# open-mmlab/PowerPaint

Hardware: AMD Instinct MI355X
Metric: inpainted images/sec @512x512, 50-step DDIM CFG, batch4/GPU (higher is better)
Workload: dtype bf16; 1 GPU; ppt-v1 SD1.5-inpaint UNet (9-ch in), 512x512, 50-step DDIM, CFG=7.5, bf16, batch=4/GPU; global_batch=4, denoise_steps=50, network_evaluations=50, parallelism=dp1 (image shards, no step collectives), hipgraph=True, weights=random init (no checkpoints offline)

## Files before the change

### include/pp_hip.h

```cpp
#ifndef PP_HIP_H_
#define PP_HIP_H_

#include <stddef.h>
#include <stdint.h>

#ifdef __cplusplus
extern "C" {
#endif

#define PP_OK 0
#define PP_ERR_BAD_ARG (-1)
#define PP_ERR_UNSUPPORTED (-2)
#define PP_ERR_LAUNCH (-3)
#define PP_ERR_WORKSPACE (-4)

#define PP_ABI_VERSION 29
#define PP_DT_F32 0
#define PP_DT_BF16 1
#define PP_DT_F16 2
int pp_abi_version(void);
const char* pp_build_id(void);
const char* pp_last_error(void);

#define PP_X_PLAIN 0
#define PP_X_CONV3X3 1
#define PP_ACT_NONE 0
#define PP_ACT_GEGLU 1
#define PP_ACT_SILU 2
#define PP_ACT_SOFTMAX80 3

typedef struct PPGemmArgs {
  int32_t M, N, K;
  int32_t x_mode;
  const void* x1;
  const void* x2;
  int32_t c1, c2;
  int32_t ldx1, ldx2;
  int32_t batch, hin, win, hout, wout, stride, up;
  const void* w;
  const float* bias;
  const float* rowvec;
  int32_t ld_rowvec, rows_per_batch;
  const void* res1;
  int32_t ldres1;
  const void* res2;
  int32_t ldres2;
  float scale;
  int32_t act;
  void* out;
  int32_t ldo;
  int32_t out_f32;
  void* out_vt;
  int32_t vt_col0;
  int32_t vt_ld;
  int32_t splitk;
  int32_t tile;
  float* workspace;
  int32_t dbg;
  int32_t dtype;
  int32_t out_dup_rows;
  int32_t res1_wrap_rows;
  float* row_stats_out;
  const float* ln_stats;
  const float* ln_colsum;
  int32_t ln_tiles;
  int32_t ln_dim;
  float ln_eps;
  int32_t w_batch_stride;
  int64_t* gn_acc[2];
  int32_t gn_cg[2];
  int32_t gn_c0[2];
  int32_t gn_groups[2];
  const void* x3;
  const void* x4;
  int32_t c3;
  int32_t c4;
  const int64_t* gn_in_acc;
  const float* gn_in_gb;
  int32_t gn_in_groups;
  int32_t gn_in_silu;
  float gn_in_eps;
  int32_t gn_dup_batch;
  void* gn_next_out;
  const float* gn_next_gamma;
  const float* gn_next_beta;
  float gn_next_eps;
  int32_t gn_next_silu;
  int32_t gn_next_sub;
  int32_t gn_dup_mask;
  int32_t vec_batch_stride;
  uint64_t* tile_ctr;
  uint32_t* combine_fault;
  int32_t subpix;
} PPGemmArgs;
#define PP_GN_SUM_SCALE 16777216.0f
#define PP_GN_SQ_SCALE 1048576.0f

#define PP_TILE_AUTO 0
#define PP_TILE_128x160 1
#define PP_TILE_64x160 2
#define PP_TILE_256x160 3

int pp_gemm_bf16(const PPGemmArgs* args, void* stream);
size_t pp_gemm_workspace_bytes(const PPGemmArgs* args);
int pp_gemm_gn_stats_ok(const PPGemmArgs* args);
int pp_conv_gn_supported(const PPGemmArgs* args);
int pp_conv_gn_preferred(const PPGemmArgs* args);
int pp_upconv_subpix_supported(int batch, int h, int w, int cin, int cout, int dtype);
int pp_upconv_subpix_supported_to(int batch, int h, int w, int hout, int wout, int cin, int cout, int dtype);
int pp_upconv_fold(const void* w, int cout, int cin, int dtype, void* out, void* stream);
int pp_gemm_gn_next_ok(const PPGemmArgs* args, int sub);
size_t pp_gemm_combine_ctr_bytes(const PPGemmArgs* args);
int pp_gemm_combine_fused(const PPGemmArgs* args);
int pp_xcd_placement_ok(void);

int pp_linear_skinny(const float* x, int rows, int K, const void* w, const float* bias, int N, float* out, int ldo,
                     int act_in, int act_out, int dtype, void* stream);

int pp_timestep_embedding(const float* t_dev, int rows, int dim, float* out, void* stream);

size_t pp_groupnorm_workspace_bytes(int batch, int hw, int C);
int pp_groupnorm_stats(const void* x1, int c1, const void* x2, int c2, int batch, int hw, int groups,
                       float* workspace, int dtype, void* stream);
int pp_groupnorm_apply(const void* x1, int c1, const void* x2, int c2, int batch, int hw, int groups, float eps,
                       const float* gamma, const float* beta, const float* workspace, int silu, void* y,
                       int dtype, void* stream);

int pp_groupnorm_apply_acc(const void* x1, int c1, const void* x2, int c2, int batch, int hw, int groups, float eps,
                           const float* gamma, const float* beta, const int64_t* acc, int silu, void* y, int dtype,
                           void* stream);
int pp_zero_u64(void* dst, long long n, void* stream);

int pp_layernorm(const void* x, int rows, int C, const float* gamma, const float* beta, float eps, void* y,
                 int dtype, void* stream);

int pp_attention_fwd(const void* q, int ldq, const void* k, int ldk, const void* vt, int ldvt, void* o, int ldo,
                     int batch, int heads, int nq, int nk, int d, float scale, int dtype, void* stream);
#define PP_ATTN_AUTO 0
#define PP_ATTN_PHASED 1
#define PP_ATTN_PIPE_Q32 2
#define PP_ATTN_PIPE_Q64 3
#define PP_ATTN_PIPE_LOG2 4
int pp_attention_log2_ok(int nq, int nk, int d);
int pp_attention_fwd_variant(const void* q, int ldq, const void* k, int ldk, const void* vt, int ldvt, void* o, int ldo,
                             int batch, int heads, int nq, int nk, int d, float scale, int dtype, int variant,
                             void* stream);
int pp_transpose_v(const void* v, int ld, int batch, int nk, int cols, void* vt, int ldvt, void* stream);

int pp_conv3x3_direct(const void* x, int batch, int hin, int win, int cin, const void* w, const float* bias,
                      int cout, int stride, int silu_out, const void* add, void* out, int dtype, void* stream);
int pp_conv3x3_smallcout(const void* x, int batch, int h, int w_, int cin, const void* w, const float* bias, int cout,
                         float* out_nchw, int dtype, void* stream);
int pp_gn_conv3x3_smallcout_supported(int cin, int cout, int groups);
int pp_gn_conv3x3_smallcout(const void* x, int batch, int h, int w, int cin, int groups, float eps, const float* gamma,
                            const float* beta, const int64_t* acc, const void* wgt, const float* bias, int cout,
                            float* out_nchw, int dtype, void* stream);

int pp_nchw_to_nhwc(const void* src, int src_dtype, int batch, int c, int hw, int src_batch_mod, void* dst, int ldc,
                    int c0, int dtype, void* stream);
int pp_nhwc_to_nchw(const void* src, int batch, int c, int hw, void* dst, int dst_dtype, int dtype, void* stream);
int pp_add_bf16(const void* a, const void* b, void* out, long long n, int dtype, void* stream);

int pp_cfg_sched_step(const float* eps2, int cfg, float guidance, float* latents, float* m_prev, int n, int kind,
                      const float* coef_table, int32_t* step_dev, uint32_t* advance_ticket, void* stream);
int pp_ddim_variance_noise(float* latents, const float* noise, int n, const float* coef_table, const int32_t* step_dev,
                           void* stream);
int pp_cfg_lcm_step(const float* eps2, int cfg, float guidance, float* latents, const float* noise, int n,
                    const float* coef_table, int32_t* step_dev, uint32_t* advance_ticket, void* stream);
int pp_cfg_sigma_step(const float* eps2, int cfg, float guidance, float* latents, const float* noise, int n,
                      const float* coef_table, int32_t* step_dev, uint32_t* advance_ticket, void* stream);
int pp_cfg_ksampler_step(const float* eps2, int cfg, float guidance, float* latents, float* state, const float* noise, int n,
                         const float* coef_table, int32_t* step_dev, uint32_t* advance_ticket, void* stream);

int pp_tfront_supported(int M, int c, int rows_per_batch, int gn_groups);
int pp_tfront(const void* x, int ldx, const void* gn_acc, const float* gn_gamma, const float* gn_beta, float gn_eps, int gn_groups,
              const void* w1, const float* b1, const void* w2p, const float* cs2, const float* b2, float ln_eps, void* hs,
              int ldhs, void* qk, int ldqk, void* vt, int ldvt, int M, int c, int rows_per_batch, float q_scale, int dtype,
              void* stream);
int pp_xattn_block_supported(int M, int c, int rows_per_batch, int nctx, int heads);
int pp_xattn_fold(const void* k, int ldk, const void* vt, int ldvt, int batch, int nctx, int heads, int c, const void* wq,
                  const float* q_colsum, const float* q_bias, const void* wo, float scale, void* gt, float* gcs,
                  float* gbias, void* ht, int kperm, int dtype, void* stream);
int pp_xattn_block(const void* x, int ldx, const void* res, int ldres, const float* ln_stats, int ln_tiles, float ln_eps,
                   const void* gt, const float* gcs, const float* gbias, const void* ht, const float* bias_o, void* out,
                   int ldo, float* row_stats_out, int M, int c, int rows_per_batch, int src_wrap_rows, const void* pre_w,
                   const float* pre_b, int dtype, void* stream);

int pp_ff_fused_supported(int M, int c, int rows_per_batch);
int pp_ff_fused(const PPGemmArgs* g2, const void* w1, const float* b1, const float* cs1, const float* ln_stats, int ln_tiles,
                float ln_eps, int w2_kperm, void* stream);

int pp_latent_blend(float* latents, const float* image_latents, const float* mask, const float* noise,
                    const float* renoise_table, const int32_t* step_dev, int batch, int channels, int hw, void* stream);

int pp_step_head(const float* temb_table, const int32_t* step_dev, float* temb_out, int row_floats, const float* latents,
                 int batch, int c, int hw, int src_batch_mod, void* x_in, int ldc, int c0, int dtype, void* zero_dst,
                 long long n_zero, void* stream);
int pp_step_head_scaled(const float* temb_table, const int32_t* step_dev, float* temb_out, int row_floats, const float* latents,
                        int batch, int c, int hw, int src_batch_mod, void* x_in, int ldc, int c0, int dtype, void* zero_dst,
                        long long n_zero, const float* in_div, void* stream);
int pp_step_select_t(const float* timesteps, const int32_t* step_dev, float* t_out, void* stream);
int pp_step_advance(int32_t* step_dev, void* stream);

int pp_mask_prep(int mode, const float* a, const float* b, float* out, int batch, int c, int h, int w, int ho, int wo,
                 void* stream);

int pp_embed_splice(const void* table, const void* ext, const int32_t* src_row, void* out, int n_rows,
                    long long row_bytes, void* stream);

int pp_softmax_rows(const float* s, long long lds, int rows, int n, float scale, void* p, long long ldp, int dtype,
                    void* stream);

int pp_attention_small(const void* q, int ldq, const void* k, int ldk, const void* v, int ldv, void* o, int ldo,
                       int batch, int heads, int nq, int nk, int d, float scale, int causal, int dtype, void* stream);

#define PP_LORA_MAX_ADAPTERS 8
#define PP_LORA_MAX_RANK 128
#define PP_LORA_ROWS_PLAIN 0
#define PP_LORA_ROWS_GEGLU 1
#define PP_LORA_COLS_PLAIN 0
#define PP_LORA_COLS_IGEMM 1
#define PP_LORA_COLS_KPERM 2
#define PP_LORA_COLS_KPERM_GEGLU 3
typedef struct PPLoraMergeArgs {
  int32_t N, K;
  const float* w;
  int64_t ldw;
  int32_t n_adapters;
  int32_t rank[PP_LORA_MAX_ADAPTERS];
  float coef[PP_LORA_MAX_ADAPTERS];
  const float* up[PP_LORA_MAX_ADAPTERS];
  const float* down[PP_LORA_MAX_ADAPTERS];
  const float* gamma;
  const float* beta;
  const float* badd;
  void* out;
  int64_t ldo;
  int32_t out_rows, out_cols, out_dtype;
  int32_t row_mode, row_off;
  int32_t col_mode, col_off, taps, cin_pad;
  float* colsum;
  float* bias;
} PPLoraMergeArgs;
int pp_lora_merge(const PPLoraMergeArgs* args, void* stream);

int pp_freeu(const void* hidden, void* hidden_out, int ch, const void* skip, void* skip_out, int cs, int batch, int h, int w,
             const float* bs, int64_t* acc, int groups, int dtype, void* stream);

#define PP_IP_MAX_TOKENS 64
int pp_ip_attn_add(const void* q, int ldq, const void* k_ip, const void* v_ip, void* o, int ldo, int batch, int heads, int nq,
                   int nk, int d, float qk_scale, float ip_scale, int dtype, void* stream);

#ifdef __cplusplus
}
#endif
#endif
```

### powerpaint_amd/_lib.py

```python
import ctypes as C
import os

_HERE = os.path.dirname(os.path.abspath(__file__))
LIB_PATH = os.path.join(_HERE, "libpp_hip.so")
if os.environ.get("PP_LAB") == "1" and os.environ.get("PP_LIB"):
    LIB_PATH = os.path.abspath(os.environ["PP_LIB"])

PP_X_PLAIN, PP_X_CONV3X3 = 0, 1
PP_ACT_NONE, PP_ACT_GEGLU, PP_ACT_SILU, PP_ACT_SOFTMAX80 = 0, 1, 2, 3
PP_TILE_AUTO, PP_TILE_128x160, PP_TILE_64x160, PP_TILE_256x160 = 0, 1, 2, 3
PP_DT_F32, PP_DT_BF16, PP_DT_F16 = 0, 1, 2
PP_ATTN_AUTO, PP_ATTN_PHASED, PP_ATTN_PIPE_Q32, PP_ATTN_PIPE_Q64, PP_ATTN_PIPE_LOG2 = 0, 1, 2, 3, 4
ABI_VERSION = 29
PP_ERR = {0: "PP_OK", -1: "PP_ERR_BAD_ARG", -2: "PP_ERR_UNSUPPORTED", -3: "PP_ERR_LAUNCH", -4: "PP_ERR_WORKSPACE"}

vp, i32, f32, sz = C.c_void_p, C.c_int32, C.c_float, C.c_size_t


class PPGemmArgs(C.Structure):
    _fields_ = [
        ("M", i32), ("N", i32), ("K", i32), ("x_mode", i32),
        ("x1", vp), ("x2", vp),
        ("c1", i32), ("c2", i32), ("ldx1", i32), ("ldx2", i32),
        ("batch", i32), ("hin", i32), ("win", i32), ("hout", i32), ("wout", i32), ("stride", i32), ("up", i32),
        ("w", vp), ("bias", vp), ("rowvec", vp),
        ("ld_rowvec", i32), ("rows_per_batch", i32),
        ("res1", vp), ("ldres1", i32),
        ("res2", vp), ("ldres2", i32),
        ("scale", f32), ("act", i32),
        ("out", vp), ("ldo", i32), ("out_f32", i32),
        ("out_vt", vp), ("vt_col0", i32), ("vt_ld", i32),
        ("splitk", i32), ("tile", i32),
        ("workspace", vp),
        ("dbg", i32), ("dtype", i32), ("out_dup_rows", i32), ("res1_wrap_rows", i32),
        ("row_stats_out", vp), ("ln_stats", vp), ("ln_colsum", vp),
        ("ln_tiles", i32), ("ln_dim", i32), ("ln_eps", f32), ("w_batch_stride", i32),
        ("gn_acc", vp * 2), ("gn_cg", i32 * 2), ("gn_c0", i32 * 2), ("gn_groups", i32 * 2),
        ("x3", vp), ("x4", vp), ("c3", i32), ("c4", i32),
        ("gn_in_acc", vp), ("gn_in_gb", vp), ("gn_in_groups", i32), ("gn_in_silu", i32), ("gn_in_eps", f32),
        ("gn_dup_batch", i32),
        ("gn_next_out", vp), ("gn_next_gamma", vp), ("gn_next_beta", vp), ("gn_next_eps", f32), ("gn_next_silu", i32),
        ("gn_next_sub", i32), ("gn_dup_mask", i32), ("vec_batch_stride", i32),
        ("tile_ctr", vp), ("combine_fault", vp),
        ("subpix", i32),
    ]


def gemm_args(dtype: int, M: int, N: int, K: int, x, w, out, x2=None, K2: int = 0, ldx=None, ldx2: int = 0, ldo: int = 0,
              ldres1: int = 0, ldres2: int = 0, rows_per_batch: int = 0, scale: float = 1.0) -> PPGemmArgs:
    a = PPGemmArgs()
    a.dtype = dtype
    a.M, a.N, a.K, a.x_mode = M, N, K + K2, PP_X_PLAIN
    a.x1, a.x2, a.c1, a.c2 = x, x2 or None, K, K2
    a.ldx1, a.ldx2 = (K if ldx is None else ldx), (ldx2 or K2)
    a.w, a.out = w, out
    a.ldo, a.ldres1, a.ldres2 = ldo or N, ldres1 or N, ldres2 or N
    a.rows_per_batch, a.scale = rows_per_batch, scale
    return a


def conv3x3_args(dtype: int, B: int, H: int, W: int, c1: int, cout: int, x, x2=None, c2: int = 0, x3=None, c3: int = 0,
                 x4=None, c4: int = 0, stride: int = 1, up: bool = False, w=None, out=None, scale: float = 1.0,
                 up_size=None) -> PPGemmArgs:
    hv, wv = (2 * H, 2 * W) if up else (H, W)
    if up_size is not None:
        if not up or stride != 1 or up_size[0] not in (2 * H - 1, 2 * H) or up_size[1] not in (2 * W - 1, 2 * W):
            raise ValueError(f"up_size {tuple(up_size)} is no nearest-resize target of a {H}x{W} source")
        hv, wv = up_size
    ho, wo = (hv - 1) // stride + 1, (wv - 1) // stride + 1
    a = PPGemmArgs()
    a.dtype = dtype
    a.M, a.N, a.K, a.x_mode = B * ho * wo, cout, 9 * (c1 + c2) + c3 + c4, PP_X_CONV3X3
    a.x1, a.x2, a.c1, a.c2 = x, x2 or None, c1, c2
    a.x3, a.x4, a.c3, a.c4 = x3 or None, x4 or None, c3, c4
    a.batch, a.hin, a.win, a.hout, a.wout, a.stride, a.up = B, H, W, ho, wo, stride, int(up)
    a.w, a.out = w, out
    a.ldo, a.ldres1, a.ldres2 = cout, cout, cout
    a.rows_per_batch, a.scale = ho * wo, scale
    return a


PP_LORA_MAX_ADAPTERS, PP_LORA_MAX_RANK = 8, 128
PP_LORA_ROWS_PLAIN, PP_LORA_ROWS_GEGLU = 0, 1
PP_IP_MAX_TOKENS = 64
PP_LORA_COLS_PLAIN, PP_LORA_COLS_IGEMM, PP_LORA_COLS_KPERM, PP_LORA_COLS_KPERM_GEGLU = 0, 1, 2, 3


class PPLoraMergeArgs(C.Structure):
    _fields_ = [
        ("N", i32), ("K", i32), ("w", vp), ("ldw", C.c_int64), ("n_adapters", i32),
        ("rank", i32 * PP_LORA_MAX_ADAPTERS), ("coef", f32 * PP_LORA_MAX_ADAPTERS),
        ("up", vp * PP_LORA_MAX_ADAPTERS), ("down", vp * PP_LORA_MAX_ADAPTERS),
        ("gamma", vp), ("beta", vp), ("badd", vp),
        ("out", vp), ("ldo", C.c_int64), ("out_rows", i32), ("out_cols", i32), ("out_dtype", i32),
        ("row_mode", i32), ("row_off", i32), ("col_mode", i32), ("col_off", i32), ("taps", i32), ("cin_pad", i32),
        ("colsum", vp), ("bias", vp),
    ]


SIGNATURES = {
    "pp_abi_version": (C.c_int, []),
    "pp_last_error": (C.c_char_p, []),
    "pp_build_id": (C.c_char_p, []),
    "pp_gemm_bf16": (C.c_int, [C.POINTER(PPGemmArgs), vp]),
    "pp_gemm_workspace_bytes": (sz, [C.POINTER(PPGemmArgs)]),
    "pp_linear_skinny": (C.c_int, [vp, C.c_int, C.c_int, vp, vp, C.c_int, vp, C.c_int, C.c_int, C.c_int, C.c_int, vp]),
    "pp_timestep_embedding": (C.c_int, [vp, C.c_int, C.c_int, vp, vp]),
    "pp_groupnorm_workspace_bytes": (sz, [C.c_int, C.c_int, C.c_int]),
    "pp_gemm_gn_stats_ok": (C.c_int, [C.POINTER(PPGemmArgs)]),
    "pp_conv_gn_supported": (C.c_int, [C.POINTER(PPGemmArgs)]),
    "pp_conv_gn_preferred": (C.c_int, [C.POINTER(PPGemmArgs)]),
    "pp_gemm_gn_next_ok": (C.c_int, [C.POINTER(PPGemmArgs), C.c_int]),
    "pp_upconv_subpix_supported": (C.c_int, [C.c_int] * 6),
    "pp_upconv_subpix_supported_to": (C.c_int, [C.c_int] * 8),
    "pp_upconv_fold": (C.c_int, [vp, C.c_int, C.c_int, C.c_int, vp, vp]),
    "pp_gemm_combine_ctr_bytes": (sz, [C.POINTER(PPGemmArgs)]),
    "pp_gemm_combine_fused": (C.c_int, [C.POINTER(PPGemmArgs)]),
    "pp_xcd_placement_ok": (C.c_int, []),
    "pp_groupnorm_apply_acc": (C.c_int, [vp, C.c_int, vp, C.c_int, C.c_int, C.c_int, C.c_int, f32, vp, vp, vp, C.c_int, vp,
                                         C.c_int, vp]),
    "pp_zero_u64": (C.c_int, [vp, C.c_longlong, vp]),
    "pp_embed_splice": (C.c_int, [vp, vp, vp, vp, C.c_int, C.c_longlong, vp]),
    "pp_attention_small": (C.c_int, [vp, C.c_int, vp, C.c_int, vp, C.c_int, vp, C.c_int, C.c_int, C.c_int, C.c_int,
                                     C.c_int, C.c_int, f32, C.c_int, C.c_int, vp]),
    "pp_softmax_rows": (C.c_int, [vp, C.c_longlong, C.c_int, C.c_int, f32, vp, C.c_longlong, C.c_int, vp]),
    "pp_groupnorm_stats": (C.c_int, [vp, C.c_int, vp, C.c_int, C.c_int, C.c_int, C.c_int, vp, C.c_int, vp]),
    "pp_groupnorm_apply": (C.c_int, [vp, C.c_int, vp, C.c_int, C.c_int, C.c_int, C.c_int, f32, vp, vp, vp, C.c_int, vp,
                                     C.c_int, vp]),
    "pp_layernorm": (C.c_int, [vp, C.c_int, C.c_int, vp, vp, f32, vp, C.c_int, vp]),
    "pp_attention_fwd": (C.c_int, [vp, C.c_int, vp, C.c_int, vp, C.c_int, vp, C.c_int, C.c_int, C.c_int, C.c_int,
                                   C.c_int, C.c_int, f32, C.c_int, vp]),
    "pp_attention_fwd_variant": (C.c_int, [vp, C.c_int, vp, C.c_int, vp, C.c_int, vp, C.c_int, C.c_int, C.c_int, C.c_int,
                                           C.c_int, C.c_int, f32, C.c_int, C.c_int, vp]),
    "pp_transpose_v": (C.c_int, [vp, C.c_int, C.c_int, C.c_int, C.c_int, vp, C.c_int, vp]),
    "pp_conv3x3_direct": (C.c_int, [vp, C.c_int, C.c_int, C.c_int, C.c_int, vp, vp, C.c_int, C.c_int, C.c_int, vp,
                                    vp, C.c_int, vp]),
    "pp_conv3x3_smallcout": (C.c_int, [vp, C.c_int, C.c_int, C.c_int, C.c_int, vp, vp, C.c_int, vp, C.c_int, vp]),
    "pp_nchw_to_nhwc": (C.c_int, [vp, C.c_int, C.c_int, C.c_int, C.c_int, C.c_int, vp, C.c_int, C.c_int, C.c_int, vp]),
    "pp_nhwc_to_nchw": (C.c_int, [vp, C.c_int, C.c_int, C.c_int, vp, C.c_int, C.c_int, vp]),
    "pp_add_bf16": (C.c_int, [vp, vp, vp, C.c_longlong, C.c_int, vp]),
    "pp_cfg_sched_step": (C.c_int, [vp, C.c_int, f32, vp, vp, C.c_int, C.c_int, vp, vp, vp, vp]),
    "pp_step_select_t": (C.c_int, [vp, vp, vp, vp]),
    "pp_ddim_variance_noise": (C.c_int, [vp, vp, C.c_int, vp, vp, vp]),
    "pp_cfg_lcm_step": (C.c_int, [vp, C.c_int, f32, vp, vp, C.c_int, vp, vp, vp, vp]),
    "pp_cfg_sigma_step": (C.c_int, [vp, C.c_int, f32, vp, vp, C.c_int, vp, vp, vp, vp]),
    "pp_cfg_ksampler_step": (C.c_int, [vp, C.c_int, f32, vp, vp, vp, C.c_int, vp, vp, vp, vp]),
    "pp_latent_blend": (C.c_int, [vp, vp, vp, vp, vp, vp, C.c_int, C.c_int, C.c_int, vp]),
    "pp_gn_conv3x3_smallcout_supported": (C.c_int, [C.c_int] * 3),
    "pp_gn_conv3x3_smallcout": (C.c_int, [vp, C.c_int, C.c_int, C.c_int, C.c_int, C.c_int, C.c_float, vp, vp, vp, vp, vp,
                                          C.c_int, vp, C.c_int, vp]),
    "pp_tfront_supported": (C.c_int, [C.c_int] * 4),
    "pp_tfront": (C.c_int, [vp, C.c_int, vp, vp, vp, C.c_float, C.c_int, vp, vp, vp, vp, vp, C.c_float, vp, C.c_int, vp, C.c_int,
                            vp, C.c_int, C.c_int, C.c_int, C.c_int, C.c_float, C.c_int, vp]),
    "pp_attention_log2_ok": (C.c_int, [C.c_int] * 3),
    "pp_xattn_block_supported": (C.c_int, [C.c_int] * 5),
    "pp_xattn_fold": (C.c_int, [vp, C.c_int, vp, C.c_int, C.c_int, C.c_int, C.c_int, C.c_int, vp, vp, vp, vp, C.c_float,
                                vp, vp, vp, vp, C.c_int, C.c_int, vp]),
    "pp_xattn_block": (C.c_int, [vp, C.c_int, vp, C.c_int, vp, C.c_int, C.c_float, vp, vp, vp, vp, vp, vp, C.c_int, vp,
                                 C.c_int, C.c_int, C.c_int, C.c_int, vp, vp, C.c_int, vp]),
    "pp_ff_fused_supported": (C.c_int, [C.c_int] * 3),
    "pp_ff_fused": (C.c_int, [C.POINTER(PPGemmArgs), vp, vp, vp, vp, C.c_int, C.c_float, C.c_int, vp]),
    "pp_step_head": (C.c_int, [vp, vp, vp, C.c_int, vp, C.c_int, C.c_int, C.c_int, C.c_int, vp, C.c_int, C.c_int, C.c_int, vp,
                              C.c_longlong, vp]),
    "pp_step_head_scaled": (C.c_int, [vp, vp, vp, C.c_int, vp, C.c_int, C.c_int, C.c_int, C.c_int, vp, C.c_int, C.c_int, C.c_int,
                                     vp, C.c_longlong, vp, vp]),
    "pp_step_advance": (C.c_int, [vp, vp]),
    "pp_lora_merge": (C.c_int, [C.POINTER(PPLoraMergeArgs), vp]),
    "pp_freeu": (C.c_int, [vp, vp, C.c_int, vp, vp, C.c_int, C.c_int, C.c_int, C.c_int, vp, vp, C.c_int, C.c_int, vp]),
    "pp_mask_prep": (C.c_int, [C.c_int, vp, vp, vp, C.c_int, C.c_int, C.c_int, C.c_int, C.c_int, C.c_int, vp]),
    "pp_ip_attn_add": (C.c_int, [vp, C.c_int, vp, vp, vp, C.c_int, C.c_int, C.c_int, C.c_int, C.c_int, C.c_int, f32, f32,
                                 C.c_int, vp]),
}

_lib = None


class PPError(RuntimeError):
    pass


def lib():
    global _lib
    if _lib is None:
        if not os.path.exists(LIB_PATH):
            raise PPError(
                f"{LIB_PATH} not found: the HIP extension is not built. Run `python -c 'import __graft_entry__ as g; "
                f"g.build()'` (or `make -C powerpaint_amd/csrc`). There is no CPU/PyTorch fallback.")
        l = C.CDLL(LIB_PATH)
        for name, (res, args) in SIGNATURES.items():
            fn = getattr(l, name)
            fn.restype = res
            fn.argtypes = args
        if l.pp_abi_version() != ABI_VERSION:
            raise PPError("libpp_hip.so ABI version mismatch")
        _lib = l
    return _lib


def dtype_code(dtype) -> int:
    import torch
    if dtype == torch.bfloat16:
        return PP_DT_BF16
    if dtype == torch.float16:
        return PP_DT_F16
    raise PPError(f"the HIP path computes in bf16 or fp16 (fp32 accumulate), not {dtype}")


def build_id() -> str:
    return lib().pp_build_id().decode()


def check(rc: int, what: str = ""):
    if rc != 0:
        msg = lib().pp_last_error().decode() if rc == -3 else ""
        raise PPError(f"{what} failed: {PP_ERR.get(rc, rc)} {msg}")
```

### powerpaint_amd/csrc/conv_gn.hip

```cpp
#include <type_traits>
#include <utility>

#include "pp_common.h"
#include "gemm_gn.h"
#include "gemm_combine.h"

namespace {

typedef __attribute__((address_space(3))) void* cg_lds_t;

constexpr int CG_T = 512, CG_BN = 160, CG_NI = 5;
constexpr int CG_WP = 3;
constexpr int CG_HPW_MAX = 6;
constexpr int CG_HALO_PX = 384;
constexpr int CG_HALO = CG_HALO_PX * 128;
constexpr int CG_WST = CG_BN * 128;
constexpr int CG_WOFF = 2 * CG_HALO;
constexpr int CG_TAB = CG_WOFF + 3 * CG_WST;
constexpr int CG_T_STATS = CG_TAB;
constexpr int CG_T_ZERO = CG_TAB + 256;
constexpr int CG_T_GB = CG_TAB + 1024;
constexpr int CG_T_SCSH = CG_TAB + 3072;
constexpr int CG_LDS = CG_TAB + 3584;
static_assert(CG_LDS <= 160 * 1024, "LDS budget");

struct CGDerived {
  int tiles_m, tiles_n, n_major;
  int nch1, nch;
  int ntail3, ntail;
  int hp;
  int cg;
  float inv_cg;
};

template <int... I, class F>
PP_DEVINL void cg_static_for_impl(std::integer_sequence<int, I...>, F&& f) { (f(std::integral_constant<int, I>{}), ...); }
template <int N, class F>
PP_DEVINL void cg_static_for(F&& f) { cg_static_for_impl(std::make_integer_sequence<int, N>{}, f); }

template <int BM, int HPW, bool PP, int NMODE, int EDT>
__global__ void __launch_bounds__(CG_T, 2) pp_conv_gn_kernel(const PPGemmArgs a, const CGDerived d) {
  using E = E16<EDT>;
  typedef typename E::v8 v8_t;
  constexpr int T = CG_T, WN = 2, MI = BM / 64, NI = CG_NI, BN = CG_BN;
  constexpr int CG_HPW = HPW;
  constexpr bool SUBPIX = NMODE == 4;
  static_assert(!SUBPIX || PP, "the sub-pixel form has the ping-pong loop only");
  constexpr bool NORM = NMODE != 2 && !SUBPIX;
  constexpr bool NREAD = NMODE == 0 || NMODE == 3;
  static_assert(HPW >= 2 && HPW <= CG_HPW_MAX, "halo strips per wave");
  constexpr int XP2 = BM / 64;
  constexpr int P2 = XP2 + CG_WP;
  constexpr int ST2 = BM * 128;
  constexpr int EPI_ROWS = 64, EPI_LD = BN * 4 + 16;
  constexpr int RS_OFF = EPI_ROWS * EPI_LD + BM * 8;
  static_assert(3 * ST2 <= 2 * CG_HALO, "tail stages live in the halo buffers");
  static_assert(MI * 16 <= EPI_ROWS && EPI_ROWS % (MI * 16) == 0, "wave rows vs epilogue pass");

  extern __shared__ __attribute__((aligned(16))) char smem[];

  const int tid = threadIdx.x;
  const int lane = tid & 63;
  const int wave = __builtin_amdgcn_readfirstlane(tid >> 6);
  const int wm = wave >> 1, wn = wave & 1;
  const int grp = wave >> 2;

  int lid;
  {
    const int nwg = gridDim.x, bid = blockIdx.x;
    const int q = nwg >> 3, r = nwg & 7, xcd = bid & 7, idx = bid >> 3;
    lid = (xcd < r ? xcd * (q + 1) : r * (q + 1) + (xcd - r) * q) + idx;
  }
  const int par = SUBPIX ? (lid & 3) : 0, pa = par >> 1, pb = par & 1;
  if constexpr (SUBPIX) lid >>= 2;
  int tile_m, tile_n;
  if (d.n_major) {
    tile_n = lid / d.tiles_m;
    tile_m = lid - tile_n * d.tiles_m;
  } else {
    tile_m = lid / d.tiles_n;
    tile_n = lid - tile_m * d.tiles_n;
  }
  const int m_blk = tile_m * BM, n_blk = tile_n * BN;
  const int split = blockIdx.y, splits = gridDim.y;
  const int ch_b = split * d.nch / splits, ch_e = (split + 1) * d.nch / splits;
  const int tk_b = split * d.ntail / splits, tk_e = (split + 1) * d.ntail / splits;

  const int Wd = a.wout, Hd = a.hout, HW = Hd * Wd;
  const int HWs = a.hin * a.win;
  const int bimg = m_blk / HW;
  const int y0 = (m_blk - bimg * HW) / Wd;
  const int ctot = a.c1 + a.c2;
  const uint32_t wbytes = (uint32_t)a.N * (uint32_t)a.K * 2u;
  const void* const wmat = SUBPIX ? (const void*)((const char*)a.w + (size_t)par * wbytes) : a.w;

  const int lrow = lane >> 3;
  const int kslot = (lane & 7) ^ lrow;

  int vw[CG_WP], wlds[CG_WP];
#pragma unroll
  for (int i = 0; i < CG_WP; ++i) {
    const int strip = (wave * 8 + i * 64 < BN) ? i : i - 1;
    const int n = n_blk + wave * 8 + lrow + strip * 64;
    vw[i] = (n < a.N) ? (n * a.K + kslot * 8) * 2 : (int)PP_OOB;
    wlds[i] = (wave * 8 + strip * 64) * 128;
  }
  int hpix[CG_HPW];
#pragma unroll
  for (int j = 0; j < CG_HPW; ++j) {
    const int hp = (wave + 8 * j) * 8 + lrow;
    const int hr = hp / Wd, hx = hp - hr * Wd;
    const int iy = y0 + hr - 1;
    hpix[j] = (hp < d.hp && iy >= 0 && iy < Hd) ? (a.up ? bimg * HWs + (iy >> 1) * a.win + (hx >> 1) : bimg * HW + iy * Wd + hx) : -1;
  }
  const int r16 = lane & 15, g = lane >> 4;
  const int fsw = r16 & 7;
  const int wrow0 = wn * (NI * 16) + r16;
  const int rt0 = wm * (MI * 16) + r16;
  unsigned edge = 0u;
#pragma unroll
  for (int mi = 0; mi < MI; ++mi) {
    const int lx = (rt0 + mi * 16) % Wd;
    if (lx == 0) edge |= 1u << mi;
    if (lx == Wd - 1) edge |= 1u << (8 + mi);
  }

  f32x4_t acc[NI][MI];
#pragma unroll
  for (int ni = 0; ni < NI; ++ni)
#pragma unroll
    for (int mi = 0; mi < MI; ++mi) acc[ni][mi] = f32x4_t{0.f, 0.f, 0.f, 0.f};

  auto mfma_all = [&](const v8_t (&wf)[2][NI], const v8_t (&xf)[2][MI]) __attribute__((always_inline)) {
#pragma unroll
    for (int ks = 0; ks < 2; ++ks)
#pragma unroll
      for (int ni = 0; ni < NI; ++ni)
#pragma unroll
        for (int mi = 0; mi < MI; ++mi) acc[ni][mi] = E::mfma16(wf[ks][ni], xf[ks][mi], acc[ni][mi]);
  };

  if (ch_b < ch_e) {
    auto issue_gb = [&](int c, int gbuf, bool live) __attribute__((always_inline)) {
      const __amdgpu_buffer_rsrc_t rs = make_rsrc(a.gn_in_gb, (NORM && live) ? (uint32_t)ctot * 8u : 0u);
      const int vo = lane < 32 ? lane * 16 : (int)PP_OOB;
      __builtin_amdgcn_raw_ptr_buffer_load_lds(rs, (cg_lds_t)(smem + CG_T_GB + gbuf * 1024), 16, vo, c * 512, 0, 0);
    };
    auto compute_scsh = [&](int c, int gbuf) __attribute__((always_inline)) {
      const char* gp = smem + CG_T_GB + gbuf * 1024 + kslot * 64;
      const f32x2_t* st = reinterpret_cast<const f32x2_t*>(smem + CG_T_STATS);
#pragma unroll
      for (int q = 0; q < 4; ++q) {
        const f32x4_t gbv = *reinterpret_cast<const f32x4_t*>(gp + q * 16);
        f32x4_t o;
#pragma unroll
        for (int h = 0; h < 2; ++h) {
          const int ch = c * 64 + kslot * 8 + 2 * q + h;
          const int gi = min((int)(((float)ch + 0.5f) * d.inv_cg), 31);
          const f32x2_t mr = st[gi];
          const float sv = mr[1] * gbv[2 * h];
          o[2 * h] = sv;
          o[2 * h + 1] = gbv[2 * h + 1] - mr[0] * sv;
        }
        if (lrow == 0) *reinterpret_cast<f32x4_t*>(smem + CG_T_SCSH + kslot * 64 + q * 16) = o;
      }
      asm volatile("s_waitcnt lgkmcnt(0)" ::: "memory");
    };
    auto norm_piece = [&](int hbuf, int j) __attribute__((always_inline)) {
      char* p = smem + hbuf * CG_HALO + (wave + 8 * j) * 1024 + lane * 16;
      if (hpix[j] >= 0) {
        const u32x4_t v = *reinterpret_cast<const u32x4_t*>(p);
        float r[8];
#pragma unroll
        for (int q = 0; q < 4; ++q) {
          const f32x4_t ss = *reinterpret_cast<const f32x4_t*>(smem + CG_T_SCSH + kslot * 64 + q * 16);
          r[2 * q] = E::lo(v[q]) * ss[0] + ss[1];
          r[2 * q + 1] = E::hi(v[q]) * ss[2] + ss[3];
        }
#pragma unroll
        for (int e = 0; e < 8; ++e)
          r[e] = r[e] * __builtin_amdgcn_rcpf(1.0f + __builtin_amdgcn_exp2f(r[e] * -1.44269504088896340736f));
        u32x4_t o;
#pragma unroll
        for (int q = 0; q < 4; ++q) o[q] = E::pack2(r[2 * q], r[2 * q + 1]);
        *reinterpret_cast<u32x4_t*>(p) = o;
      }
    };

    auto norm_math = [&](const u32x4_t v, uint32_t vmask) __attribute__((always_inline)) -> u32x4_t {
      u32x4_t o;
#pragma unroll
      for (int q = 0; q < 4; ++q) {
        const f32x4_t ss = *reinterpret_cast<const f32x4_t*>(smem + CG_T_SCSH + kslot * 64 + q * 16);
        float r0 = E::lo(v[q]) * ss[0] + ss[1];
        float r1 = E::hi(v[q]) * ss[2] + ss[3];
        const float e0 = __builtin_amdgcn_exp2f(r0 * -1.44269504088896340736f);
        const float e1 = __builtin_amdgcn_exp2f(r1 * -1.44269504088896340736f);
        r0 *= __builtin_amdgcn_rcpf(1.0f + e0);
        r1 *= __builtin_amdgcn_rcpf(1.0f + e1);
        o[q] = E::pack2(r0, r1) & vmask;
      }
      return o;
    };

    __amdgpu_buffer_rsrc_t rs_h = make_rsrc(a.x1, 0u);
    int hsoff = 0, hcsrc = 0;
    auto halo_source = [&](int c, bool live) __attribute__((always_inline)) {
      const bool first = c < d.nch1;
      int csrc;
      if (first) {
        csrc = a.c1;
        rs_h = make_rsrc(a.x1, live ? (uint32_t)a.batch * (uint32_t)HWs * (uint32_t)a.c1 * 2u : 0u);
        hsoff = c * 128;
      } else {
        csrc = a.c2;
        rs_h = make_rsrc(a.x2 ? a.x2 : a.x1, (live && a.x2) ? (uint32_t)a.batch * (uint32_t)HWs * (uint32_t)a.c2 * 2u : 0u);
        hsoff = (c - d.nch1) * 128;
      }
      hcsrc = csrc;
    };
    auto issue_halo_piece = [&](int hbuf, int j) __attribute__((always_inline)) {
      const int vo = hpix[j] >= 0 ? (hpix[j] * hcsrc + kslot * 8) * 2 : (int)PP_OOB;
      __builtin_amdgcn_raw_ptr_buffer_load_lds(rs_h, (cg_lds_t)(smem + hbuf * CG_HALO + (wave + 8 * j) * 1024), 16, vo,
                                               hsoff, 0, 0);
    };
    auto issue_w_piece = [&](const __amdgpu_buffer_rsrc_t rs, int stage, int i, int sow) __attribute__((always_inline)) {
      const int vo = vw[i], lo = wlds[i];
      __builtin_amdgcn_raw_ptr_buffer_load_lds(rs, (cg_lds_t)(smem + CG_WOFF + stage * CG_WST + lo), 16, vo, sow, 0, 0);
    };

    {
      const __amdgpu_buffer_rsrc_t rsw = make_rsrc(wmat, wbytes);
#pragma unroll
      for (int i = 0; i < CG_WP; ++i) issue_w_piece(rsw, 0, i, (0 * ctot + ch_b * 64) * 2);
#pragma unroll
// ... 349 lines not shown
        }
#pragma unroll
        for (int j = 0; j < EP; ++j) {
          const int row = r0 + j * ER, m = m0 + row;
          if (row < EPI_ROWS && m < a.M) {
            f32x4_t v0 = *reinterpret_cast<const f32x4_t*>(smem + row * EPI_LD + c8 * 32);
            f32x4_t v1 = *reinterpret_cast<const f32x4_t*>(smem + row * EPI_LD + c8 * 32 + 16);
            v0 += bs0;
            v1 += bs1;
            v0 *= a.scale;
            v1 *= a.scale;
            v0[0] += E::lo(r1[j][0]) + E::lo(r2[j][0]); v0[1] += E::hi(r1[j][0]) + E::hi(r2[j][0]);
            v0[2] += E::lo(r1[j][1]) + E::lo(r2[j][1]); v0[3] += E::hi(r1[j][1]) + E::hi(r2[j][1]);
            v1[0] += E::lo(r1[j][2]) + E::lo(r2[j][2]); v1[1] += E::hi(r1[j][2]) + E::hi(r2[j][2]);
            v1[2] += E::lo(r1[j][3]) + E::lo(r2[j][3]); v1[3] += E::hi(r1[j][3]) + E::hi(r2[j][3]);
            u32x4_t o;
            o[0] = E::pack2(v0[0], v0[1]); o[1] = E::pack2(v0[2], v0[3]);
            o[2] = E::pack2(v1[0], v1[1]); o[3] = E::pack2(v1[2], v1[3]);
            *reinterpret_cast<u32x4_t*>((uint16_t*)a.out + (SUBPIX ? out_row(m) : (size_t)m) * a.ldo + n) = o;
            if (gns) {
#pragma unroll
              for (int jj = 0; jj < 4; ++jj) {
                const float lo = E::lo(o[jj]), hi = E::hi(o[jj]);
                gcs[2 * jj] += lo; gcq[2 * jj] += lo * lo;
                gcs[2 * jj + 1] += hi; gcq[2 * jj + 1] += hi * hi;
              }
            }
          }
        }
      }
    }
  }
  if (gns) {
    unsigned long long* slots = reinterpret_cast<unsigned long long*>(smem + RS_OFF);
    if (tid < 2 * GN_SLOTS * 2) slots[tid] = 0ull;
    asm volatile("s_waitcnt lgkmcnt(0)\n\ts_barrier" ::: "memory");
    if (r0 < ER && n < a.N) {
      float* dstp = reinterpret_cast<float*>(smem) + ((size_t)r0 * BN + c8 * 8) * 2;
#pragma unroll
      for (int jj = 0; jj < 4; ++jj)
        *reinterpret_cast<f32x4_t*>(dstp + 4 * jj) = f32x4_t{gcs[2 * jj], gcq[2 * jj], gcs[2 * jj + 1], gcq[2 * jj + 1]};
    }
    asm volatile("s_waitcnt lgkmcnt(0)\n\ts_barrier" ::: "memory");
    const int ncols = min(BN, a.N - n_blk);
    if (tid < ncols) {
      float sm = 0.f, sq = 0.f;
#pragma unroll 5
      for (int r = 0; r < ER; ++r) {
        const f32x2_t v = *reinterpret_cast<const f32x2_t*>(smem + ((size_t)r * BN + tid) * 8);
        sm += v[0];
        sq += v[1];
      }
      gn_column(a, slots, n_blk, tid, sm, sq);
    }
    asm volatile("s_waitcnt lgkmcnt(0)\n\ts_barrier" ::: "memory");
    gn_flush(a, slots, m_blk, n_blk, ncols, tid);
  }
  if (splitk && a.tile_ctr) {
    static_assert(fc_lds_bytes(BM) <= CG_LDS, "fused combine staging must fit in the kernel's LDS");
    splitk_fused_combine<BM, T, EDT>(a, smem, m_blk, n_blk, blockIdx.x, blockIdx.y, splits, tid);
  }
}

bool cg_shape_ok(const PPGemmArgs& a, int bm) {
  const int hw = a.hout * a.wout;
  return bm % a.wout == 0 && hw % bm == 0 && bm + 2 * a.wout <= CG_HALO_PX;
}

bool cg_geometry_ok(const PPGemmArgs& a) {
  if (a.x_mode != PP_X_CONV3X3 || !pp_dt_ok(a.dtype)) return false;
  if (a.stride != 1 || a.wout < 8 || (a.wout & 7)) return false;
  if (a.up ? (a.hout != 2 * a.hin || a.wout != 2 * a.win) : (a.hin != a.hout || a.win != a.wout)) return false;
  const int ctot = a.c1 + a.c2;
  if (a.c1 <= 0 || a.c1 % 64 || a.c2 % 64 || (a.c2 > 0 && !a.x2)) return false;
  if (a.c3 < 0 || a.c4 < 0 || a.c3 % 64 || a.c4 % 64 || (a.c3 > 0 && !a.x3) || (a.c4 > 0 && (!a.x4 || a.c3 == 0))) return false;
  if (a.K != (a.subpix ? 4 : 9) * ctot + a.c3 + a.c4 || a.M != a.batch * a.hout * a.wout || a.M <= 0 || a.N <= 0) return false;
  if (a.N % 8 || a.ldo % 8 || a.out_f32 || a.out_vt || a.act != PP_ACT_NONE || a.ln_stats || a.row_stats_out) return false;
  if ((a.res1 && a.ldres1 % 8) || (a.res2 && a.ldres2 % 8)) return false;
  if (a.rows_per_batch != a.hout * a.wout || a.out_dup_rows > 0 || a.w_batch_stride > 0 || a.vec_batch_stride > 0) return false;
  if ((uint64_t)a.batch * a.hin * a.win * (uint64_t)(a.c1 > a.c2 ? a.c1 : a.c2) * 2u >= 0x80000000ull) return false;
  if ((uint64_t)a.N * (uint64_t)a.K * 2u >= 0x80000000ull) return false;
  if ((uint64_t)a.M * (uint64_t)(a.c3 > a.c4 ? a.c3 : a.c4) * 2u >= 0x80000000ull) return false;
  for (int k = 0; k < 2; ++k)
    if (a.gn_acc[k] && (a.gn_cg[k] < 8 || a.gn_groups[k] <= 0 || a.gn_c0[k] < 0)) return false;
  return cg_shape_ok(a, 256) || cg_shape_ok(a, 128) || cg_shape_ok(a, 64);
}

bool cg_fused_ok(const PPGemmArgs& a) {
  if (!a.gn_in_acc || !a.gn_in_gb || a.up || a.subpix || !cg_geometry_ok(a)) return false;
  if (a.gn_in_silu != 1 || a.gn_in_groups <= 0 || a.gn_in_groups > 32) return false;
  return (a.c1 + a.c2) % a.gn_in_groups == 0;
}

bool cg_raw_ok(const PPGemmArgs& a) {
  static const int min_w = pp_lab_env("PP_CONV_RAW", 16);
  if (a.gn_in_acc || a.gn_in_gb || a.subpix || a.tile != PP_TILE_AUTO || min_w <= 0 || a.wout < min_w) return false;
  return cg_geometry_ok(a);
}

bool cg_subpix_ok(const PPGemmArgs& a) {
  if (a.subpix != 1 || a.up || a.gn_in_acc || a.gn_in_gb || a.c2 || a.c3 || a.c4 || a.splitk > 1) return false;
  if (a.res1_wrap_rows > 0 || a.gn_next_out || a.gn_dup_mask) return false;
  return cg_geometry_ok(a);
}

CGChoice cg_choose_subpix(const PPGemmArgs& a) {
  const int tn = (a.N + 159) / 160;
  const int want = a.tile == PP_TILE_256x160 ? 256 : a.tile == PP_TILE_128x160 ? 128 : a.tile == PP_TILE_64x160 ? 64 : 0;
  if (want && cg_shape_ok(a, want)) return CGChoice{want, 1};
  for (int bm = 256; bm >= 64; bm >>= 1)
    if (cg_shape_ok(a, bm) && 4 * (a.M / bm) * tn >= 224) return CGChoice{bm, 1};
  return CGChoice{cg_shape_ok(a, 256) ? 256 : cg_shape_ok(a, 128) ? 128 : 64, 1};
}

CGChoice cg_choose(const PPGemmArgs& a) {
  const int tn = (a.N + 159) / 160;
  auto tiles = [&](int bm) { return (a.M / bm) * tn; };
  CGChoice c{0, 1};
  const int want = a.tile == PP_TILE_256x160 ? 256 : a.tile == PP_TILE_128x160 ? 128 : a.tile == PP_TILE_64x160 ? 64 : 0;
  const int nch0 = (a.c1 + a.c2) / 64;
  static const int sk2_from = pp_lab_env("PP_CONV_GN_SK2", 12);
#ifdef PP_LAB
  static const int w16 = pp_lab_env("PP_CONV_GN_W16", 0);
  if (w16 > 0 && a.wout == 16 && !want && a.splitk <= 0 && cg_shape_ok(a, w16 / 10)) {
    c.bm = w16 / 10;
    c.splitk = w16 % 10;
    if (c.splitk > nch0) c.splitk = nch0;
    return c;
  }
#endif
  if (want && cg_shape_ok(a, want)) c.bm = want;
  else if (cg_shape_ok(a, 256) && tiles(256) >= 224) c.bm = 256;
  else if (sk2_from > 0 && nch0 >= sk2_from && a.splitk <= 0 && cg_shape_ok(a, 256) && tiles(256) * 2 >= 224 &&
           tiles(256) < 224 && cg_shape_ok(a, 128) && tiles(128) >= 224) {
    c.bm = 256;
    c.splitk = 2;
    return c;
  }
  else if (cg_shape_ok(a, 128) && tiles(128) >= 224) c.bm = 128;
  else if (cg_shape_ok(a, 256) && cg_shape_ok(a, 128) && tiles(256) * 4 <= 256 && nch0 <= 10 && a.splitk <= 0) c.bm = 128;
  else if (cg_shape_ok(a, 256)) c.bm = 256;
  else if (cg_shape_ok(a, 128)) c.bm = 128;
  else c.bm = 64;
  const int nch = (a.c1 + a.c2) / 64;
  int sk = 1;
  while (tiles(c.bm) * sk * 2 <= 256 && nch / (sk * 2) >= 2 && sk < 8) sk *= 2;
  c.splitk = a.splitk > 0 ? a.splitk : sk;
  if (c.splitk > 8) c.splitk = 8;
  if (c.splitk > nch) c.splitk = nch;
  return c;
}

template <int BM, int HPW, bool PP, int NMODE, int EDT>
int cg_launch(const PPGemmArgs& a, int splitk, hipStream_t st) {
  auto kern = pp_conv_gn_kernel<BM, HPW, PP, NMODE, EDT>;
  if (pp_func_lds(reinterpret_cast<const void*>(kern), CG_LDS, "hipFuncSetAttribute(conv_gn)") != PP_OK) return PP_ERR_LAUNCH;
  CGDerived d;
  d.tiles_m = a.M / BM;
  d.tiles_n = (a.N + CG_BN - 1) / CG_BN;
  d.n_major = (d.tiles_m < d.tiles_n && d.tiles_m <= 8) ? 1 : 0;
  d.nch1 = a.c1 / 64;
  d.nch = (a.c1 + a.c2) / 64;
  d.ntail3 = a.c3 / 64;
  d.ntail = (a.c3 + a.c4) / 64;
  d.hp = BM + 2 * a.wout;
  d.cg = a.gn_in_groups > 0 ? (a.c1 + a.c2) / a.gn_in_groups : 1;
  d.inv_cg = 1.0f / (float)d.cg;
  hipLaunchKernelGGL(kern, dim3(d.tiles_m * d.tiles_n * (NMODE == 4 ? 4 : 1), splitk, 1), dim3(CG_T), CG_LDS, st, a, d);
  PP_CHECK_LAUNCH("pp_conv_gn_kernel");
  return PP_OK;
}

template <int BM, bool PP, int NMODE, int EDT>
int cg_launch_hpw(const PPGemmArgs& a, int splitk, hipStream_t st) {
  const int need = (BM + 2 * a.wout + 63) / 64;
  if constexpr (BM == 256) {
    if (need <= 5) return cg_launch<256, 5, PP, NMODE, EDT>(a, splitk, st);
    return cg_launch<256, 6, PP, NMODE, EDT>(a, splitk, st);
  } else if constexpr (BM == 128) {
    if (need <= 3) return cg_launch<128, 3, PP, NMODE, EDT>(a, splitk, st);
    if (need <= 4) return cg_launch<128, 4, PP, NMODE, EDT>(a, splitk, st);
    return cg_launch<128, 6, PP, NMODE, EDT>(a, splitk, st);
  } else {
    if (need <= 2) return cg_launch<64, 2, PP, NMODE, EDT>(a, splitk, st);
    return cg_launch<64, 3, PP, NMODE, EDT>(a, splitk, st);
  }
}

template <int EDT>
int cg_dispatch(const PPGemmArgs& a, const CGChoice& c, hipStream_t st) {
#ifdef PP_LAB
  static const int pp = pp_lab_env("PP_CONV_GN_PP", 1), nm = pp_lab_env("PP_CONV_GN_NMODE", 1);
  if (!pp || nm != 1) {
#define CG_CASE(BM_)                                                                        \
    case BM_:                                                                               \
      if (!pp) return cg_launch_hpw<BM_, false, 1, EDT>(a, c.splitk, st);                   \
      if (nm == 0) return cg_launch_hpw<BM_, true, 0, EDT>(a, c.splitk, st);                \
      if (nm == 2) return cg_launch_hpw<BM_, true, 2, EDT>(a, c.splitk, st);                \
      return cg_launch_hpw<BM_, true, 3, EDT>(a, c.splitk, st);
    switch (c.bm) {
      CG_CASE(256)
      CG_CASE(128)
      default:
      CG_CASE(64)
    }
#undef CG_CASE
  }
#endif
  if (a.subpix) {
    switch (c.bm) {
      case 256: return cg_launch_hpw<256, true, 4, EDT>(a, 1, st);
      case 128: return cg_launch_hpw<128, true, 4, EDT>(a, 1, st);
      default: return cg_launch_hpw<64, true, 4, EDT>(a, 1, st);
    }
  }
  if (!a.gn_in_acc) {
    switch (c.bm) {
      case 256: return cg_launch_hpw<256, true, 2, EDT>(a, c.splitk, st);
      case 128: return cg_launch_hpw<128, true, 2, EDT>(a, c.splitk, st);
      default: return cg_launch_hpw<64, true, 2, EDT>(a, c.splitk, st);
    }
  }
  switch (c.bm) {
    case 256: return cg_launch_hpw<256, true, 1, EDT>(a, c.splitk, st);
    case 128: return cg_launch_hpw<128, true, 1, EDT>(a, c.splitk, st);
    default: return cg_launch_hpw<64, true, 1, EDT>(a, c.splitk, st);
  }
}

}

int pp_conv_gn_form(const PPGemmArgs& a, CGChoice* c) {
  if (a.x_mode != PP_X_CONV3X3) return 0;
  if (a.subpix) {
    if (!cg_subpix_ok(a)) return PP_ERR_UNSUPPORTED;
    *c = cg_choose_subpix(a);
    return 1;
  }
  if (a.gn_in_acc) {
    if (!cg_fused_ok(a)) return PP_ERR_UNSUPPORTED;
  } else if (!cg_raw_ok(a)) {
    return 0;
  }
  *c = cg_choose(a);
  return 1;
}
int pp_conv_gn_run(const PPGemmArgs& a, const CGChoice& c, hipStream_t st) {
  if (c.splitk > 1 && !a.workspace) return PP_ERR_WORKSPACE;
  return a.dtype == PP_DT_F16 ? cg_dispatch<PP_DT_F16>(a, c, st) : cg_dispatch<PP_DT_BF16>(a, c, st);
}

extern "C" int pp_conv_gn_supported(const PPGemmArgs* args) {
  if (!args) return 0;
  return cg_fused_ok(*args) ? 1 : cg_raw_ok(*args) ? 2 : 0;
}

extern "C" int pp_upconv_subpix_supported(int batch, int h, int w, int cin, int cout, int dtype) {
  if (batch <= 0 || h <= 0 || w <= 0 || cin <= 0 || cout <= 0) return 0;
  PPGemmArgs a = {};
  a.x_mode = PP_X_CONV3X3;
  a.dtype = dtype;
  a.batch = batch;
  a.hin = a.hout = h;
  a.win = a.wout = w;
  a.stride = 1;
  a.c1 = cin;
  a.M = batch * h * w;
  a.N = cout;
  a.K = 4 * cin;
  a.ldo = a.ldres1 = a.ldres2 = cout;
  a.rows_per_batch = h * w;
  a.subpix = 1;
  if ((uint64_t)batch * h * w * 4u * (uint64_t)cout * 2u >= (1ull << 40)) return 0;
  if (!cg_subpix_ok(a)) return 0;
  return w >= 16 ? 2 : 1;
}

extern "C" int pp_upconv_subpix_supported_to(int batch, int h, int w, int hout, int wout, int cin, int cout, int dtype) {
  if (hout != 2 * h || wout != 2 * w) return 0;
  return pp_upconv_subpix_supported(batch, h, w, cin, cout, dtype);
}

extern "C" int pp_conv_gn_preferred(const PPGemmArgs* args) {
  if (!args || !cg_fused_ok(*args)) return 0;
  const PPGemmArgs& a = *args;
  const int nch = (a.c1 + a.c2) / 64;
  int cls;
  if (a.win >= 64) cls = 1;
  else if (a.win == 32) cls = (nch <= 5 && a.c2 == 0) ? 2 : 8;
  else if (a.win == 16) cls = 4;
  else cls = a.win < 16 ? 16 : 8;
  static const int mask = pp_lab_env("PP_CONV_GN_ROUTE", 0);
  return (mask & cls) ? 1 : 0;
}
```

### powerpaint_amd/csrc/gemm.hip

```cpp
#include "pp_common.h"
#include "gemm_gn.h"
#include "gemm_combine.h"

namespace {

struct GemmDerived {
  int tiles_m, tiles_n, kt_total, kt_per_split, ctiles;
  int n_major;
};

PP_DEVINL void ln_row_moments(const PPGemmArgs& a, int m, float& mean, float& rstd) {
  const f32x2_t* p = reinterpret_cast<const f32x2_t*>(a.ln_stats) + (size_t)m * a.ln_tiles;
  float s = 0.f, q = 0.f;
  for (int t = 0; t < a.ln_tiles; ++t) {
    const f32x2_t v = p[t];
    s += v[0];
    q += v[1];
  }
  const float inv = 1.0f / (float)a.ln_dim;
  mean = s * inv;
  rstd = rsqrtf(fmaxf(q * inv - mean * mean, 0.f) + a.ln_eps);
}

PP_DEVINL size_t res1_row(const PPGemmArgs& a, int m) {
  return (size_t)((a.res1_wrap_rows > 0 && m >= a.res1_wrap_rows) ? m - a.res1_wrap_rows : m);
}

template <int BN, int EDT>
PP_DEVINL void epilogue4(const PPGemmArgs& a, int m, int n, f32x4_t v) {
  if (a.ln_stats) {
    float mean, rstd;
    ln_row_moments(a, m, mean, rstd);
    const f32x4_t cs = *reinterpret_cast<const f32x4_t*>(a.ln_colsum + n);
    v = (v - cs * mean) * rstd;
  }
  if (a.bias) {
    const f32x4_t b = *reinterpret_cast<const f32x4_t*>(a.bias + n);
    v += b;
  }
  int bidx = 0, rin = m;
  if (a.rowvec || a.out_vt) {
    bidx = m / a.rows_per_batch;
    rin = m - bidx * a.rows_per_batch;
  }
  if (a.rowvec) {
    const f32x4_t t = *reinterpret_cast<const f32x4_t*>(a.rowvec + (size_t)bidx * a.ld_rowvec + n);
    v += t;
  }
  v *= a.scale;
  if (a.res1) {
    const u32x2_t r = *reinterpret_cast<const u32x2_t*>((const uint16_t*)a.res1 + res1_row(a, m) * a.ldres1 + n);
    v[0] += E16<EDT>::lo(r[0]); v[1] += E16<EDT>::hi(r[0]); v[2] += E16<EDT>::lo(r[1]); v[3] += E16<EDT>::hi(r[1]);
  }
  if (a.res2) {
    const u32x2_t r = *reinterpret_cast<const u32x2_t*>((const uint16_t*)a.res2 + (size_t)m * a.ldres2 + n);
    v[0] += E16<EDT>::lo(r[0]); v[1] += E16<EDT>::hi(r[0]); v[2] += E16<EDT>::lo(r[1]); v[3] += E16<EDT>::hi(r[1]);
  }
  if (a.act == PP_ACT_GEGLU) {
    const float o0 = v[0] * gelu_fast_f(v[2]);
    const float o1 = v[1] * gelu_fast_f(v[3]);
    *reinterpret_cast<uint32_t*>((uint16_t*)a.out + (size_t)m * a.ldo + (n >> 1)) = E16<EDT>::pack2(o0, o1);
    return;
  }
  if (a.act == PP_ACT_SILU) {
    v[0] = silu_f(v[0]); v[1] = silu_f(v[1]); v[2] = silu_f(v[2]); v[3] = silu_f(v[3]);
  }
  if (a.out_vt && n >= a.vt_col0) {
    const int ncols = a.N - a.vt_col0;
    uint16_t* dst = (uint16_t*)a.out_vt + ((size_t)bidx * ncols + (n - a.vt_col0)) * a.vt_ld + rin;
#pragma unroll
    for (int j = 0; j < 4; ++j) dst[(size_t)j * a.vt_ld] = E16<EDT>::from_f(v[j]);
    return;
  }
  if (a.out_f32) {
    *reinterpret_cast<f32x4_t*>((float*)a.out + (size_t)m * a.ldo + n) = v;
  } else {
    u32x2_t o;
    o[0] = E16<EDT>::pack2(v[0], v[1]);
    o[1] = E16<EDT>::pack2(v[2], v[3]);
    *reinterpret_cast<u32x2_t*>((uint16_t*)a.out + (size_t)m * a.ldo + n) = o;
  }
}

template <int BM, int BN, int WM, int WN, int XMODE, int EDT>
__global__ void __launch_bounds__(WM* WN * 64, 2) pp_gemm_kernel(const PPGemmArgs a, const GemmDerived d) {
  typedef typename E16<EDT>::v8 v8_t;
  constexpr int T = WM * WN * 64;
  constexpr int MI = BM / WM / 16;
  constexpr int NI = BN / WN / 16;
  constexpr int RPP = T / 8;
  constexpr int XP = (BM + RPP - 1) / RPP;
  constexpr int WP = (BN + RPP - 1) / RPP;
  constexpr int XBYTES = BM * 128, WBYTES = BN * 128, BUFBYTES = XBYTES + WBYTES;
  static_assert(BM % (WM * 16) == 0 && BN % (WN * 16) == 0, "tile/wave mismatch");

  extern __shared__ __attribute__((aligned(16))) char smem[];

  const int tid = threadIdx.x;
  const int lane = tid & 63;
  const int wave = tid >> 6;
  const int wm = wave / WN, wn = wave % WN;

  int lid;
  {
    const int nwg = gridDim.x, bid = blockIdx.x;
    const int q = nwg >> 3, r = nwg & 7, xcd = bid & 7, idx = bid >> 3;
    lid = (xcd < r ? xcd * (q + 1) : r * (q + 1) + (xcd - r) * q) + idx;
  }
  int tile_m, tile_n;
  if (d.n_major) {
    tile_n = lid / d.tiles_m;
    tile_m = lid - tile_n * d.tiles_m;
  } else {
    tile_m = lid / d.tiles_n;
    tile_n = lid - tile_m * d.tiles_n;
  }
  const int m_blk = tile_m * BM, n_blk = tile_n * BN;
  const int split = blockIdx.y;
  const int kt_begin = split * d.kt_per_split;
  int kt_end = kt_begin + d.kt_per_split;
  if (kt_end > d.kt_total) kt_end = d.kt_total;

  const int slot = tid & 7;
  const int prow = tid >> 3;
  const int lds_piece = prow * 128 + ((slot ^ (prow & 7)) << 4);

  const int ctot = a.c1 + a.c2;
  const __amdgpu_buffer_rsrc_t rs_x1 = make_rsrc(
      a.x1, XMODE == PP_X_PLAIN ? (uint32_t)a.M * (uint32_t)a.ldx1 * 2u
                                : (uint32_t)a.batch * (uint32_t)a.hin * (uint32_t)a.win * (uint32_t)a.c1 * 2u);
  const __amdgpu_buffer_rsrc_t rs_x2 = make_rsrc(
      a.x2 ? a.x2 : a.x1, !a.x2 ? 0u
                          : (XMODE == PP_X_PLAIN ? (uint32_t)a.M * (uint32_t)a.ldx2 * 2u
                                                 : (uint32_t)a.batch * (uint32_t)a.hin * (uint32_t)a.win * (uint32_t)a.c2 * 2u));
  const __amdgpu_buffer_rsrc_t rs_w = make_rsrc(a.w, (uint32_t)a.N * (uint32_t)a.K * 2u);

  bool xvalid[XP];
  int xa[XP], xb[XP], xc[XP];
#pragma unroll
  for (int i = 0; i < XP; ++i) {
    const int row = prow + i * RPP;
    const int m = m_blk + row;
    xvalid[i] = (row < BM) && (m < a.M);
    if (XMODE == PP_X_PLAIN) {
      xa[i] = m * a.ldx1;
      xb[i] = m * a.ldx2;
      xc[i] = 0;
    } else {
      const int hw = a.hout * a.wout;
      const int b = m / hw;
      const int rem = m - b * hw;
      const int oy = rem / a.wout;
      const int ox = rem - oy * a.wout;
      xa[i] = b * a.hin * a.win;
      xb[i] = oy * a.stride - 1;
      xc[i] = ox * a.stride - 1;
    }
  }
  bool wvalid[WP];
  int wo[WP];
#pragma unroll
  for (int i = 0; i < WP; ++i) {
    const int row = prow + i * RPP;
    const int n = n_blk + row;
    wvalid[i] = (row < BN) && (n < a.N);
    wo[i] = n * a.K;
  }

  int tap = 0, cc = 0;
  if (XMODE == PP_X_CONV3X3) {
    tap = kt_begin / d.ctiles;
    cc = (kt_begin - tap * d.ctiles) * 64;
  }
  const int hv = a.up ? (a.stride == 1 ? a.hout : a.hin * 2) : a.hin;
  const int wv = a.up ? (a.stride == 1 ? a.wout : a.win * 2) : a.win;

  u32x4_t xr[XP], wr[WP];

  auto load_tile = [&](int kt) {
    const int k0 = kt * 64;
    if (XMODE == PP_X_PLAIN) {
      const bool first = k0 < a.c1;
      const __amdgpu_buffer_rsrc_t rs = first ? rs_x1 : rs_x2;
      const int kk = (first ? k0 : k0 - a.c1) + slot * 8;
#pragma unroll
      for (int i = 0; i < XP; ++i) {
        const uint32_t off = xvalid[i] ? (uint32_t)((first ? xa[i] : xb[i]) + kk) * 2u : PP_OOB;
        xr[i] = __builtin_amdgcn_raw_buffer_load_b128(rs, off, 0, 0);
      }
    } else {
      const int ky = tap / 3, kx = tap - ky * 3;
      const bool first = cc < a.c1;
      const __amdgpu_buffer_rsrc_t rs = first ? rs_x1 : rs_x2;
      const int csrc = first ? a.c1 : a.c2;
      const int kk = (first ? cc : cc - a.c1) + slot * 8;
#pragma unroll
      for (int i = 0; i < XP; ++i) {
        const int iy = xb[i] + ky, ix = xc[i] + kx;
        const bool ok = xvalid[i] && (unsigned)iy < (unsigned)hv && (unsigned)ix < (unsigned)wv;
        const int sy = a.up ? (iy >> 1) : iy;
        const int sx = a.up ? (ix >> 1) : ix;
        const uint32_t off = ok ? (uint32_t)((xa[i] + sy * a.win + sx) * csrc + kk) * 2u : PP_OOB;
        xr[i] = __builtin_amdgcn_raw_buffer_load_b128(rs, off, 0, 0);
      }
      cc += 64;
      if (cc == ctot) { cc = 0; ++tap; }
    }
#pragma unroll
    for (int i = 0; i < WP; ++i) {
      const uint32_t off = wvalid[i] ? (uint32_t)(wo[i] + k0 + slot * 8) * 2u : PP_OOB;
      wr[i] = __builtin_amdgcn_raw_buffer_load_b128(rs_w, off, 0, 0);
    }
  };
  auto store_tile = [&](int buf) {
    char* xs = smem + buf * BUFBYTES;
    char* ws = xs + XBYTES;
#pragma unroll
    for (int i = 0; i < XP; ++i)
      if ((XP * RPP == BM) || (prow + i * RPP < BM)) *reinterpret_cast<u32x4_t*>(xs + lds_piece + i * RPP * 128) = xr[i];
#pragma unroll
    for (int i = 0; i < WP; ++i)
      if ((WP * RPP == BN) || (prow + i * RPP < BN)) *reinterpret_cast<u32x4_t*>(ws + lds_piece + i * RPP * 128) = wr[i];
  };

  f32x4_t acc[NI][MI];
#pragma unroll
  for (int ni = 0; ni < NI; ++ni)
#pragma unroll
    for (int mi = 0; mi < MI; ++mi) acc[ni][mi] = f32x4_t{0.f, 0.f, 0.f, 0.f};

  const int frow = lane & 15;
  const int fk = lane >> 4;
  const int xrow0 = wm * (MI * 16) + frow;
  const int wrow0 = wn * (NI * 16) + frow;
  const int fsw = frow & 7;

  if (kt_begin < kt_end) {
    load_tile(kt_begin);
    store_tile(0);
  }
  __syncthreads();

  int cur = 0;
  for (int kt = kt_begin; kt < kt_end; ++kt) {
    const bool more = (kt + 1 < kt_end);
    if (more) load_tile(kt + 1);

    const char* xs = smem + cur * BUFBYTES;
    const char* ws = xs + XBYTES;
#pragma unroll
    for (int ks = 0; ks < 2; ++ks) {
      const int so = ((ks * 4 + fk) ^ fsw) << 4;
      v8_t xf[MI], wf[NI];
#pragma unroll
      for (int mi = 0; mi < MI; ++mi)
        xf[mi] = *reinterpret_cast<const v8_t*>(xs + (xrow0 + mi * 16) * 128 + so);
#pragma unroll
      for (int ni = 0; ni < NI; ++ni)
        wf[ni] = *reinterpret_cast<const v8_t*>(ws + (wrow0 + ni * 16) * 128 + so);
#pragma unroll
      for (int ni = 0; ni < NI; ++ni)
#pragma unroll
        for (int mi = 0; mi < MI; ++mi)
          acc[ni][mi] = E16<EDT>::mfma16(wf[ni], xf[mi], acc[ni][mi], 0, 0, 0);
    }

    if (more) store_tile(cur ^ 1);
    __syncthreads();
    cur ^= 1;
  }

  const int m_base = m_blk + wm * (MI * 16) + (lane & 15);
  const int n_base = n_blk + wn * (NI * 16) + 4 * (lane >> 4);
  if (gridDim.y > 1) {
    float* ws = a.workspace + (size_t)split * a.M * a.N;
#pragma unroll
    for (int mi = 0; mi < MI; ++mi) {
      const int m = m_base + mi * 16;
#pragma unroll
      for (int ni = 0; ni < NI; ++ni) {
        const int n = n_base + ni * 16;
        if (m < a.M && n < a.N) *reinterpret_cast<f32x4_t*>(ws + (size_t)m * a.N + n) = acc[ni][mi];
      }
    }
    return;
  }
#pragma unroll
  for (int mi = 0; mi < MI; ++mi) {
    const int m = m_base + mi * 16;
#pragma unroll
    for (int ni = 0; ni < NI; ++ni) {
      const int n = n_base + ni * 16;
      if (m < a.M && n < a.N) epilogue4<BN, EDT>(a, m, n, acc[ni][mi]);
    }
  }
}

template <int BM, int BN, int WM, int WN, int XMODE, int NS, int EPI, bool DMAI, bool PP, int EDT>
__global__ void __launch_bounds__(WM* WN * 64, (PP ? 2 : (WM * WN == 8 && (BM / WM / 16) * (BN / WN / 16) <= 10 ? 4 : 2)))
pp_gemm_kernel_v2(const PPGemmArgs a, const GemmDerived d) {
  typedef typename E16<EDT>::v8 v8_t;
  constexpr bool LNF = EPI == 1 || EPI == 2 || EPI == 5;
  constexpr bool GNS = EPI == 4;
  constexpr int T = WM * WN * 64;
  constexpr int MI = BM / WM / 16;
  constexpr int NI = BN / WN / 16;
  constexpr int RPP = T / 8;
  constexpr int XP = BM / RPP;
  constexpr int WP = (BN + RPP - 1) / RPP;
  constexpr int P = XP + WP;
  constexpr int XBYTES = BM * 128, WBYTES = BN * 128, STAGE = XBYTES + WBYTES;
  constexpr int EPI_ROWS = 64;
  constexpr int EPI_LD = BN * 4 + 16;
  static_assert(BM % RPP == 0, "X tile must be whole passes");
  static_assert(P * (NS - 1) < 64, "vmcnt field");
  constexpr int LN_OFF = EPI_ROWS * EPI_LD;
  constexpr int RS_OFF = LN_OFF + BM * 8;
  static_assert(RS_OFF + EPI_ROWS * (BN / 8) * 8 <= NS * STAGE, "epilogue staging must fit in the pipeline stages");
  static_assert(MI * 16 <= EPI_ROWS && EPI_ROWS % (MI * 16) == 0, "wave rows vs epilogue pass");
  constexpr int LN_TMAX = 4;
  constexpr int PRE_B = NS * STAGE, PRE_C = PRE_B + 1024, PRE_M = PRE_C + 1024;

  extern __shared__ __attribute__((aligned(16))) char smem[];
  typedef __attribute__((address_space(3))) void* lds_ptr_t;

  const int tid = threadIdx.x;
  const int lane = tid & 63;
  const int wave = __builtin_amdgcn_readfirstlane(tid >> 6);
  const int wm = wave / WN, wn = wave % WN;

  int lid;
  {
    const int nwg = gridDim.x, bid = blockIdx.x;
    const int q = nwg >> 3, r = nwg & 7, xcd = bid & 7, idx = bid >> 3;
    lid = (xcd < r ? xcd * (q + 1) : r * (q + 1) + (xcd - r) * q) + idx;
  }
  int tile_m, tile_n;
  if (d.n_major) {
    tile_n = lid / d.tiles_m;
    tile_m = lid - tile_n * d.tiles_m;
  } else {
    tile_m = lid / d.tiles_n;
    tile_n = lid - tile_m * d.tiles_n;
  }
  const int m_blk = tile_m * BM, n_blk = tile_n * BN;
  const int split = blockIdx.y;
  const int kt_begin = split * d.kt_per_split;
  int kt_end = kt_begin + d.kt_per_split;
  if (kt_end > d.kt_total) kt_end = d.kt_total;
  const int nkt = kt_end - kt_begin;
#if defined(PP_LAB) && defined(PP_GEMM_DBG)
  const int dbg = a.dbg;
#elif defined(PP_LAB)
  const int dbg = PP ? 0 : a.dbg;
#else
  constexpr int dbg = 0;
#endif

  const int lrow = lane >> 3;
  const int kslot = (lane & 7) ^ lrow;
  const int prow = wave * 8 + lrow;

  const int ctot = a.c1 + a.c2;
  const uint32_t xbytes1 = XMODE == PP_X_PLAIN ? (uint32_t)a.M * (uint32_t)a.ldx1 * 2u
                                               : (uint32_t)a.batch * (uint32_t)a.hin * (uint32_t)a.win * (uint32_t)a.c1 * 2u;
  const uint32_t xbytes2 = !a.x2 ? 0u
                           : (XMODE == PP_X_PLAIN ? (uint32_t)a.M * (uint32_t)a.ldx2 * 2u
                                                  : (uint32_t)a.batch * (uint32_t)a.hin * (uint32_t)a.win * (uint32_t)a.c2 * 2u);
  const uint32_t wbytes = (uint32_t)a.N * (uint32_t)a.K * 2u;
  const int bitem = a.w_batch_stride > 0 ? m_blk / a.rows_per_batch : 0;
  const void* const w_base = reinterpret_cast<const uint16_t*>(a.w) + (size_t)bitem * (size_t)a.w_batch_stride;

  int vx1[XP], vx2[XP];
  int xa[XP], xb[XP], xc[XP];
#pragma unroll
  for (int i = 0; i < XP; ++i) {
    const int m = m_blk + prow + i * RPP;
    const bool ok = m < a.M;
    if (XMODE == PP_X_PLAIN) {
      vx1[i] = ok ? (m * a.ldx1 + kslot * 8) * 2 : (int)PP_OOB;
      vx2[i] = ok ? (m * a.ldx2 + kslot * 8) * 2 : (int)PP_OOB;
      xa[i] = xb[i] = xc[i] = 0;
    } else {
      const int hw = a.hout * a.wout;
      const int b = m / hw;
      const int rem = m - b * hw;
      const int oy = rem / a.wout;
      const int ox = rem - oy * a.wout;
      xa[i] = ok ? b * a.hin * a.win : -1;
      xb[i] = oy * a.stride - 1;
      xc[i] = ox * a.stride - 1;
      vx1[i] = (int)PP_OOB;
      vx2[i] = (int)PP_OOB;
    }
  }
  int vw[WP];
  int wlds[WP];
#pragma unroll
  for (int i = 0; i < WP; ++i) {
    const int strip = (wave * 8 + i * RPP < BN) ? i : i - 1;
    const int n = n_blk + prow + strip * RPP;
    vw[i] = (n < a.N) ? (n * a.K + kslot * 8) * 2 : (int)PP_OOB;
    wlds[i] = (wave * 8 + strip * RPP) * 128;
  }

  int tap = 0, cc = 0;
  bool retap = true;
  if (XMODE == PP_X_CONV3X3) {
    tap = kt_begin / d.ctiles;
    if (tap > 9) tap = 9;
    cc = (kt_begin - tap * d.ctiles) * 64;
  }
  const uint64_t px1 = reinterpret_cast<uint64_t>(a.x1), px2 = reinterpret_cast<uint64_t>(a.x2);
  const uint64_t px3 = XMODE == PP_X_CONV3X3 ? reinterpret_cast<uint64_t>(a.x3) : 0ull;
  const uint64_t px4 = XMODE == PP_X_CONV3X3 ? reinterpret_cast<uint64_t>(a.x4) : 0ull;
  const int pc1 = a.c1, pc2 = a.c2, pc3 = XMODE == PP_X_CONV3X3 ? a.c3 : 0, pc4 = XMODE == PP_X_CONV3X3 ? a.c4 : 0;
  uint64_t cur_src = px1;
  uint32_t cur_bytes = 0u;
  int cur_cA = pc1, cur_c0 = 0;
  const uint32_t xbytes3 = (XMODE == PP_X_CONV3X3 && a.x3) ? (uint32_t)a.M * (uint32_t)a.c3 * 2u : 0u;
  const uint32_t xbytes4 = (XMODE == PP_X_CONV3X3 && a.x4) ? (uint32_t)a.M * (uint32_t)a.c4 * 2u : 0u;
  const int hv = a.up ? (a.stride == 1 ? a.hout : a.hin * 2) : a.hin;
  const int wv = a.up ? (a.stride == 1 ? a.wout : a.win * 2) : a.win;

  __amdgpu_buffer_rsrc_t is_rsx, is_rsw;
  int is_sox = 0, is_sow = 0, is_second = 0;
  char* is_xs = smem;
  char* is_ws = smem;
  auto issue_begin = [&](int kt, int stage) __attribute__((always_inline)) {
    is_xs = smem + stage * STAGE;
    is_ws = is_xs + XBYTES;
    const bool live = kt < kt_end;
    const int k0 = kt * 64;
    if (XMODE == PP_X_PLAIN) {
      const bool first = k0 < a.c1;
      is_rsx = make_rsrc(first ? a.x1 : a.x2, live ? (first ? xbytes1 : xbytes2) : 0u);
      is_sox = (first ? k0 : k0 - a.c1) * 2;
      is_second = first ? 0 : 1;
    } else {
      const bool tail = tap >= 9;
      if (live && (retap || cc == 0 || cc == cur_cA)) {
        const bool first = cc < (tail ? pc3 : pc1);
        int csrc;
        if (!tail) {
          cur_cA = pc1;
          if (first) { cur_src = px1; cur_bytes = xbytes1; csrc = pc1; cur_c0 = 0; }
          else { cur_src = px2; cur_bytes = xbytes2; csrc = pc2; cur_c0 = pc1; }
        } else {
          cur_cA = pc3;
          if (first) { cur_src = px3; cur_bytes = xbytes3; csrc = pc3; cur_c0 = 0; }
          else { cur_src = px4; cur_bytes = xbytes4; csrc = pc4; cur_c0 = pc3; }
        }
        const int ky = tail ? 1 : tap / 3, kx = tail ? 1 : tap - (tap / 3) * 3;
#pragma unroll
        for (int i = 0; i < XP; ++i) {
          const int iy = xb[i] + ky, ix = xc[i] + kx;
          const bool ok = xa[i] >= 0 && (unsigned)iy < (unsigned)hv && (unsigned)ix < (unsigned)wv;
          const int sy = a.up ? (iy >> 1) : iy;
          const int sx = a.up ? (ix >> 1) : ix;
          vx1[i] = ok ? ((xa[i] + sy * a.win + sx) * csrc + kslot * 8) * 2 : (int)PP_OOB;
        }
        retap = false;
      }
      is_rsx = make_rsrc(reinterpret_cast<const void*>(cur_src), live ? cur_bytes : 0u);
      is_sox = (cc - cur_c0) * 2;
      if (live) {
        cc += 64;
        if (!tail && cc == ctot) { cc = 0; ++tap; retap = true; }
      }
    }
    is_rsw = make_rsrc(w_base, live ? wbytes : 0u);
    is_sow = k0 * 2;
  };
  auto issue_piece = [&](int i) __attribute__((always_inline)) {
    if (i < XP) {
      const int ii = i < XP ? i : 0;
      const int vo = (XMODE == PP_X_PLAIN && is_second) ? vx2[ii] : vx1[ii];
      __builtin_amdgcn_raw_ptr_buffer_load_lds(is_rsx, (lds_ptr_t)(is_xs + (wave * 8 + ii * RPP) * 128), 16, vo, is_sox,
                                               0, 0);
    } else {
      const int j = i - XP < WP ? i - XP : 0;
      const int vo = vw[j], lo = wlds[j];
      __builtin_amdgcn_raw_ptr_buffer_load_lds(is_rsw, (lds_ptr_t)(is_ws + lo), 16, vo, is_sow, 0, 0);
    }
  };
  auto issue = [&](int kt, int stage) __attribute__((always_inline)) {
    issue_begin(kt, stage);
#pragma unroll
    for (int i = 0; i < P; ++i) issue_piece(i);
  };

  f32x4_t acc[NI][MI];
#pragma unroll
  for (int ni = 0; ni < NI; ++ni)
#pragma unroll
    for (int mi = 0; mi < MI; ++mi) acc[ni][mi] = f32x4_t{0.f, 0.f, 0.f, 0.f};

// ... 706 lines not shown
  }
  *reinterpret_cast<f32x4_t*>(&tile[row][c8 * 8]) = w0;
  *reinterpret_cast<f32x4_t*>(&tile[row][c8 * 8 + 4]) = w1;
  __syncthreads();
  const int ncols = min(BN, a.N - n_blk);
  if (tid < ncols) {
    float sm = 0.f, sq = 0.f;
#pragma unroll
    for (int r = 0; r < ROWS; ++r) {
      const float v = tile[r][tid];
      sm += v;
      sq += v * v;
    }
    gn_column(a, slots, n_blk, tid, sm, sq);
  }
  __syncthreads();
  gn_flush(a, slots, m0, n_blk, ncols, tid);
}

template <int EDT>
__global__ void __launch_bounds__(640) pp_splitk_reduce_gn_apply_kernel(const PPGemmArgs a, int splits, int tiles_n, int rows_pass) {
  using E = E16<EDT>;
  constexpr int BN = 40, EC = BN / 8, RMAX = 128;
  __shared__ __attribute__((aligned(16))) char vals[256 * BN * 2];
  __shared__ __attribute__((aligned(16))) float tile[RMAX][BN + 4];
  __shared__ unsigned long long slots[2 * GN_SLOTS * 2];
  __shared__ __attribute__((aligned(16))) float sc_s[BN], sh_s[BN];
  const int tid = threadIdx.x;
  const int b = blockIdx.x / tiles_n, tile_n = blockIdx.x - b * tiles_n;
  const int hw = a.rows_per_batch, n_blk = tile_n * BN;
  const int c8 = tid % EC, row = tid / EC;
  const int n = n_blk + c8 * 8;
  for (int i = tid; i < 2 * GN_SLOTS * 2; i += blockDim.x) slots[i] = 0ull;
  const size_t slab = (size_t)a.M * a.N;
  for (int r0 = 0; r0 < hw; r0 += rows_pass) {
    const int m = b * hw + r0 + row;
    const float* src = a.workspace + (size_t)m * a.N + n;
    f32x4_t p0[8], p1[8];
#pragma unroll
    for (int s = 0; s < 8; ++s) {
      if (s < splits) {
        p0[s] = *reinterpret_cast<const f32x4_t*>(src + s * slab);
        p1[s] = *reinterpret_cast<const f32x4_t*>(src + s * slab + 4);
      } else {
        p0[s] = f32x4_t{0.f, 0.f, 0.f, 0.f};
        p1[s] = f32x4_t{0.f, 0.f, 0.f, 0.f};
      }
    }
    u32x4_t r1 = {0u, 0u, 0u, 0u}, r2 = {0u, 0u, 0u, 0u};
    if (a.res1) r1 = *reinterpret_cast<const u32x4_t*>((const uint16_t*)a.res1 + res1_row(a, m) * a.ldres1 + n);
    if (a.res2) r2 = *reinterpret_cast<const u32x4_t*>((const uint16_t*)a.res2 + (size_t)m * a.ldres2 + n);
    f32x4_t v0 = p0[0], v1 = p1[0];
#pragma unroll
    for (int s = 1; s < 8; ++s) { v0 += p0[s]; v1 += p1[s]; }
    if (a.bias) {
      v0 += *reinterpret_cast<const f32x4_t*>(a.bias + n);
      v1 += *reinterpret_cast<const f32x4_t*>(a.bias + n + 4);
    }
    if (a.rowvec) {
      const float* rv = a.rowvec + (size_t)b * a.ld_rowvec + n;
      v0 += *reinterpret_cast<const f32x4_t*>(rv);
      v1 += *reinterpret_cast<const f32x4_t*>(rv + 4);
    }
    v0 *= a.scale;
    v1 *= a.scale;
    v0[0] += E::lo(r1[0]) + E::lo(r2[0]); v0[1] += E::hi(r1[0]) + E::hi(r2[0]);
    v0[2] += E::lo(r1[1]) + E::lo(r2[1]); v0[3] += E::hi(r1[1]) + E::hi(r2[1]);
    v1[0] += E::lo(r1[2]) + E::lo(r2[2]); v1[1] += E::hi(r1[2]) + E::hi(r2[2]);
    v1[2] += E::lo(r1[3]) + E::lo(r2[3]); v1[3] += E::hi(r1[3]) + E::hi(r2[3]);
    u32x4_t o;
    o[0] = E::pack2(v0[0], v0[1]); o[1] = E::pack2(v0[2], v0[3]);
    o[2] = E::pack2(v1[0], v1[1]); o[3] = E::pack2(v1[2], v1[3]);
    *reinterpret_cast<u32x4_t*>((uint16_t*)a.out + (size_t)m * a.ldo + n) = o;
    *reinterpret_cast<u32x4_t*>(vals + ((size_t)(r0 + row) * BN + c8 * 8) * 2) = o;
    *reinterpret_cast<f32x4_t*>(&tile[row][c8 * 8]) = f32x4_t{E::lo(o[0]), E::hi(o[0]), E::lo(o[1]), E::hi(o[1])};
    *reinterpret_cast<f32x4_t*>(&tile[row][c8 * 8 + 4]) = f32x4_t{E::lo(o[2]), E::hi(o[2]), E::lo(o[3]), E::hi(o[3])};
    __syncthreads();
    if (tid < (rows_pass >> 4) * BN) {
      const int blk = tid / BN, col = tid - blk * BN;
      float sm = 0.f, sq = 0.f;
#pragma unroll
      for (int r = 0; r < 16; ++r) {
        const float v = tile[blk * 16 + r][col];
        sm += v;
        sq += v * v;
      }
      gn_column(a, slots, n_blk, col, sm, sq);
    }
    __syncthreads();
  }
  if (tid < BN) {
    const int k = a.gn_next_sub, cg = a.gn_cg[k], cbase = a.gn_c0[k] + n_blk;
    const int gl = (cbase + tid) / cg - cbase / cg;
    const double s = (double)(long long)slots[(k * GN_SLOTS + gl) * 2] * (1.0 / (double)PP_GN_SUM_SCALE);
    const double q = (double)(long long)slots[(k * GN_SLOTS + gl) * 2 + 1] * (1.0 / (double)PP_GN_SQ_SCALE);
    const double cnt = (double)hw * (double)cg;
    const double mean = s / cnt;
    double var = q / cnt - mean * mean;
    if (var < 0.0) var = 0.0;
    const float meanf = (float)mean, rstdf = (float)(1.0 / sqrt(var + (double)a.gn_next_eps));
    const float sc = rstdf * a.gn_next_gamma[n_blk + tid];
    sc_s[tid] = sc;
    sh_s[tid] = a.gn_next_beta[n_blk + tid] - meanf * sc;
  }
  __syncthreads();
  gn_flush(a, slots, b * hw, n_blk, BN, tid);
  const f32x4_t a0 = *reinterpret_cast<const f32x4_t*>(sc_s + c8 * 8), a1 = *reinterpret_cast<const f32x4_t*>(sc_s + c8 * 8 + 4);
  const f32x4_t b0 = *reinterpret_cast<const f32x4_t*>(sh_s + c8 * 8), b1 = *reinterpret_cast<const f32x4_t*>(sh_s + c8 * 8 + 4);
  const bool silu = a.gn_next_silu != 0;
  for (int r0 = 0; r0 < hw; r0 += rows_pass) {
    const int m = b * hw + r0 + row;
    const u32x4_t v = *reinterpret_cast<const u32x4_t*>(vals + ((size_t)(r0 + row) * BN + c8 * 8) * 2);
    float r[8];
    r[0] = E::lo(v[0]) * a0[0] + b0[0]; r[1] = E::hi(v[0]) * a0[1] + b0[1];
    r[2] = E::lo(v[1]) * a0[2] + b0[2]; r[3] = E::hi(v[1]) * a0[3] + b0[3];
    r[4] = E::lo(v[2]) * a1[0] + b1[0]; r[5] = E::hi(v[2]) * a1[1] + b1[1];
    r[6] = E::lo(v[3]) * a1[2] + b1[2]; r[7] = E::hi(v[3]) * a1[3] + b1[3];
    if (silu) {
#pragma unroll
      for (int j = 0; j < 8; ++j) r[j] = silu_fast_f(r[j]);
    }
    u32x4_t o;
    o[0] = E::pack2(r[0], r[1]); o[1] = E::pack2(r[2], r[3]);
    o[2] = E::pack2(r[4], r[5]); o[3] = E::pack2(r[6], r[7]);
    *reinterpret_cast<u32x4_t*>((uint16_t*)a.gn_next_out + (size_t)m * a.N + n) = o;
  }
}

bool reduce_lean_ok(const PPGemmArgs& a) {
  return a.act == PP_ACT_NONE && !a.out_f32 && !a.out_vt && !a.ln_stats && a.ldo % 8 == 0 &&
         (!a.res1 || a.ldres1 % 8 == 0) && (!a.res2 || a.ldres2 % 8 == 0);
}

#define PP_TILE_FORMS(X)                                                                                         \
  X(PP_TILE_128x160, 128, 2, 2, false, false)                                                                    \
  X(PP_TILE_64x160, 64, 2, 2, false, false)                                                                      \
  X(PP_TILE_256x160, 256, 4, 2, false, false)                                                                    \
  X(21, 128, 2, 2, false, true)                                                                                  \
  X(31, 128, 2, 3, false, true)                                                                                  \
  X(22, 64, 2, 2, false, true)                                                                                   \
  X(32, 64, 2, 3, false, true)                                                                                   \
  X(42, 64, 2, 4, false, true)                                                                                   \
  X(62, 64, 2, 5, false, true)                                        \
  X(23, 256, 4, 2, false, true)                                                                                  \
  X(33, 256, 4, 3, false, true)                                                                                  \
  X(24, 128, 4, 2, false, true)    \
  X(53, 256, 4, 3, true, true)                                    \
  X(44, 128, 4, 3, true, true)                                                                                   \
  X(54, 128, 4, 4, true, true)

struct TileForm {
  int id, bm;
  bool pp, v2;
};
#define PP_ROW(ID, BM_, WM_, NS_, PP_, V2_) {ID, BM_, PP_, V2_},
constexpr TileForm TILE_FORMS[] = {PP_TILE_FORMS(PP_ROW)};
#undef PP_ROW
const TileForm* tile_form(int id) {
  for (const TileForm& t : TILE_FORMS)
    if (t.id == id) return &t;
  return nullptr;
}

struct Choice {
  int tile, splitk;
};
bool gemm_pingpong();
bool gemm_n_major();

bool v2_ok(const PPGemmArgs& a) {
  if (a.N % 8) return false;
  if (a.act == PP_ACT_GEGLU && (a.N % 16 || a.ldo % 8)) return false;
  if (a.out_f32 ? (a.ldo % 4) : (a.ldo % 8)) return false;
  if (a.res1 && a.ldres1 % 8) return false;
  if (a.res2 && a.ldres2 % 8) return false;
  if (a.out_vt && (a.vt_col0 % 160 || a.res1 || a.res2 || a.rowvec)) return false;
  return true;
}

Choice choose(const PPGemmArgs& a) {
  if (a.w_batch_stride > 0 || a.act == PP_ACT_SOFTMAX80) return Choice{32, 1};
  Choice c{a.tile, a.splitk};
  const int tn = (a.N + 159) / 160;
  auto blocks = [&](int bm) { return ((a.M + bm - 1) / bm) * tn; };
  const bool conv = a.x_mode == PP_X_CONV3X3;
  const int nb256 = blocks(256), nb128 = blocks(128), nb64 = blocks(64), kt = a.K / 64;
  if (c.tile == PP_TILE_AUTO) {
    int sk = 1;
    if (!v2_ok(a)) {
      c.tile = (nb128 >= 256) ? PP_TILE_128x160 : PP_TILE_64x160;
      while (blocks(c.tile == PP_TILE_128x160 ? 128 : 64) * sk < 224 && kt / (sk * 2) >= 12 && sk < 8) sk *= 2;
    } else if (nb128 >= 512) {
      c.tile = (kt >= 20 && nb256 >= 256) ? 33 : 24;
    } else if (nb128 >= 256) {
      if (conv && kt > 140) { c.tile = 33; sk = 2; }
      else c.tile = a.out_vt ? 21 : 31;
    } else if (a.K <= 2880) {
      c.tile = 32;
      while (nb64 * sk < 128 && kt / (sk * 2) >= 24 && sk < 8) sk *= 2;
    } else if (nb64 >= 256 && kt <= 100) {
      if (kt >= 80 && nb128 * 2 >= 256 && !conv && !a.row_stats_out && !a.out_vt && a.act == PP_ACT_NONE) { c.tile = 31; sk = 2; }
      else c.tile = 32;
    } else if (nb256 >= 32) {
      c.tile = 33;
      while (nb256 * sk < 256 && sk < 8) sk *= 2;
    } else {
      c.tile = 31;
      while (nb128 * sk < 256 && kt / (sk * 2) >= 4 && sk < 8) sk *= 2;
    }
    if (c.splitk <= 0) c.splitk = sk;
    if (gemm_pingpong()) {
      const bool lnf = a.x_mode == PP_X_PLAIN && (a.ln_stats || a.row_stats_out || a.act == PP_ACT_GEGLU);
      if (c.tile == 31) c.tile = 54;
      else if (c.tile == 33 && !lnf) c.tile = 53;
    }
  }
  if (c.splitk <= 0) {
    const int tb = c.tile % 10;
    const int bm = tb == PP_TILE_128x160 ? 128 : tb == PP_TILE_64x160 ? 64 : 256;
    int sk = 1;
    while (blocks(bm) * sk < 192 && kt / (sk * 2) >= 16 && sk < 8) sk *= 2;
    c.splitk = sk;
  }
  if (a.N % 8) c.splitk = 1;
  if (a.row_stats_out) c.splitk = 1;
  return c;
}

bool gn_next_shape_ok(const PPGemmArgs& a, int sub) {
  if (sub < 0 || sub > 1 || !a.gn_acc[sub] || a.gn_c0[sub] != 0 || a.gn_cg[sub] < 8 || 40 % a.gn_cg[sub]) return false;
  if (a.gn_cg[sub] * a.gn_groups[sub] != a.N || a.N % 40 || !reduce_lean_ok(a)) return false;
  const int o = 1 - sub;
  if (a.gn_acc[o] && (a.gn_cg[o] < 8)) return false;
  const int hw = a.rows_per_batch;
  return hw >= 16 && hw <= 256 && hw % 16 == 0 && (hw <= 128 || hw % 128 == 0) && a.M % hw == 0 && a.ldo == a.N;
}

bool fused_combine_shape_ok(const PPGemmArgs& a, int bm, int tiles, int splitk, bool pp_tile, bool with_consumers, bool advice) {
  if (!(splitk == 2 || splitk == 4 || splitk == 8) || !pp_tile || !reduce_lean_ok(a)) return false;
  if (tiles % 8) return false;
  if (bm % splitk || bm / splitk < 16) return false;
  static const int max_splits = pp_lab_env("PP_FUSED_COMBINE_SPLITS", 4);
  if (advice && (splitk > max_splits || tiles * splitk > pp_cu_count())) return false;
  if (a.M % bm || a.N % 8) return false;
  if ((uint64_t)splitk * (uint64_t)a.M * (uint64_t)a.N * 4u >= 0x80000000ull) return false;
  if (a.rowvec && (a.rows_per_batch <= 0 || a.rows_per_batch % 64)) return false;
  if (!with_consumers) return true;
  if ((a.gn_acc[0] || a.gn_acc[1]) && (a.rows_per_batch <= 0 || a.rows_per_batch % 64)) return false;
  if (a.gn_next_out) {
    if (!gn_next_shape_ok(a, a.gn_next_sub)) return false;
    const int hw = a.rows_per_batch, cg = a.gn_cg[a.gn_next_sub];
    if (hw % 64 || bm % hw || 160 % cg) return false;
  }
  return true;
}

template <int EDT>
int launch_combine(const PPGemmArgs& a, int splitk, hipStream_t st) {
  const long long total = (long long)a.M * (a.N / 8);
  int nb = (int)((total + 255) / 256);
  if (nb > 4096) nb = 4096;
  if (a.gn_next_out && gn_next_shape_ok(a, a.gn_next_sub)) {
    if (!a.gn_next_gamma || !a.gn_next_beta) return PP_ERR_BAD_ARG;
    const int tn = a.N / 40;
    const int rows_pass = a.rows_per_batch < 128 ? a.rows_per_batch : 128;
    hipLaunchKernelGGL(pp_splitk_reduce_gn_apply_kernel<EDT>, dim3((a.M / a.rows_per_batch) * tn), dim3(rows_pass * 5), 0, st, a,
                       splitk, tn, rows_pass);
    PP_CHECK_LAUNCH("pp_splitk_reduce_gn_apply_kernel");
    return PP_OK;
  }
  if (a.gn_next_out) return PP_ERR_UNSUPPORTED;
  if (a.gn_acc[0] || a.gn_acc[1]) {
    const int tn = (a.N + 159) / 160;
    hipLaunchKernelGGL(pp_splitk_reduce_gn_kernel<EDT>, dim3(((a.M + 15) / 16) * tn), dim3(320), 0, st, a, splitk, tn);
  } else if (reduce_lean_ok(a)) hipLaunchKernelGGL((pp_splitk_reduce_kernel<true, EDT>), dim3(nb), dim3(256), 0, st, a, splitk);
  else hipLaunchKernelGGL((pp_splitk_reduce_kernel<false, EDT>), dim3(nb), dim3(256), 0, st, a, splitk);
  PP_CHECK_LAUNCH("pp_splitk_reduce_kernel");
  return PP_OK;
}

GemmDerived derive(const PPGemmArgs& a, int bm, int bn, int splitk) {
  GemmDerived d;
  d.tiles_m = (a.M + bm - 1) / bm;
  d.tiles_n = (a.N + bn - 1) / bn;
  d.kt_total = a.K / 64;
  d.kt_per_split = (d.kt_total + splitk - 1) / splitk;
  d.ctiles = (a.c1 + a.c2) / 64;
  d.n_major = (gemm_n_major() && d.tiles_m < d.tiles_n && d.tiles_m <= 8) ? 1 : 0;
  return d;
}

template <int BM, int BN, int WM, int WN, int XMODE, int EDT>
int launch(const PPGemmArgs& a, int splitk, hipStream_t st) {
  constexpr int T = WM * WN * 64;
  constexpr int LDS = 2 * (BM + BN) * 128;
  auto kern = pp_gemm_kernel<BM, BN, WM, WN, XMODE, EDT>;
  if (pp_func_lds(reinterpret_cast<const void*>(kern), LDS, "hipFuncSetAttribute(gemm)") != PP_OK) return PP_ERR_LAUNCH;
  const GemmDerived d = derive(a, BM, BN, splitk);
  dim3 grid(d.tiles_m * d.tiles_n, splitk, 1);
  hipLaunchKernelGGL(kern, grid, dim3(T), LDS, st, a, d);
  PP_CHECK_LAUNCH("pp_gemm_kernel");
  if (splitk > 1) return launch_combine<EDT>(a, splitk, st);
  return PP_OK;
}

bool gemm_n_major() {
  static const int v = pp_lab_env("PP_GEMM_NMAJOR", 1);
  return v != 0;
}

bool gemm_pingpong() {
  static const int v = pp_lab_env("PP_GEMM_PP", 1);
  return v != 0;
}

bool gemm_dma_interleave() {
  static const int v = pp_lab_env("PP_GEMM_DMAI", 1);
  return v != 0;
}

template <int BM, int BN, int WM, int WN, int XMODE, int NS, int EPI, bool PP, int EDT>
int launch2(const PPGemmArgs& a, int splitk, hipStream_t st) {
  if constexpr (EPI == 0) {
    if ((a.gn_acc[0] || a.gn_acc[1]) && splitk == 1) return launch2<BM, BN, WM, WN, XMODE, NS, 4, PP, EDT>(a, splitk, st);
  }
  if constexpr (XMODE == PP_X_PLAIN && EPI == 0) {
    if (a.act == PP_ACT_SOFTMAX80) {
      if constexpr (BM == 64 && NS == 3 && !PP) return launch2<BM, BN, WM, WN, XMODE, NS, 5, PP, EDT>(a, splitk, st);
      else return PP_ERR_UNSUPPORTED;
    }
    if (a.act == PP_ACT_GEGLU && splitk == 1) return launch2<BM, BN, WM, WN, XMODE, NS, 2, PP, EDT>(a, splitk, st);
    if (a.ln_stats || a.row_stats_out) return launch2<BM, BN, WM, WN, XMODE, NS, 1, PP, EDT>(a, splitk, st);
  }
  constexpr bool LNF = EPI == 1 || EPI == 2 || EPI == 5;
  constexpr int T = WM * WN * 64;
  constexpr int LDS = NS * (BM + BN) * 128 + (LNF ? 2048 + BM * 32 : 0);
  static_assert(LDS <= 160 * 1024 || (LNF && NS > 2), "LDS budget");
  if constexpr (LDS > 160 * 1024) {
    return launch2<BM, BN, WM, WN, XMODE, 2, EPI, false, EDT>(a, splitk, st);
  } else {
#ifdef PP_LAB
  auto kern = pp_gemm_kernel_v2<BM, BN, WM, WN, XMODE, NS, EPI, false, PP, EDT>;
  if constexpr (NS >= 3 && !PP) {
    if (gemm_dma_interleave()) kern = pp_gemm_kernel_v2<BM, BN, WM, WN, XMODE, NS, EPI, true, false, EDT>;
  }
#else
  auto kern = pp_gemm_kernel_v2<BM, BN, WM, WN, XMODE, NS, EPI, (NS >= 3 && !PP), PP, EDT>;
#endif
  if (pp_func_lds(reinterpret_cast<const void*>(kern), LDS, "hipFuncSetAttribute(gemm v2)") != PP_OK) return PP_ERR_LAUNCH;
  const GemmDerived d = derive(a, BM, BN, splitk);
  dim3 grid(d.tiles_m * d.tiles_n, splitk, 1);
  hipLaunchKernelGGL(kern, grid, dim3(T), LDS, st, a, d);
  PP_CHECK_LAUNCH("pp_gemm_kernel_v2");
  if (splitk > 1 && !a.tile_ctr) return launch_combine<EDT>(a, splitk, st);
  return PP_OK;
  }
}

bool gn_stats_supported(const PPGemmArgs& a) {
  if (a.act != PP_ACT_NONE || a.out_f32 || a.out_vt || a.ln_stats || a.row_stats_out) return false;
  if (!v2_ok(a) || !reduce_lean_ok(a)) return false;
  if (a.rows_per_batch <= 0 || a.rows_per_batch % 64) return false;
  for (int k = 0; k < 2; ++k)
    if (a.gn_acc[k] && (a.gn_cg[k] < 8 || a.gn_groups[k] <= 0 || a.gn_c0[k] < 0)) return false;
  return true;
}

int validate(const PPGemmArgs& a) {
  if (a.M <= 0 || a.N <= 0 || a.K <= 0 || !pp_dt_ok(a.dtype)) return PP_ERR_BAD_ARG;
  if (a.K % 64 != 0 || a.N % 4 != 0) return PP_ERR_BAD_ARG;
  if (!a.x1 || !a.w || !a.out) return PP_ERR_BAD_ARG;
  if (a.x_mode == PP_X_PLAIN) {
    if (a.subpix) return PP_ERR_BAD_ARG;
    if (a.c1 + a.c2 != a.K) return PP_ERR_BAD_ARG;
    if (a.c2 > 0 && (!a.x2 || a.c1 % 64 != 0)) return PP_ERR_BAD_ARG;
    if (a.ldx1 % 8 != 0 || (a.c2 > 0 && a.ldx2 % 8 != 0)) return PP_ERR_BAD_ARG;
    if ((uint64_t)a.M * (uint64_t)a.ldx1 * 2u >= 0x80000000ull) return PP_ERR_UNSUPPORTED;
  } else if (a.x_mode == PP_X_CONV3X3) {
    if (a.c1 % 64 != 0 || a.c2 % 64 != 0 || a.c1 <= 0) return PP_ERR_BAD_ARG;
    if (a.c2 > 0 && !a.x2) return PP_ERR_BAD_ARG;
    if (a.c3 < 0 || a.c4 < 0 || a.c3 % 64 || a.c4 % 64 || (a.c3 > 0 && !a.x3) || (a.c4 > 0 && (!a.x4 || a.c3 == 0)))
      return PP_ERR_BAD_ARG;
    if ((a.c3 > 0) && (a.stride != 1 || a.up)) return PP_ERR_UNSUPPORTED;
    if (a.subpix != 0 && a.subpix != 1) return PP_ERR_BAD_ARG;
    if (a.subpix && (a.up || a.stride != 1)) return PP_ERR_BAD_ARG;
    if (a.K != (a.subpix ? 4 : 9) * (a.c1 + a.c2) + a.c3 + a.c4) return PP_ERR_BAD_ARG;
    if (a.stride != 1 && a.stride != 2) return PP_ERR_BAD_ARG;
    if (a.M != a.batch * a.hout * a.wout) return PP_ERR_BAD_ARG;
    const int hv = a.up ? 2 * a.hin : a.hin, wv = a.up ? 2 * a.win : a.win;
    if (a.up && a.stride == 1) {
      if ((a.hout != hv && a.hout != hv - 1) || (a.wout != wv && a.wout != wv - 1) || a.hout <= 0 || a.wout <= 0) return PP_ERR_BAD_ARG;
    } else if (a.hout != (hv + 2 - 3) / a.stride + 1 || a.wout != (wv + 2 - 3) / a.stride + 1) {
      return PP_ERR_BAD_ARG;
    }
    if ((uint64_t)a.batch * a.hin * a.win * (uint64_t)(a.c1 > a.c2 ? a.c1 : a.c2) * 2u >= 0x80000000ull)
      return PP_ERR_UNSUPPORTED;
  } else {
    return PP_ERR_BAD_ARG;
  }
  if ((uint64_t)a.N * (uint64_t)a.K * 2u >= 0x80000000ull) return PP_ERR_UNSUPPORTED;
  if ((a.rowvec || a.out_vt) && a.rows_per_batch <= 0) return PP_ERR_BAD_ARG;
  if (a.act == PP_ACT_GEGLU && (a.out_f32 || a.out_vt || a.x_mode != PP_X_PLAIN)) return PP_ERR_BAD_ARG;
  if (a.w_batch_stride < 0 || a.vec_batch_stride < 0) return PP_ERR_BAD_ARG;
  if (a.w_batch_stride > 0) {
    if (a.x_mode != PP_X_PLAIN || a.rows_per_batch <= 0 || a.rows_per_batch % 64 || a.M % a.rows_per_batch || (a.w_batch_stride & 7))
      return PP_ERR_BAD_ARG;
    if (a.out_vt || a.out_f32 || a.act == PP_ACT_GEGLU || a.splitk > 1 || !v2_ok(a)) return PP_ERR_UNSUPPORTED;
  }
  if (a.vec_batch_stride > 0 && (a.act != PP_ACT_SOFTMAX80 || a.w_batch_stride <= 0 || (a.vec_batch_stride & 3))) return PP_ERR_UNSUPPORTED;
  if (a.act == PP_ACT_SOFTMAX80) {
    if (a.x_mode != PP_X_PLAIN || a.N % 80 || a.ldo % 8 || a.ldo < a.N) return PP_ERR_BAD_ARG;
    if (a.out_f32 || a.out_vt || a.res1 || a.res2 || a.rowvec || a.row_stats_out || a.gn_acc[0] || a.gn_acc[1] ||
        a.gn_next_out || a.out_dup_rows > 0 || a.splitk > 1 || a.scale != 1.0f || !v2_ok(a))
      return PP_ERR_UNSUPPORTED;
  }
  if (a.out_vt && a.vt_col0 % 4 != 0) return PP_ERR_BAD_ARG;
  if (a.ln_stats && (!a.ln_colsum || a.ln_tiles <= 0 || a.ln_dim <= 0)) return PP_ERR_BAD_ARG;
  if (a.row_stats_out && (a.out_f32 || a.out_vt || a.act == PP_ACT_GEGLU || !v2_ok(a))) return PP_ERR_UNSUPPORTED;
  if ((a.gn_acc[0] || a.gn_acc[1]) && !gn_stats_supported(a)) return PP_ERR_UNSUPPORTED;
  if ((a.gn_in_acc || a.gn_in_gb) && a.x_mode != PP_X_CONV3X3) return PP_ERR_UNSUPPORTED;
  if ((a.gn_in_acc != nullptr) != (a.gn_in_gb != nullptr)) return PP_ERR_BAD_ARG;
  if (a.res1_wrap_rows < 0 || a.out_dup_rows < 0 || a.gn_dup_batch < 0 || (a.gn_dup_mask & ~3)) return PP_ERR_BAD_ARG;
  if (a.res1_wrap_rows > 0 && (!a.res1 || a.M > 2 * a.res1_wrap_rows || a.res1_wrap_rows % 64)) return PP_ERR_BAD_ARG;
  if (a.out_dup_rows > 0) {
    if (a.out_dup_rows < a.M) return PP_ERR_BAD_ARG;
    if (a.out_f32 || a.out_vt || a.act == PP_ACT_GEGLU || a.row_stats_out || a.ln_stats || a.gn_next_out || a.gn_in_acc ||
        !v2_ok(a))
      return PP_ERR_UNSUPPORTED;
  }
  if (a.gn_dup_mask) {
    if (a.out_dup_rows <= 0 || a.gn_dup_batch <= 0 || a.rows_per_batch <= 0 ||
        a.gn_dup_batch * a.rows_per_batch != a.out_dup_rows)
      return PP_ERR_BAD_ARG;
    for (int k = 0; k < 2; ++k)
      if ((a.gn_dup_mask >> k & 1) && !a.gn_acc[k]) return PP_ERR_BAD_ARG;
  }
  return PP_OK;
}

enum class Family { V1, V2, HALO };
struct LaunchForm {
  Family family;
  int tile;
  int bm, tiles;
  int splitk;
  bool pp_tile;
  bool staged_epilogue() const { return family != Family::V1; }
};

int resolve_form(const PPGemmArgs& a, LaunchForm* f) {
  const int tn = (a.N + 159) / 160;
  CGChoice cg;
  const int halo = pp_conv_gn_form(a, &cg);
  if (halo < 0) return halo;
  if (halo) {
    *f = LaunchForm{Family::HALO, 0, cg.bm, (a.M / cg.bm) * tn * (a.subpix ? 4 : 1), cg.splitk, true};
    return PP_OK;
  }
  const Choice c = choose(a);
  const TileForm* t = tile_form(c.tile);
  if (!t) return PP_ERR_BAD_ARG;
  *f = LaunchForm{t->v2 ? Family::V2 : Family::V1, t->id, t->bm, ((a.M + t->bm - 1) / t->bm) * tn, c.splitk, t->pp};
  return PP_OK;
}

bool gn_next_ok(const PPGemmArgs& a, const LaunchForm& f, int sub) {
  return f.staged_epilogue() && f.splitk > 1 && gn_next_shape_ok(a, sub);
}

bool combine_fusable(const PPGemmArgs& a, const LaunchForm& f, bool with_consumers, bool advice) {
  return f.staged_epilogue() && fused_combine_shape_ok(a, f.bm, f.tiles, f.splitk, f.pp_tile, with_consumers, advice);
}

template <bool V2, int BM, int WM, int NS, bool PP, int XMODE, int EDT>
int launch_tile(const PPGemmArgs& a, int splitk, hipStream_t st) {
  if constexpr (V2) return launch2<BM, 160, WM, 2, XMODE, NS, 0, PP, EDT>(a, splitk, st);
  else return launch<BM, 160, WM, 2, XMODE, EDT>(a, splitk, st);
}

template <int EDT>
int dispatch(const PPGemmArgs& a, const LaunchForm& f, hipStream_t st) {
  const bool conv = a.x_mode == PP_X_CONV3X3;
  switch (f.tile) {
#define PP_CASE(ID, BM_, WM_, NS_, PP_, V2_)                                                         \
    case ID:                                                                                         \
      return conv ? launch_tile<V2_, BM_, WM_, NS_, PP_, PP_X_CONV3X3, EDT>(a, f.splitk, st)         \
                  : launch_tile<V2_, BM_, WM_, NS_, PP_, PP_X_PLAIN, EDT>(a, f.splitk, st);
    PP_TILE_FORMS(PP_CASE)
#undef PP_CASE
    default:
      return PP_ERR_BAD_ARG;
  }
}

}

static bool query_form(const PPGemmArgs* args, LaunchForm* f) {
  return args && validate(*args) == PP_OK && resolve_form(*args, f) == PP_OK;
}

extern "C" int pp_gemm_gn_stats_ok(const PPGemmArgs* args) {
  if (!args) return 0;
  PPGemmArgs a = *args;
  a.gn_acc[0] = a.gn_acc[1] = nullptr;
  a.gn_dup_mask = 0;
  LaunchForm f;
  return (query_form(&a, &f) && gn_stats_supported(a) && f.staged_epilogue()) ? 1 : 0;
}

extern "C" int pp_gemm_gn_next_ok(const PPGemmArgs* args, int sub) {
  LaunchForm f;
  return (query_form(args, &f) && gn_next_ok(*args, f, sub)) ? 1 : 0;
}

extern "C" size_t pp_gemm_combine_ctr_bytes(const PPGemmArgs* args) {
  LaunchForm f;
  if (!query_form(args, &f) || !combine_fusable(*args, f, false, true)) return 0;
  if (!pp_xcd_placement_ok()) return 0;
  return (size_t)f.tiles * FC_CTR_BYTES;
}

static bool combine_fused(const PPGemmArgs& a, const LaunchForm& f) { return a.tile_ctr && combine_fusable(a, f, true, false); }

extern "C" int pp_gemm_combine_fused(const PPGemmArgs* args) {
  LaunchForm f;
  return (query_form(args, &f) && combine_fused(*args, f)) ? 1 : 0;
}

extern "C" size_t pp_gemm_workspace_bytes(const PPGemmArgs* args) {
  LaunchForm f;
  if (!query_form(args, &f) || f.splitk <= 1) return 0;
  const size_t scratch = combine_fusable(*args, f, false, false) ? (size_t)f.tiles * FC_SCR_BYTES : 0;
  return (size_t)f.splitk * args->M * args->N * sizeof(float) + scratch;
}

extern "C" int pp_gemm_bf16(const PPGemmArgs* args, void* stream) {
  if (!args) return PP_ERR_BAD_ARG;
  const int v = validate(*args);
  if (v != PP_OK) return v;
  LaunchForm f;
  const int rf = resolve_form(*args, &f);
  if (rf != PP_OK) return rf;
  PPGemmArgs a_ = *args;
  const bool fused = combine_fused(a_, f);
  if (!fused) a_.tile_ctr = nullptr;
  const PPGemmArgs& a = a_;
  hipStream_t st = (hipStream_t)stream;
  if (a.gn_next_out && !gn_next_ok(a, f, a.gn_next_sub)) return PP_ERR_UNSUPPORTED;
  if (f.family == Family::HALO) {
    if ((a.gn_acc[0] || a.gn_acc[1]) && !gn_stats_supported(a)) return PP_ERR_UNSUPPORTED;
    const int rc = pp_conv_gn_run(a, CGChoice{f.bm, f.splitk}, st);
    if (rc != PP_OK || f.splitk == 1 || fused) return rc;
    return a.dtype == PP_DT_F16 ? launch_combine<PP_DT_F16>(a, f.splitk, st) : launch_combine<PP_DT_BF16>(a, f.splitk, st);
  }
  if (f.splitk > 1 && !a.workspace) return PP_ERR_WORKSPACE;
  if (f.family == Family::V2 && !v2_ok(a)) return PP_ERR_BAD_ARG;
  if (a.out_dup_rows > 0 && (!f.staged_epilogue() || f.splitk > 1)) return PP_ERR_UNSUPPORTED;
  if ((a.row_stats_out || a.gn_acc[0] || a.gn_acc[1] || (a.x_mode == PP_X_CONV3X3 && a.c3 > 0)) && !f.staged_epilogue())
    return PP_ERR_UNSUPPORTED;
  return a.dtype == PP_DT_F16 ? dispatch<PP_DT_F16>(a, f, st) : dispatch<PP_DT_BF16>(a, f, st);
}
```

### powerpaint_amd/csrc/pp_api.cpp

```cpp
#include <hip/hip_runtime.h>
#include <stdio.h>

#include <map>
#include <mutex>
#include <utility>

#include "pp_hip.h"

static thread_local char g_err[256] = "";

void pp_set_last_error(const char* what, hipError_t e) {
  snprintf(g_err, sizeof(g_err), "%s: %s", what, hipGetErrorString(e));
}

int pp_func_lds(const void* kern, int bytes, const char* what) {
  static std::mutex mu;
  static std::map<std::pair<const void*, int>, int> granted;
  int dev = 0;
  if (hipGetDevice(&dev) != hipSuccess) dev = 0;
  std::lock_guard<std::mutex> g(mu);
  int& have = granted[std::make_pair(kern, dev)];
  if (bytes <= have) return PP_OK;
  if (hipFuncSetAttribute(kern, hipFuncAttributeMaxDynamicSharedMemorySize, bytes) != hipSuccess) {
    pp_set_last_error(what, hipGetLastError());
    return PP_ERR_LAUNCH;
  }
  have = bytes;
  return PP_OK;
}

int pp_cu_count() {
  static std::mutex mu;
  static std::map<int, int> cus;
  int dev = 0;
  if (hipGetDevice(&dev) != hipSuccess) return 256;
  std::lock_guard<std::mutex> g(mu);
  auto it = cus.find(dev);
  if (it != cus.end()) return it->second;
  int n = 0;
  if (hipDeviceGetAttribute(&n, hipDeviceAttributeMultiprocessorCount, dev) != hipSuccess || n <= 0) n = 256;
  cus[dev] = n;
  return n;
}

__global__ void __launch_bounds__(64) pp_xcc_probe_kernel(unsigned* out) {
  if (threadIdx.x == 0) {
    unsigned v;
    asm volatile("s_getreg_b32 %0, hwreg(HW_REG_XCC_ID)" : "=s"(v));
    out[blockIdx.y * gridDim.x + blockIdx.x] = v & 7u;
  }
}

extern "C" int pp_xcd_placement_ok(void) {
  static std::mutex mu;
  static std::map<int, int> verdict;
  int dev = 0;
  if (hipGetDevice(&dev) != hipSuccess) return 0;
  std::lock_guard<std::mutex> g(mu);
  auto it = verdict.find(dev);
  if (it != verdict.end()) return it->second;
  int ok = 1;
  const int shapes[2][2] = {{64, 4}, {32, 8}};
  unsigned* d = nullptr;
  if (hipMalloc(&d, 256 * sizeof(unsigned)) != hipSuccess) return 0;
  for (int sh = 0; sh < 2 && ok; ++sh) {
    const int X = shapes[sh][0], Y = shapes[sh][1];
    unsigned h[256];
    if (hipMemset(d, 0xff, sizeof(h)) != hipSuccess) { ok = 0; break; }
    hipLaunchKernelGGL(pp_xcc_probe_kernel, dim3(X, Y), dim3(64), 0, 0, d);
    if (hipGetLastError() != hipSuccess || hipDeviceSynchronize() != hipSuccess ||
        hipMemcpy(h, d, sizeof(h), hipMemcpyDeviceToHost) != hipSuccess) { ok = 0; break; }
    int map[8] = {-1, -1, -1, -1, -1, -1, -1, -1};
    for (int f = 0; f < X * Y; ++f) {
      if (h[f] > 7u) ok = 0;
      else if (map[f & 7] < 0) map[f & 7] = (int)h[f];
      else if (map[f & 7] != (int)h[f]) ok = 0;
    }
    for (int i = 0; i < 8 && ok; ++i)
      for (int j = i + 1; j < 8; ++j)
        if (map[i] == map[j]) ok = 0;
  }
  (void)hipFree(d);
  verdict[dev] = ok;
  return ok;
}

#ifndef PP_BUILD_ID
#define PP_BUILD_ID "unknown"
#endif
extern "C" int pp_abi_version(void) { return PP_ABI_VERSION; }
extern "C" const char* pp_build_id(void) { return PP_BUILD_ID; }
extern "C" const char* pp_last_error(void) { return g_err; }
```

### powerpaint_amd/csrc/pp_common.h

```cpp
#pragma once
#include <hip/hip_runtime.h>
#include <stdint.h>
#include <stdlib.h>

#include "pp_hip.h"

typedef __attribute__((ext_vector_type(8))) __bf16 bf16x8_t;
typedef __attribute__((ext_vector_type(4))) float f32x4_t;
typedef __attribute__((ext_vector_type(16))) float f32x16_t;
typedef __attribute__((ext_vector_type(4))) uint32_t u32x4_t;
typedef __attribute__((ext_vector_type(2))) uint32_t u32x2_t;

#define PP_DEVINL __device__ __forceinline__

PP_DEVINL float bf2f(uint16_t v) { return __uint_as_float(((uint32_t)v) << 16); }
PP_DEVINL uint16_t f2bf(float f) {
  __bf16 b = (__bf16)f;
  return __builtin_bit_cast(uint16_t, b);
}
typedef __attribute__((ext_vector_type(2))) float f32x2_t;
typedef __attribute__((ext_vector_type(2))) __bf16 bf16x2_t;
PP_DEVINL uint32_t pack2bf(float lo, float hi) {
  const f32x2_t v = {lo, hi};
  return __builtin_bit_cast(uint32_t, __builtin_convertvector(v, bf16x2_t));
}
PP_DEVINL float bflo(uint32_t u) { return __uint_as_float(u << 16); }
PP_DEVINL float bfhi(uint32_t u) { return __uint_as_float(u & 0xffff0000u); }

typedef __attribute__((ext_vector_type(8))) _Float16 f16x8_t;
typedef __attribute__((ext_vector_type(2))) _Float16 f16x2_t;
template <int DT>
struct E16;
template <>
struct E16<PP_DT_BF16> {
  typedef bf16x8_t v8;
  static PP_DEVINL float to_f(uint16_t v) { return bf2f(v); }
  static PP_DEVINL uint16_t from_f(float f) { return f2bf(f); }
  static PP_DEVINL float lo(uint32_t u) { return bflo(u); }
  static PP_DEVINL float hi(uint32_t u) { return bfhi(u); }
  static PP_DEVINL uint32_t pack2(float lo, float hi) { return pack2bf(lo, hi); }
  static PP_DEVINL f32x4_t mfma16(v8 a, v8 b, f32x4_t c) { return __builtin_amdgcn_mfma_f32_16x16x32_bf16(a, b, c, 0, 0, 0); }
  static PP_DEVINL f32x16_t mfma32(v8 a, v8 b, f32x16_t c) { return __builtin_amdgcn_mfma_f32_32x32x16_bf16(a, b, c, 0, 0, 0); }
  static PP_DEVINL f32x16_t mfma32(v8 a, v8 b, f32x16_t c, int, int, int) { return mfma32(a, b, c); }
  static PP_DEVINL f32x4_t mfma16(v8 a, v8 b, f32x4_t c, int, int, int) { return mfma16(a, b, c); }
};
template <>
struct E16<PP_DT_F16> {
  typedef f16x8_t v8;
  static PP_DEVINL float to_f(uint16_t v) { return (float)__builtin_bit_cast(_Float16, v); }
  static PP_DEVINL uint16_t from_f(float f) { return __builtin_bit_cast(uint16_t, (_Float16)f); }
  static PP_DEVINL float lo(uint32_t u) { return to_f((uint16_t)(u & 0xffffu)); }
  static PP_DEVINL float hi(uint32_t u) { return to_f((uint16_t)(u >> 16)); }
  static PP_DEVINL uint32_t pack2(float lo, float hi) {
    const f32x2_t v = {lo, hi};
    return __builtin_bit_cast(uint32_t, __builtin_convertvector(v, f16x2_t));
  }
  static PP_DEVINL f32x4_t mfma16(v8 a, v8 b, f32x4_t c) { return __builtin_amdgcn_mfma_f32_16x16x32_f16(a, b, c, 0, 0, 0); }
  static PP_DEVINL f32x16_t mfma32(v8 a, v8 b, f32x16_t c) { return __builtin_amdgcn_mfma_f32_32x32x16_f16(a, b, c, 0, 0, 0); }
  static PP_DEVINL f32x16_t mfma32(v8 a, v8 b, f32x16_t c, int, int, int) { return mfma32(a, b, c); }
  static PP_DEVINL f32x4_t mfma16(v8 a, v8 b, f32x4_t c, int, int, int) { return mfma16(a, b, c); }
};
#define PP_DT_SWITCH(DTV, ...)                    \
  do {                                            \
    if ((DTV) == PP_DT_F16) {                     \
      constexpr int EDT = PP_DT_F16;               \
      __VA_ARGS__;                                \
    } else {                                      \
      constexpr int EDT = PP_DT_BF16;             \
      __VA_ARGS__;                                \
    }                                             \
  } while (0)
inline bool pp_dt_ok(int dt) { return dt == PP_DT_BF16 || dt == PP_DT_F16; }

PP_DEVINL float silu_f(float x) { return x / (1.0f + __expf(-x)); }
PP_DEVINL float silu_fast_f(float x) { return x * __builtin_amdgcn_rcpf(1.0f + __builtin_amdgcn_exp2f(x * -1.44269504088896340736f)); }
PP_DEVINL float gelu_erf_f(float x) { return 0.5f * x * (1.0f + erff(x * 0.70710678118654752440f)); }
PP_DEVINL float gelu_fast_f(float x) {
  const float ax = __builtin_fabsf(x);
  const float t = __builtin_amdgcn_rcpf(__builtin_fmaf(ax, 0.3275911f * 0.70710678118654752440f, 1.0f));
  float p = __builtin_fmaf(t, 0.5f * 1.061405429f, 0.5f * -1.453152027f);
  p = __builtin_fmaf(t, p, 0.5f * 1.421413741f);
  p = __builtin_fmaf(t, p, 0.5f * -0.284496736f);
  p = __builtin_fmaf(t, p, 0.5f * 0.254829592f);
  const float q = p * t * __builtin_amdgcn_exp2f(x * x * (-0.5f * 1.44269504088896340736f));
  return __builtin_fmaf(-ax, q, __builtin_fmaxf(x, 0.f));
}

PP_DEVINL __amdgpu_buffer_rsrc_t make_rsrc(const void* base, uint32_t bytes) {
  return __builtin_amdgcn_make_buffer_rsrc(const_cast<void*>(base), 0, bytes, 0x00020000);
}
#define PP_OOB 0x80000000u

PP_DEVINL float wave_sum(float v) {
#pragma unroll
  for (int o = 32; o > 0; o >>= 1) v += __shfl_xor(v, o, 64);
  return v;
}
PP_DEVINL float wave_max(float v) {
#pragma unroll
  for (int o = 32; o > 0; o >>= 1) v = fmaxf(v, __shfl_xor(v, o, 64));
  return v;
}

#ifdef PP_LAB
inline int pp_lab_env(const char* name, int dflt) {
  const char* e = getenv(name);
  return e ? atoi(e) : dflt;
}
#else
constexpr int pp_lab_env(const char*, int dflt) { return dflt; }
#endif

void pp_set_last_error(const char* what, hipError_t e);
int pp_func_lds(const void* kern, int bytes, const char* what);
int pp_cu_count();
struct CGChoice {
  int bm, splitk;
};
int pp_conv_gn_form(const PPGemmArgs& a, CGChoice* c);
int pp_conv_gn_run(const PPGemmArgs& a, const CGChoice& c, hipStream_t st);
#define PP_CHECK_LAUNCH(what)                         \
  do {                                                \
    hipError_t e__ = hipGetLastError();               \
    if (e__ != hipSuccess) {                          \
      pp_set_last_error(what, e__);                   \
      return PP_ERR_LAUNCH;                           \
    }                                                 \
  } while (0)
```

### powerpaint_amd/engine.py

```python
import ctypes as C
import enum
import os
from dataclasses import dataclass
from typing import Dict, List, NamedTuple, Optional, Sequence, Tuple

import torch

from . import _lib as L

ALIGN = 256


def _align(x: int, a: int = ALIGN) -> int:
    return (x + a - 1) // a * a


def _lab_switch(name: str) -> bool:
    return not (os.environ.get("PP_LAB") == "1" and os.environ.get(name, "1") == "0")


GN_STATS_IN_EPILOGUE = _lab_switch("PP_GN_EPILOGUE")
GN_NEXT_IN_COMBINE = _lab_switch("PP_GN_NEXT")
FUSE_GN_CONV = _lab_switch("PP_FUSE_GN_CONV")
TWIN_PREFIX = _lab_switch("PP_TWIN")
# ... 50 lines not shown
            for s in shape:
                n *= s
            return typed[off // esize: off // esize + n].view(*shape)
        return torch.as_strided(typed, tuple(shape), tuple(strides), off // esize)


class ParamPack:

    def __init__(self):
        self.items: List[Tuple[str, torch.Tensor]] = []
        self.offsets: Dict[str, int] = {}
        self.shapes: Dict[str, Tuple[torch.Size, torch.dtype]] = {}
        self.total = 0
        self.buf = None
        self.ptr: Dict[str, int] = {}
        self.version = 0

    def touch(self):
        self.version += 1

    def add(self, name: str, t: torch.Tensor, dtype: torch.dtype):
        assert name not in self.offsets, name
        t = t.detach().to(dtype).contiguous()
        off = _align(self.total)
        self.offsets[name] = off
        self.shapes[name] = (t.shape, dtype)
        self.total = off + t.numel() * t.element_size()
        self.items.append((name, t))

    def to_device(self, device, materialize: bool = True):
        self.buf = torch.zeros(_align(self.total) + ALIGN, dtype=torch.uint8, device=device)
        skew = (-self.buf.data_ptr()) % ALIGN
        self.buf = self.buf[skew:skew + _align(self.total)]
        base = self.buf.data_ptr()
        for name, t in self.items:
            off = self.offsets[name]
            if materialize and t.device.type != "meta":
                nb = t.numel() * t.element_size()
                self.buf[off:off + nb].copy_(t.view(-1).view(torch.uint8))
            self.ptr[name] = base + off
        self.items = []
        return self

    def regrow(self, keep: int):
        old = self.buf
        self.total = max(self.total, keep)
        buf = torch.zeros(_align(self.total) + ALIGN, dtype=torch.uint8, device=old.device)
        skew = (-buf.data_ptr()) % ALIGN
        buf = buf[skew:skew + _align(self.total)]
        buf[:keep].copy_(old[:keep])
        for name, t in self.items:
            off, nb = self.offsets[name], t.numel() * t.element_size()
            buf[off:off + nb].copy_(t.view(-1).view(torch.uint8))
        self.items = []
        self.buf = buf
        base = buf.data_ptr()
        self.ptr.clear()
        self.ptr.update({name: base + off for name, off in self.offsets.items()})
        self.touch()

    def forget(self, prefix: str, keep: int):
        for name in [n for n in self.offsets if n.startswith(prefix)]:
            assert self.offsets[name] >= keep, name
            del self.offsets[name], self.shapes[name]
            self.ptr.pop(name, None)
        self.total = keep

    def tensor(self, name: str) -> torch.Tensor:
        shape, dtype = self.shapes[name]
        off = self.offsets[name]
        n = 1
        for s in shape:
            n *= s
        es = torch.empty((), dtype=dtype).element_size()
        return self.buf[off:off + n * es].view(dtype).view(shape)


@dataclass
class Act:
    ptr: int
    B: int
    H: int
    W: int
    C: int
    producer: object = None
    dup_half: int = 0
    gn_filled: object = None

    @property
    def rows(self) -> int:
        return self.B * self.H * self.W

    @property
    def nbytes(self) -> int:
        return self.rows * self.C * 2


class Plan:

    def __init__(self):
        self.calls: List[Tuple] = []
        self.keep: List = []
        self.flops = 0.0
        self.flops_by_kind: Dict[str, float] = {}
        self.flops_skipped = 0.0

    def add(self, name: str, fn, *args):
        self.calls.append((fn, args, name))

    def count(self, kind: str, flops: float):
        self.flops += flops
        self.flops_by_kind[kind] = self.flops_by_kind.get(kind, 0.0) + flops

    def skip(self, flops: float):
        self.flops += flops
        self.flops_skipped += flops

    @property
    def flops_executed(self) -> float:
        return self.flops - self.flops_skipped

    def run(self, stream: int):
        for fn, args, name in self.calls:
            rc = fn(*args, stream)
            if rc != 0:
                L.check(rc, name)

    def run_timed(self, stream_obj) -> Dict[str, float]:
        evs = []
        s = stream_obj.cuda_stream
        for fn, args, name in self.calls:
            e0 = torch.cuda.Event(enable_timing=True)
            e1 = torch.cuda.Event(enable_timing=True)
            e0.record(stream_obj)
            rc = fn(*args, s)
            e1.record(stream_obj)
            if rc != 0:
                L.check(rc, name)
            evs.append((name, e0, e1))
        stream_obj.synchronize()
        out: Dict[str, float] = {}
        self.last_launch_ms = []
        for name, e0, e1 in evs:
            dt = e0.elapsed_time(e1)
            out[name] = out.get(name, 0.0) + dt
            self.last_launch_ms.append(dt)
        return out

    def describe(self, i: int) -> str:
        fn, args, name = self.calls[i]
        a = getattr(args[0], "_obj", None) if args else None
        if isinstance(a, L.PPGemmArgs):
            return (f"{name} M={a.M} N={a.N} K={a.K} {'conv' if a.x_mode else 'lin'}"
                    f"{' s2' if a.stride == 2 else ''}{' up' if a.up else ''}{' cat' if a.c2 else ''}")
        return name


class Builder:

    def __init__(self, arena: Arena, plan: Optional[Plan] = None, dtype: torch.dtype = torch.bfloat16):
        self.arena = arena
        self.plan = plan or Plan()
        self.lib = L.lib()
        self.dtype = dtype
        self.dt = L.dtype_code(dtype)
        self.gemm_tile = 0
        self.gemm_splitk = 0
        self.last_gemm = None
        self.gn_acc_base = 0
        self.gn_acc_cap = 0
        self.gn_acc_used = 0
        self.fault_ptr = 0

    def alloc(self, nbytes: int) -> int:
        return self.arena.alloc(nbytes)

    def new_act(self, B, H, W, Cc) -> Act:
        return Act(self.alloc(B * H * W * Cc * 2), B, H, W, Cc)

    def mark(self):
        return self.arena.mark()

    def release(self, m):
        self.arena.release(m)

    def _gemm(self, a: L.PPGemmArgs, name: str):
        if a.tile == 0:
            a.tile = self.gemm_tile
        if a.splitk == 0:
            a.splitk = self.gemm_splitk
        a.dtype = self.dt
        ws = self.lib.pp_gemm_workspace_bytes(C.byref(a))
        if ws:
            a.workspace = self.alloc(ws)
            if FUSED_COMBINE and self.gn_acc_cap:
                nctr = _align(self.lib.pp_gemm_combine_ctr_bytes(C.byref(a)), 8)
                if nctr and self.gn_acc_used + nctr <= self.gn_acc_cap:
                    a.tile_ctr = self.gn_acc_base + self.gn_acc_used
                    a.combine_fault = self.fault_ptr or None
                    self.gn_acc_used += nctr
        self.plan.keep.append(a)
        self.last_gemm = a
        a._arena_top = self.arena.off
        self.plan.add(name, self.lib.pp_gemm_bf16, C.byref(a))
        if a.subpix:
            self.plan.count(name, 4 * 2.0 * a.M * a.N * a.K)
            self.plan.skip(5 * 2.0 * a.M * a.N * a.K)
        else:
            self.plan.count(name, 2.0 * a.M * a.N * a.K)

    def linear(self, x: int, rows: int, K: int, w: int, N: int, bias: int = 0, ldx: Optional[int] = None,
               x2: int = 0, K2: int = 0, ldx2: int = 0, res1: int = 0, ldres1: int = 0, res2: int = 0,
               ldres2: int = 0, scale: float = 1.0, act: int = 0, out: int = 0, ldo: Optional[int] = None,
               rowvec: int = 0, ld_rowvec: int = 0, rows_per_batch: int = 0, out_vt: int = 0, vt_col0: int = 0,
               vt_ld: int = 0, out_f32: bool = False, row_stats_out: int = 0, ln_stats: int = 0, ln_colsum: int = 0,
               ln_tiles: int = 0, ln_dim: int = 0, ln_eps: float = 1e-5, name: str = "gemm", res1_wrap: int = 0,
               w_batch_stride: int = 0, vec_batch_stride: int = 0) -> int:
        n_out = N // 2 if act == L.PP_ACT_GEGLU else (vt_col0 if out_vt else N)
        if ldo is None:
            ldo = n_out
        if not out:
            out = self.alloc(rows * ldo * (4 if out_f32 else 2))
        m = self.mark()
        a = L.gemm_args(self.dt, rows, N, K, x, w, out, x2=x2, K2=K2, ldx=ldx, ldx2=ldx2, ldo=ldo, ldres1=ldres1, ldres2=ldres2,
                        rows_per_batch=rows_per_batch, scale=scale)
        a.bias, a.rowvec, a.ld_rowvec, a.res1, a.res2 = bias or None, rowvec or None, ld_rowvec, res1 or None, res2 or None
        a.w_batch_stride, a.vec_batch_stride, a.res1_wrap_rows = w_batch_stride, vec_batch_stride, res1_wrap
        a.act, a.out_f32 = act, int(out_f32)
        a.out_vt, a.vt_col0, a.vt_ld = out_vt or None, vt_col0, vt_ld
        a.row_stats_out = row_stats_out or None
        if ln_stats:
            a.ln_stats, a.ln_colsum, a.ln_tiles, a.ln_dim, a.ln_eps = ln_stats, ln_colsum, ln_tiles, ln_dim, ln_eps
        self._gemm(a, name)
        self.release(m)
        return out

    def conv3x3(self, x: Act, w: int, cout: int, bias: int = 0, stride: int = 1, up: bool = False,
                x2: Optional[Act] = None, rowvec: int = 0, res1: int = 0, res2: int = 0, scale: float = 1.0,
                out: Optional[Act] = None, x3: Optional[Act] = None, x4: Optional[Act] = None,
                name: str = "conv3x3", gn_in: Optional[Tuple[int, int, int, float, int]] = None, dup: bool = False,
                up_size: Optional[Tuple[int, int]] = None) -> Act:
        if gn_in is not None:
            gamma, beta, gb, eps, groups = gn_in
            acc = self._subscribe_gn_stats(x, x2, groups) if FUSE_GN_CONV else 0
            fused = None
            if acc:
                fused = (acc, gb, groups, eps)
            else:
                x, x2 = self.groupnorm(x, gamma, beta, eps, True, x2=x2, groups=groups), None
        else:
            fused = None
        c2 = x2.C if x2 is not None else 0
        ptr = lambda t: t.ptr if t is not None else None
        a = L.conv3x3_args(self.dt, x.B, x.H, x.W, x.C, cout, x.ptr, ptr(x2), c2, ptr(x3), x3.C if x3 is not None else 0,
                           ptr(x4), x4.C if x4 is not None else 0, stride, up, w=w, scale=scale, up_size=up_size)
        ho, wo = a.hout, a.wout
        if dup:
            assert out is None and gn_in is None
            out = self.new_act(2 * x.B, ho, wo, cout)
            out.dup_half = x.B
        if out is None:
            out = self.new_act(x.B, ho, wo, cout)
        m = self.mark()
        a.out, a.bias, a.rowvec, a.res1, a.res2 = out.ptr, bias or None, rowvec or None, res1 or None, res2 or None
        if dup:
            a.out_dup_rows = a.M
            if self.lib.pp_gemm_workspace_bytes(C.byref(a)):
                raise L.PPError("twin-prefix conv would run split-K; the caller must not request dup for this shape")
        if fused is not None:
            a.gn_in_acc, a.gn_in_gb, a.gn_in_groups, a.gn_in_eps, a.gn_in_silu = fused[0], fused[1], fused[2], fused[3], 1
            if not self.lib.pp_conv_gn_preferred(C.byref(a)):
                a.gn_in_acc, a.gn_in_gb, a.gn_in_groups, a.gn_in_silu = None, None, 0, 0
                gamma, beta, gb, eps, groups = gn_in
                self.release(m)
                xn = self._apply_in_producer_combine(x, fused[0], gamma, beta, eps, True, None) if x2 is None else None
                if xn is None:
                    xn = self.new_act(x.B, x.H, x.W, x.C + c2)
                    self.plan.add("groupnorm_apply", self.lib.pp_groupnorm_apply_acc, x.ptr, x.C,
                                  x2.ptr if x2 is not None else None, c2, x.B, x.H * x.W, groups, eps, gamma, beta, fused[0],
                                  1, xn.ptr, self.dt)
                m = self.mark()
                a.x1, a.x2, a.c1, a.c2 = xn.ptr, None, x.C + c2, 0
        self._gemm(a, name)
        out.producer = a
        self.release(m)
        return out

    def conv3x3_up_subpix(self, x: Act, wfold: int, cout: int, bias: int = 0, res2: int = 0, name: str = "conv3x3") -> Act:
        a = L.conv3x3_args(self.dt, x.B, x.H, x.W, x.C, cout, x.ptr, w=wfold)
        a.K, a.subpix = 4 * x.C, 1
        out = self.new_act(x.B, 2 * x.H, 2 * x.W, cout)
        a.out, a.bias, a.res2 = out.ptr, bias or None, res2 or None
        self._gemm(a, name)
        out.producer = a
        return out

    def groupnorm(self, x: Act, gamma: int, beta: int, eps: float, silu: bool, x2: Optional[Act] = None,
                  groups: int = 32, out: Optional[Act] = None) -> Act:
        c2 = x2.C if x2 is not None else 0
        Ct = x.C + c2
        hw = x.H * x.W
        out_given = out
        x2p = x2.ptr if x2 is not None else None
        acc = self._subscribe_gn_stats(x, x2, groups)
        if acc and x2 is None:
            fused = self._apply_in_producer_combine(x, acc, gamma, beta, eps, silu, out_given)
            if fused is not None:
# ... 1132 lines not shown
```

### powerpaint_amd/ops.py

```python
import ctypes as C
from typing import Optional

import torch

from . import _lib as L

_DT = {torch.float32: 0, torch.bfloat16: 1, torch.float16: 2}


def _s():
    return torch.cuda.current_stream().cuda_stream


def _p(t: Optional[torch.Tensor]):
    return t.data_ptr() if t is not None else None


def _set_gn(a, gn, rows_per_batch):
    if not gn:
        return
    a.rows_per_batch = rows_per_batch
    for k, (acc, cg, c0, groups) in enumerate(gn):
        a.gn_acc[k], a.gn_cg[k], a.gn_c0[k], a.gn_groups[k] = acc.data_ptr(), cg, c0, groups


last_combine = {"fused": False, "ctr": None}
_fault_words = {}


def _fault_word(device) -> torch.Tensor:
    key = torch.device(device)
    if key not in _fault_words:
        _fault_words[key] = torch.zeros(1, dtype=torch.int32, device=device)
    return _fault_words[key]


def combine_faults(device) -> int:
    return int(_fault_word(device).item())


def _attach_combine(a, device, enable):
    last_combine["fused"], last_combine["ctr"] = False, None
    if enable is None or enable is False:
        return
    bound = ((a.M + 127) // 128) * ((a.N + 159) // 160) * 16
    if torch.is_tensor(enable):
        ctr = enable
        assert ctr.dtype == torch.int64 and ctr.numel() * 8 >= bound
    else:
        n = L.lib().pp_gemm_combine_ctr_bytes(C.byref(a))
        if enable == "force":
            n = max(n, bound)
        if not n:
            return
        ctr = torch.zeros(n // 8, dtype=torch.int64, device=device)
    a.tile_ctr, a.combine_fault = ctr.data_ptr(), _fault_word(device).data_ptr()
    last_combine["ctr"] = ctr
    last_combine["fused"] = bool(L.lib().pp_gemm_combine_fused(C.byref(a)))


def _norm_out(out, shape, like: torch.Tensor, what: str) -> torch.Tensor:
    if out is None:
        return torch.empty(*shape, dtype=like.dtype, device=like.device)
    if tuple(out.shape) != tuple(shape) or not out.is_contiguous() or out.dtype != like.dtype or out.device != like.device:
        raise L.PPError(f"{what}: `out` must be a contiguous {list(shape)} tensor of the inputs' format")
    return out


def _view2d(t, rows: int, cols: int, dtype, like: torch.Tensor, what: str) -> torch.Tensor:
    if (t.dim() != 2 or tuple(t.shape) != (rows, cols) or t.stride(1) != 1 or t.stride(0) < cols or t.dtype != dtype
            or t.device != like.device):
        raise L.PPError(f"{what}: must be a [{rows}, {cols}] row-major view (unit column stride) of the output format")
    return t


def _rows_in(t, cols: int, like: torch.Tensor, what: str) -> int:
    if t.dim() != 2 or t.shape[1] != cols or t.stride(1) != 1 or (t.shape[0] > 1 and t.stride(0) < cols) or t.dtype != like.dtype \
            or t.device != like.device:
        raise L.PPError(f"{what}: must be a [rows, {cols}] row-major view (unit column stride) of the inputs' format")
    return t.stride(0) if t.shape[0] > 1 else cols


def _exact(t, shape, dtype, like: torch.Tensor, what: str) -> torch.Tensor:
    if tuple(t.shape) != tuple(shape) or not t.is_contiguous() or t.dtype != dtype or t.device != like.device:
        raise L.PPError(f"{what}: must be a contiguous {list(shape)} tensor of {dtype}")
    return t


def _vt_window(t, nb: int, cols: int, rows: int, like: torch.Tensor, what: str) -> torch.Tensor:
    if (t.dim() != 3 or tuple(t.shape) != (nb, cols, rows) or t.stride(2) != 1 or t.dtype != like.dtype or t.device != like.device
            or t.stride(1) < rows or (nb > 1 and t.stride(0) != cols * t.stride(1))):
        raise L.PPError(f"{what}: must be a [{nb}, {cols}, {rows}] window of a contiguous [nb, cols, ld] buffer of the inputs' format")
    return t


def _nhwc_view(t, shape, like: torch.Tensor, what: str) -> torch.Tensor:
    B, H, W, Cc = shape
    bad = t.dim() != 4 or tuple(t.shape) != tuple(shape) or t.stride(3) != 1 or t.dtype != like.dtype or t.device != like.device
    if not bad:
        ld = t.stride(2) if W > 1 else (t.stride(1) if H > 1 else (t.stride(0) if B > 1 else Cc))
        bad = (ld < Cc or (W > 1 and H > 1 and t.stride(1) != W * ld) or (B > 1 and H * W > 1 and t.stride(0) != H * W * ld))
    if bad:
        raise L.PPError(f"{what}: must be a {list(shape)} NHWC view of the inputs' format with dense pixels (channel stride = ld)")
    return t


def _nhwc_ld(t, shape) -> int:
    B, H, W, Cc = shape
    return t.stride(2) if W > 1 else (t.stride(1) if H > 1 else (t.stride(0) if B > 1 else Cc))


def _res_ld(t, shape, like: torch.Tensor, what: str, rows_only: bool = False) -> int:
    if t is None:
        return shape[3]
    if t.dim() == 2:
        if t.shape[1] != shape[3] or t.stride(1) != 1 or t.dtype != like.dtype or t.device != like.device or \
                (not rows_only and t.shape[0] != shape[0] * shape[1] * shape[2]):
            raise L.PPError(f"{what}: must be [{shape[0] * shape[1] * shape[2]}, {shape[3]}] rows of the inputs' format")
        return t.stride(0) if t.shape[0] > 1 else shape[3]
    if rows_only:
        shape = tuple(t.shape[:3]) + (shape[3],) if t.dim() == 4 else shape
    _nhwc_view(t, shape, like, what)
    return _nhwc_ld(t, shape)


last_workspace = {"bytes": 0}


def _workspace(lib, a, device, workspace):
    ws = lib.pp_gemm_workspace_bytes(C.byref(a))
    last_workspace["bytes"] = ws
    if workspace is None:
        return torch.empty(max(ws, 4) // 4, dtype=torch.float32, device=device) if ws else None
    if (workspace.dtype != torch.float32 or not workspace.is_contiguous() or workspace.device != device
            or workspace.numel() * 4 < ws):
        raise L.PPError(f"`workspace` must be a contiguous fp32 tensor of at least {ws} bytes on the inputs' device")
    return workspace if ws else None


def groupnorm_apply_acc(x: torch.Tensor, acc: torch.Tensor, gamma, beta, eps: float, silu: bool, groups: int = 32,
                        x2=None, out: Optional[torch.Tensor] = None):
    B, H, W, C1 = x.shape
    C2 = x2.shape[3] if x2 is not None else 0
    y = _norm_out(out, (B, H, W, C1 + C2), x, "groupnorm_apply_acc")
    L.check(L.lib().pp_groupnorm_apply_acc(_p(x), C1, _p(x2), C2, B, H * W, groups, eps, _p(gamma), _p(beta), _p(acc),
                                           int(silu), _p(y), L.dtype_code(x.dtype), _s()), "pp_groupnorm_apply_acc")
    return y


def gemm(x: torch.Tensor, w: torch.Tensor, bias=None, x2=None, res1=None, res2=None, scale: float = 1.0, act: int = 0,
         rowvec=None, rows_per_batch: int = 0, out_f32: bool = False, vt_col0: int = 0, tile: int = 0,
         splitk: int = 0, row_stats: bool = False, ln_stats=None, ln_colsum=None, ln_dim: int = 0,
         ln_eps: float = 1e-5, gn=None, res1_wrap: int = 0, fuse_combine: bool = False, out=None, vt=None, stats=None,
         workspace=None):
    lib = L.lib()
    M, K1 = x.shape
    K2 = x2.shape[1] if x2 is not None else 0
    N = w.shape[-2]
    n_out = N // 2 if act == L.PP_ACT_GEGLU else (vt_col0 if vt_col0 else N)
    odt = torch.float32 if out_f32 else x.dtype
    if out is None:
        out = torch.empty(M, n_out, dtype=odt, device=x.device)
    else:
        _view2d(out, M, n_out, odt, x, "gemm: `out`")
    a = L.gemm_args(L.dtype_code(x.dtype), M, N, K1, _p(x), _p(w), _p(out), x2=_p(x2), K2=K2, ldx=x.stride(0),
                    ldx2=x2.stride(0) if x2 is not None else 0, ldo=out.stride(0) if M > 1 else n_out,
                    ldres1=res1.stride(0) if res1 is not None else 0,
                    ldres2=res2.stride(0) if res2 is not None else 0, rows_per_batch=rows_per_batch, scale=scale)
    if w.dim() == 3:
        a.w_batch_stride = w.stride(0)
        if bias is not None and bias.dim() == 2:
            a.vec_batch_stride = bias.stride(0)
    a.bias, a.rowvec, a.res1, a.res2 = _p(bias), _p(rowvec), _p(res1), _p(res2)
    a.ld_rowvec = rowvec.stride(0) if (rowvec is not None and rowvec.dim() == 2 and rowvec.shape[0] > 1) else 0
    a.res1_wrap_rows, a.act, a.out_f32 = res1_wrap, act, int(out_f32)
    if vt_col0:
        nb, ncols = M // rows_per_batch, N - vt_col0
        if vt is None:
            vt = torch.zeros(nb, ncols, rows_per_batch, dtype=x.dtype, device=x.device)
        elif (vt.dim() != 3 or tuple(vt.shape) != (nb, ncols, rows_per_batch) or vt.stride(2) != 1 or vt.dtype != x.dtype
              or vt.device != x.device or vt.stride(1) < rows_per_batch or vt.stride(0) != ncols * vt.stride(1)):
            raise L.PPError(f"gemm: `vt` must be a [{nb}, {ncols}, {rows_per_batch}] window of a contiguous [nb, cols, vt_ld] "
                            "buffer of the inputs' format")
        a.out_vt, a.vt_col0, a.vt_ld = _p(vt), vt_col0, vt.stride(1)
    elif vt is not None:
        raise L.PPError("gemm: `vt` without vt_col0")
    a.tile, a.splitk = tile, splitk
    _set_gn(a, gn, rows_per_batch)
    if row_stats:
        tn = (N + 159) // 160
        if stats is None:
            stats = torch.zeros(M, tn, 2, dtype=torch.float32, device=x.device)
        elif (tuple(stats.shape) != (M, tn, 2) or not stats.is_contiguous() or stats.dtype != torch.float32
              or stats.device != x.device):
            raise L.PPError(f"gemm: `stats` must be a contiguous [{M}, {tn}, 2] fp32 tensor")
        a.row_stats_out = _p(stats)
    elif stats is not None:
        raise L.PPError("gemm: `stats` without row_stats")
    if ln_stats is not None:
        a.ln_stats, a.ln_colsum, a.ln_tiles, a.ln_dim, a.ln_eps = _p(ln_stats), _p(ln_colsum), ln_stats.shape[1], ln_dim, ln_eps
    wsb = _workspace(lib, a, x.device, workspace)
    a.workspace = _p(wsb)
    _attach_combine(a, x.device, fuse_combine)
    L.check(lib.pp_gemm_bf16(C.byref(a), _s()), "pp_gemm_bf16")
    if row_stats:
        return out, stats
    return (out, vt) if vt_col0 else out


def gn_gamma_beta(gamma: torch.Tensor, beta: torch.Tensor) -> torch.Tensor:
    return torch.stack([gamma.float(), beta.float()], 1).contiguous()


def conv_gn_supported(x: torch.Tensor, cout: int, x2=None, x3=None, x4=None, groups: int = 32) -> bool:
    a = _conv_request(x, cout, 1, False, x2, x3, x4)
    a.gn_in_acc, a.gn_in_gb, a.gn_in_groups, a.gn_in_silu, a.gn_in_eps = 1, 1, groups, 1, 1e-5
    return bool(L.lib().pp_conv_gn_supported(C.byref(a)))


def conv_halo_routed(x: torch.Tensor, cout: int, x2=None, x3=None, x4=None, stride: int = 1, up: bool = False,
                     tile: int = 0, up_size=None) -> bool:
    a = _conv_request(x, cout, stride, up, x2, x3, x4, up_size)
    a.tile = tile
    return L.lib().pp_conv_gn_supported(C.byref(a)) == 2


def _conv_request(x, cout, stride, up, x2, x3, x4, up_size=None) -> L.PPGemmArgs:
    B, H, W, C1 = x.shape
    ch = lambda t: t.shape[3] if t is not None else 0
    return L.conv3x3_args(L.dtype_code(x.dtype), B, H, W, C1, cout, _p(x), _p(x2), ch(x2), _p(x3), ch(x3), _p(x4), ch(x4),
                          stride, up, up_size=up_size)


def conv3x3(x: torch.Tensor, w: torch.Tensor, bias=None, stride: int = 1, up: bool = False, x2=None, rowvec=None,
            res1=None, res2=None, scale: float = 1.0, tile: int = 0, splitk: int = 0, gn=None, x3=None, x4=None,
            gn_in=None, gn_next=None, dup: bool = False, gn_dup_mask: int = 0, res1_wrap: int = 0,
            fuse_combine: bool = False, out=None, workspace=None, ynext=None, up_size=None):
    lib = L.lib()
    B, C1, C2, cout = x.shape[0], x.shape[3], (x2.shape[3] if x2 is not None else 0), w.shape[0]
    a = _conv_request(x, cout, stride, up, x2, x3, x4, up_size)
    ho, wo = a.hout, a.wout
    oshape = (2 * B if dup else B, ho, wo, cout)
    if out is None:
        out = torch.empty(*oshape, dtype=x.dtype, device=x.device)
    else:
        a.ldo = _nhwc_ld(_nhwc_view(out, oshape, x, "conv3x3: `out`"), oshape)
    a.w, a.out, a.scale = _p(w), _p(out), scale
    a.bias, a.rowvec, a.res1, a.res2 = _p(bias), _p(rowvec), _p(res1), _p(res2)
    rshape = (B, ho, wo, cout)
    a.ldres1 = _res_ld(res1, rshape, x, "conv3x3: `res1`", rows_only=res1_wrap > 0)
    a.ldres2 = _res_ld(res2, rshape, x, "conv3x3: `res2`")
    if rowvec is not None and rowvec.dim() == 2 and rowvec.shape[0] > 1:
        a.ld_rowvec = rowvec.stride(0)
    a.res1_wrap_rows = res1_wrap
    if dup:
        a.out_dup_rows = a.M
        if gn_dup_mask:
            a.gn_dup_batch, a.gn_dup_mask = B, gn_dup_mask
    a.tile, a.splitk = tile, splitk
    _set_gn(a, gn, ho * wo)
    if gn_next is None and ynext is not None:
        raise L.PPError("conv3x3: `ynext` without gn_next")
    if gn_next is not None:
        g_, b_, eps_, silu_, sub_ = gn_next
        ynext = _norm_out(ynext, oshape, x, "conv3x3: `ynext`")
        a.gn_next_out, a.gn_next_gamma, a.gn_next_beta = _p(ynext), _p(g_), _p(b_)
        a.gn_next_eps, a.gn_next_silu, a.gn_next_sub = eps_, int(silu_), sub_
    if gn_in is not None:
        acc, gb, groups, eps = gn_in
        assert gb.dtype == torch.float32 and gb.shape == (C1 + C2, 2) and gb.is_contiguous()
        a.gn_in_acc, a.gn_in_gb, a.gn_in_groups, a.gn_in_silu, a.gn_in_eps = _p(acc), _p(gb), groups, 1, eps
    wsb = _workspace(lib, a, x.device, workspace)
    a.workspace = _p(wsb)
    if gn_next is not None and not lib.pp_gemm_gn_next_ok(C.byref(a), a.gn_next_sub):
        raise L.PPError("pp_gemm_gn_next_ok() = 0 for this launch (PP_ERR_UNSUPPORTED)")
    _attach_combine(a, x.device, fuse_combine)
    L.check(lib.pp_gemm_bf16(C.byref(a), _s()), "pp_gemm_bf16(conv)")
    return (out, ynext) if gn_next is not None else out


def upconv_fold(w: torch.Tensor) -> torch.Tensor:
    cout, cin = w.shape[0], w.shape[1] // 9
    assert w.is_contiguous() and w.shape[1] == 9 * cin
    out = torch.empty(4, cout, 4 * cin, dtype=w.dtype, device=w.device)
    L.check(L.lib().pp_upconv_fold(_p(w), cout, cin, L.dtype_code(w.dtype), _p(out), _s()), "pp_upconv_fold")
    return out


def upconv_subpix_supported(x: torch.Tensor, cout: int) -> int:
    B, H, W, C1 = x.shape
    return int(L.lib().pp_upconv_subpix_supported(B, H, W, C1, cout, L.dtype_code(x.dtype)))


def conv3x3_up_subpix(x: torch.Tensor, wfold: torch.Tensor, bias=None, rowvec=None, res1=None, res2=None, scale: float = 1.0,
                      tile: int = 0, splitk: int = 0, gn=None, out=None, workspace=None):
    B, H, W, C1 = x.shape
    cout = wfold.shape[1]
    assert tuple(wfold.shape) == (4, cout, 4 * C1) and wfold.is_contiguous()
    a = L.conv3x3_args(L.dtype_code(x.dtype), B, H, W, C1, cout, _p(x))
    a.K, a.subpix = 4 * C1, 1
    if out is None:
        out = torch.empty(B, 2 * H, 2 * W, cout, dtype=x.dtype, device=x.device)
    else:
        a.ldo = _nhwc_ld(_nhwc_view(out, (B, 2 * H, 2 * W, cout), x, "conv3x3_up_subpix: `out`"), (B, 2 * H, 2 * W, cout))
    a.w, a.out, a.scale = _p(wfold), _p(out), scale
    a.bias, a.rowvec, a.res1, a.res2 = _p(bias), _p(rowvec), _p(res1), _p(res2)
    a.ldres1 = _res_ld(res1, (B, 2 * H, 2 * W, cout), x, "conv3x3_up_subpix: `res1`")
    a.ldres2 = _res_ld(res2, (B, 2 * H, 2 * W, cout), x, "conv3x3_up_subpix: `res2`")
    if rowvec is not None and rowvec.dim() == 2 and rowvec.shape[0] > 1:
        a.ld_rowvec = rowvec.stride(0)
    a.tile, a.splitk = tile, splitk
    _set_gn(a, gn, H * W)
    a.workspace = _p(_workspace(L.lib(), a, x.device, workspace))
    L.check(L.lib().pp_gemm_bf16(C.byref(a), _s()), "pp_gemm_bf16(sub-pixel upsampling conv)")
    return out


def groupnorm(x: torch.Tensor, gamma, beta, eps: float, silu: bool, groups: int = 32, x2=None,
              out: Optional[torch.Tensor] = None):
    lib = L.lib()
    B, H, W, C1 = x.shape
    C2 = x2.shape[3] if x2 is not None else 0
    Ct = C1 + C2
    ws = torch.empty(lib.pp_groupnorm_workspace_bytes(B, H * W, Ct) // 4, dtype=torch.float32, device=x.device)
    y = _norm_out(out, (B, H, W, Ct), x, "groupnorm")
    dt = L.dtype_code(x.dtype)
    L.check(lib.pp_groupnorm_stats(_p(x), C1, _p(x2), C2, B, H * W, groups, _p(ws), dt, _s()), "pp_groupnorm_stats")
    L.check(lib.pp_groupnorm_apply(_p(x), C1, _p(x2), C2, B, H * W, groups, eps, _p(gamma), _p(beta), _p(ws),
                                   int(silu), _p(y), dt, _s()), "pp_groupnorm_apply")
    return y


def layernorm(x: torch.Tensor, gamma, beta, eps: float = 1e-5, out: Optional[torch.Tensor] = None):
    rows, Cc = x.shape
    y = _norm_out(out, (rows, Cc), x, "layernorm")
    L.check(L.lib().pp_layernorm(_p(x), rows, Cc, _p(gamma), _p(beta), eps, _p(y), L.dtype_code(x.dtype), _s()),
            "pp_layernorm")
    return y


def transpose_v(v: torch.Tensor, batch: int, nk: int, ldvt: Optional[int] = None):
    cols = v.shape[1]
    ldvt = ldvt or (nk + 7) // 8 * 8
    vt = torch.empty(batch, cols, ldvt, dtype=v.dtype, device=v.device)
    L.check(L.lib().pp_transpose_v(_p(v), v.stride(0), batch, nk, cols, _p(vt), ldvt, _s()), "pp_transpose_v")
    return vt


def _attn_out(out, ldo, rows: int, cols: int, like: torch.Tensor) -> torch.Tensor:
    if out is None:
        return torch.empty(rows, ldo or cols, dtype=like.dtype, device=like.device)[:, :cols]
    if (tuple(out.shape) != (rows, cols) or out.stride(1) != 1 or out.dtype != like.dtype or out.device != like.device
            or (ldo is not None and ldo != out.stride(0))):
        raise L.PPError(f"attention: `out` must be a [{rows}, {cols}] row-major view of the inputs' format (row stride = ldo)")
    return out


def attention_small(q: torch.Tensor, k: torch.Tensor, v: torch.Tensor, batch: int, heads: int, nq: int, nk: int,
                    causal: bool = False, scale: Optional[float] = None, out: Optional[torch.Tensor] = None,
                    ldo: Optional[int] = None):
    d = 64
    o = _attn_out(out, ldo, batch * nq, heads * d, q)
    L.check(L.lib().pp_attention_small(_p(q), q.stride(0), _p(k), k.stride(0), _p(v), v.stride(0), _p(o), o.stride(0),
                                       batch, heads, nq, nk, d, scale if scale is not None else d ** -0.5, int(causal),
                                       L.dtype_code(q.dtype), _s()), "pp_attention_small")
    return o


def softmax_rows(s: torch.Tensor, scale: float = 1.0, dtype=torch.bfloat16):
    rows, n = s.shape
    p = torch.empty(rows, n, dtype=dtype, device=s.device)
    L.check(L.lib().pp_softmax_rows(_p(s), s.stride(0), rows, n, float(scale), _p(p), n, L.dtype_code(dtype), _s()),
            "pp_softmax_rows")
    return p


def attention(q: torch.Tensor, k: torch.Tensor, vt: torch.Tensor, batch: int, heads: int, nq: int, nk: int, d: int,
              scale: Optional[float] = None, variant: int = L.PP_ATTN_AUTO, out: Optional[torch.Tensor] = None,
              ldo: Optional[int] = None):
    o = _attn_out(out, ldo, batch * nq, heads * d, q)
    L.check(L.lib().pp_attention_fwd_variant(_p(q), q.stride(0), _p(k), k.stride(0), _p(vt), vt.stride(1), _p(o),
                                             o.stride(0), batch, heads, nq, nk, d,
                                             scale if scale is not None else d ** -0.5, L.dtype_code(q.dtype),
                                             int(variant), _s()), "pp_attention_fwd")
    return o


def xattn_fold(k: torch.Tensor, vt: torch.Tensor, batch: int, nctx: int, heads: int, wq: torch.Tensor, wo: torch.Tensor,
               q_colsum=None, q_bias=None, scale: Optional[float] = None, kperm=False, gt=None, gcs=None, gbias=None,
               ht=None):
    c = wq.shape[0]
    dev, dt = k.device, k.dtype
    if k.dim() != 2 or k.shape[0] != batch * nctx or k.shape[1] < c or k.stride(1) != 1 or (k.shape[0] > 1 and k.stride(0) < c):
        raise L.PPError(f"xattn_fold: `k` must be [{batch * nctx}, >= {c}] rows with unit column stride")
    if (vt.dim() != 3 or vt.shape[0] != batch or vt.shape[1] != c or vt.shape[2] < nctx or vt.stride(2) != 1 or vt.dtype != dt
            or vt.stride(1) < nctx or (batch > 1 and vt.stride(0) != c * vt.stride(1))):
        raise L.PPError(f"xattn_fold: `vt` must be a [{batch}, {c}, >= {nctx}] window of a contiguous [batch, c, ldvt] buffer")
    for w_, nm in ((wq, "wq"), (wo, "wo")):
        if tuple(w_.shape) != (c, c) or not w_.is_contiguous() or w_.dtype != dt:
            raise L.PPError(f"xattn_fold: `{nm}` must be a contiguous [{c}, {c}] matrix of the inputs' format")
    n = heads * 80
    gt = torch.empty(batch, n, c, dtype=dt, device=dev) if gt is None else _exact(gt, (batch, n, c), dt, k, "xattn_fold: `gt`")
    ht = torch.empty(batch, c, n, dtype=dt, device=dev) if ht is None else _exact(ht, (batch, c, n), dt, k, "xattn_fold: `ht`")
    gcs = torch.empty(batch, n, dtype=torch.float32, device=dev) if gcs is None else \
        _exact(gcs, (batch, n), torch.float32, k, "xattn_fold: `gcs`")
    gb = torch.empty(batch, n, dtype=torch.float32, device=dev) if gbias is None else \
        _exact(gbias, (batch, n), torch.float32, k, "xattn_fold: `gbias`")
    L.check(L.lib().pp_xattn_fold(_p(k), k.stride(0) if k.shape[0] > 1 else k.shape[1], _p(vt), vt.stride(1), batch, nctx, heads, c, _p(wq), _p(q_colsum),
                                  _p(q_bias), _p(wo), scale if scale is not None else (c // heads) ** -0.5, _p(gt),
                                  _p(gcs), _p(gb), _p(ht), int(kperm), L.dtype_code(dt), _s()), "pp_xattn_fold")
    return gt, gcs, gb, ht


def xattn_block(x: torch.Tensor, folded, bias_o=None, res=None, ln_stats=None, ln_eps: float = 1e-5,
                rows_per_batch: int = 0, row_stats=False, twin: bool = False, pre_w=None, pre_b=None,
                ln_fold: bool = False, out=None):
    gt, gcs, gb, ht = folded
    wrap = x.shape[0] if twin else 0
    M, c = x.shape[0] * (2 if twin else 1), x.shape[1]
    ldx = _rows_in(x, c, x, "xattn_block: `x`")
    ldres = _rows_in(res, c, x, "xattn_block: `res`") if res is not None else 0
    if res is not None and res.shape[0] != x.shape[0]:
        raise L.PPError("xattn_block: `res` must have the rows of `x`")
    nb = M // (rows_per_batch or M)
    _exact(gt, (nb, 640, c), x.dtype, x, "xattn_block: folded gt")
    _exact(ht, (nb, c, 640), x.dtype, x, "xattn_block: folded ht")
    _exact(gcs, (nb, 640), torch.float32, x, "xattn_block: folded gcs")
    _exact(gb, (nb, 640), torch.float32, x, "xattn_block: folded gbias")
    out = torch.empty(M, c, dtype=x.dtype, device=x.device) if out is None else _view2d(out, M, c, x.dtype, x, "xattn_block: `out`")
    if torch.is_tensor(row_stats):
        st = _exact(row_stats, (M, c // 160, 2), torch.float32, x, "xattn_block: `row_stats`")
        row_stats = True
    else:
        st = torch.zeros(M, c // 160, 2, dtype=torch.float32, device=x.device) if row_stats else None
    tiles = ln_stats.shape[1] if ln_stats is not None else (c // 160 if (pre_w is not None and ln_fold) else 0)
    L.check(L.lib().pp_xattn_block(_p(x), ldx, _p(res), ldres, _p(ln_stats),
                                   tiles, ln_eps, _p(gt), _p(gcs), _p(gb), _p(ht),
                                   _p(bias_o), _p(out), out.stride(0) if M > 1 else c, _p(st), M, c, rows_per_batch or M, wrap, _p(pre_w), _p(pre_b),
                                   L.dtype_code(x.dtype), _s()), "pp_xattn_block")
    return (out, st) if row_stats else out


def ff_fused(hs: torch.Tensor, w1: torch.Tensor, b1: torch.Tensor, w2kp: torch.Tensor, bias2=None, cs1=None, ln_stats=None,
             ln_eps: float = 1e-5, res1=None, res2=None, res1_wrap: int = 0, rows_per_batch: int = 0, gn=None,
             w2_kperm: bool = True, scale: float = 1.0, out=None):
    M, Cc = hs.shape
    ldx = _rows_in(hs, Cc, hs, "ff_fused: `hs`")
    ld1 = _rows_in(res1, Cc, hs, "ff_fused: `res1`") if res1 is not None else 0
    ld2 = _rows_in(res2, Cc, hs, "ff_fused: `res2`") if res2 is not None else 0
    if res1 is not None and res1.shape[0] != (res1_wrap or M):
        raise L.PPError(f"ff_fused: `res1` must have {res1_wrap or M} rows")
    if res2 is not None and res2.shape[0] != M:
        raise L.PPError(f"ff_fused: `res2` must have {M} rows")
    if tuple(w1.shape) != (8 * Cc, Cc) or not w1.is_contiguous() or tuple(w2kp.shape) != (Cc, 5 * Cc) or not w2kp.is_contiguous():
        raise L.PPError("ff_fused: `w1` / `w2kp` must be contiguous [2560, 320] / [320, 1600] matrices")
    out = torch.empty(M, Cc, dtype=hs.dtype, device=hs.device) if out is None else _view2d(out, M, Cc, hs.dtype, hs, "ff_fused: `out`")
    a = L.gemm_args(L.dtype_code(hs.dtype), M, Cc, 4 * Cc, _p(hs), _p(w2kp), _p(out), x2=_p(hs), K2=Cc, ldx2=ldx,
                    ldo=out.stride(0) if M > 1 else Cc, ldres1=ld1, ldres2=ld2, rows_per_batch=rows_per_batch, scale=scale)
    a.bias, a.res1, a.res2, a.res1_wrap_rows = _p(bias2), _p(res1), _p(res2), res1_wrap
    _set_gn(a, gn, rows_per_batch)
    L.check(L.lib().pp_ff_fused(C.byref(a), _p(w1), _p(b1), _p(cs1), _p(ln_stats),
                                ln_stats.shape[1] if ln_stats is not None else 0, ln_eps, int(w2_kperm), _s()), "pp_ff_fused")
    return out

# ... 98 lines not shown
```

Baseline: 9.175 images/s.

## Choose GEMM tile rasterization group size from an L2 reuse model

Replaces the binary n-major/m-major tile ordering with a grouped rasterization (group_m rows of tiles swept across N). A host-side model estimates the bytes each XCD's resident window of workgroups pulls from memory and picks the power-of-two group size that cuts traffic by at least a threshold versus the old heuristic. Choices are memoized per shape and can be overridden per call. The aim is better L2 reuse of the input panels and weight strips across concurrently running tiles. The cost is extra host-side logic at launch time and a heuristic that may pick orders that do not help.

```diff
diff --git a/include/pp_hip.h b/include/pp_hip.h
--- a/include/pp_hip.h
+++ b/include/pp_hip.h
@@ -92,6 +92,7 @@
   uint64_t* tile_ctr;
   uint32_t* combine_fault;
   int32_t subpix;
+  int32_t tile_group_m;
 } PPGemmArgs;
 #define PP_GN_SUM_SCALE 16777216.0f
 #define PP_GN_SQ_SCALE 1048576.0f
@@ -112,6 +113,7 @@
 int pp_gemm_gn_next_ok(const PPGemmArgs* args, int sub);
 size_t pp_gemm_combine_ctr_bytes(const PPGemmArgs* args);
 int pp_gemm_combine_fused(const PPGemmArgs* args);
+int pp_gemm_tile_group_m(const PPGemmArgs* args);
 int pp_xcd_placement_ok(void);
 
 int pp_linear_skinny(const float* x, int rows, int K, const void* w, const float* bias, int N, float* out, int ldo,
diff --git a/powerpaint_amd/_lib.py b/powerpaint_amd/_lib.py
--- a/powerpaint_amd/_lib.py
+++ b/powerpaint_amd/_lib.py
@@ -43,6 +43,7 @@
         ("gn_next_sub", i32), ("gn_dup_mask", i32), ("vec_batch_stride", i32),
         ("tile_ctr", vp), ("combine_fault", vp),
         ("subpix", i32),
+        ("tile_group_m", i32),
     ]
 
 
@@ -116,6 +117,7 @@
     "pp_upconv_fold": (C.c_int, [vp, C.c_int, C.c_int, C.c_int, vp, vp]),
     "pp_gemm_combine_ctr_bytes": (sz, [C.POINTER(PPGemmArgs)]),
     "pp_gemm_combine_fused": (C.c_int, [C.POINTER(PPGemmArgs)]),
+    "pp_gemm_tile_group_m": (C.c_int, [C.POINTER(PPGemmArgs)]),
     "pp_xcd_placement_ok": (C.c_int, []),
     "pp_groupnorm_apply_acc": (C.c_int, [vp, C.c_int, vp, C.c_int, C.c_int, C.c_int, C.c_int, f32, vp, vp, vp, C.c_int, vp,
                                          C.c_int, vp]),
diff --git a/powerpaint_amd/csrc/conv_gn.hip b/powerpaint_amd/csrc/conv_gn.hip
--- a/powerpaint_amd/csrc/conv_gn.hip
+++ b/powerpaint_amd/csrc/conv_gn.hip
@@ -25,7 +25,7 @@
 static_assert(CG_LDS <= 160 * 1024, "LDS budget");
 
 struct CGDerived {
-  int tiles_m, tiles_n, n_major;
+  int tiles_m, tiles_n, group_m;
   int nch1, nch;
   int ntail3, ntail;
   int hp;
@@ -74,13 +74,7 @@
   const int par = SUBPIX ? (lid & 3) : 0, pa = par >> 1, pb = par & 1;
   if constexpr (SUBPIX) lid >>= 2;
   int tile_m, tile_n;
-  if (d.n_major) {
-    tile_n = lid / d.tiles_m;
-    tile_m = lid - tile_n * d.tiles_m;
-  } else {
-    tile_m = lid / d.tiles_n;
-    tile_n = lid - tile_m * d.tiles_n;
-  }
+  pp_tile_decode(lid, d.tiles_m, d.tiles_n, d.group_m, &tile_m, &tile_n);
   const int m_blk = tile_m * BM, n_blk = tile_n * BN;
   const int split = blockIdx.y, splits = gridDim.y;
   const int ch_b = split * d.nch / splits, ch_e = (split + 1) * d.nch / splits;
@@ -736,13 +730,13 @@
 }
 
 template <int BM, int HPW, bool PP, int NMODE, int EDT>
-int cg_launch(const PPGemmArgs& a, int splitk, hipStream_t st) {
+int cg_launch(const PPGemmArgs& a, int splitk, int group_m, hipStream_t st) {
   auto kern = pp_conv_gn_kernel<BM, HPW, PP, NMODE, EDT>;
   if (pp_func_lds(reinterpret_cast<const void*>(kern), CG_LDS, "hipFuncSetAttribute(conv_gn)") != PP_OK) return PP_ERR_LAUNCH;
   CGDerived d;
   d.tiles_m = a.M / BM;
   d.tiles_n = (a.N + CG_BN - 1) / CG_BN;
-  d.n_major = (d.tiles_m < d.tiles_n && d.tiles_m <= 8) ? 1 : 0;
+  d.group_m = group_m < 1 ? 1 : group_m > d.tiles_m ? d.tiles_m : group_m;
   d.nch1 = a.c1 / 64;
   d.nch = (a.c1 + a.c2) / 64;
   d.ntail3 = a.c3 / 64;
@@ -756,18 +750,18 @@
 }
 
 template <int BM, bool PP, int NMODE, int EDT>
-int cg_launch_hpw(const PPGemmArgs& a, int splitk, hipStream_t st) {
+int cg_launch_hpw(const PPGemmArgs& a, int splitk, int group_m, hipStream_t st) {
   const int need = (BM + 2 * a.wout + 63) / 64;
   if constexpr (BM == 256) {
-    if (need <= 5) return cg_launch<256, 5, PP, NMODE, EDT>(a, splitk, st);
-    return cg_launch<256, 6, PP, NMODE, EDT>(a, splitk, st);
+    if (need <= 5) return cg_launch<256, 5, PP, NMODE, EDT>(a, splitk, group_m, st);
+    return cg_launch<256, 6, PP, NMODE, EDT>(a, splitk, group_m, st);
   } else if constexpr (BM == 128) {
-    if (need <= 3) return cg_launch<128, 3, PP, NMODE, EDT>(a, splitk, st);
-    if (need <= 4) return cg_launch<128, 4, PP, NMODE, EDT>(a, splitk, st);
-    return cg_launch<128, 6, PP, NMODE, EDT>(a, splitk, st);
+    if (need <= 3) return cg_launch<128, 3, PP, NMODE, EDT>(a, splitk, group_m, st);
+    if (need <= 4) return cg_launch<128, 4, PP, NMODE, EDT>(a, splitk, group_m, st);
+    return cg_launch<128, 6, PP, NMODE, EDT>(a, splitk, group_m, st);
   } else {
-    if (need <= 2) return cg_launch<64, 2, PP, NMODE, EDT>(a, splitk, st);
-    return cg_launch<64, 3, PP, NMODE, EDT>(a, splitk, st);
+    if (need <= 2) return cg_launch<64, 2, PP, NMODE, EDT>(a, splitk, group_m, st);
+    return cg_launch<64, 3, PP, NMODE, EDT>(a, splitk, group_m, st);
   }
 }
 
@@ -778,10 +772,10 @@
   if (!pp || nm != 1) {
 #define CG_CASE(BM_)                                                                        \
     case BM_:                                                                               \
-      if (!pp) return cg_launch_hpw<BM_, false, 1, EDT>(a, c.splitk, st);                   \
-      if (nm == 0) return cg_launch_hpw<BM_, true, 0, EDT>(a, c.splitk, st);                \
-      if (nm == 2) return cg_launch_hpw<BM_, true, 2, EDT>(a, c.splitk, st);                \
-      return cg_launch_hpw<BM_, true, 3, EDT>(a, c.splitk, st);
+      if (!pp) return cg_launch_hpw<BM_, false, 1, EDT>(a, c.splitk, c.group_m, st);                   \
+      if (nm == 0) return cg_launch_hpw<BM_, true, 0, EDT>(a, c.splitk, c.group_m, st);                \
+      if (nm == 2) return cg_launch_hpw<BM_, true, 2, EDT>(a, c.splitk, c.group_m, st);                \
+      return cg_launch_hpw<BM_, true, 3, EDT>(a, c.splitk, c.group_m, st);
     switch (c.bm) {
       CG_CASE(256)
       CG_CASE(128)
@@ -793,22 +787,22 @@
 #endif
   if (a.subpix) {
     switch (c.bm) {
-      case 256: return cg_launch_hpw<256, true, 4, EDT>(a, 1, st);
-      case 128: return cg_launch_hpw<128, true, 4, EDT>(a, 1, st);
-      default: return cg_launch_hpw<64, true, 4, EDT>(a, 1, st);
+      case 256: return cg_launch_hpw<256, true, 4, EDT>(a, 1, c.group_m, st);
+      case 128: return cg_launch_hpw<128, true, 4, EDT>(a, 1, c.group_m, st);
+      default: return cg_launch_hpw<64, true, 4, EDT>(a, 1, c.group_m, st);
     }
   }
   if (!a.gn_in_acc) {
     switch (c.bm) {
-      case 256: return cg_launch_hpw<256, true, 2, EDT>(a, c.splitk, st);
-      case 128: return cg_launch_hpw<128, true, 2, EDT>(a, c.splitk, st);
-      default: return cg_launch_hpw<64, true, 2, EDT>(a, c.splitk, st);
+      case 256: return cg_launch_hpw<256, true, 2, EDT>(a, c.splitk, c.group_m, st);
+      case 128: return cg_launch_hpw<128, true, 2, EDT>(a, c.splitk, c.group_m, st);
+      default: return cg_launch_hpw<64, true, 2, EDT>(a, c.splitk, c.group_m, st);
     }
   }
   switch (c.bm) {
-    case 256: return cg_launch_hpw<256, true, 1, EDT>(a, c.splitk, st);
-    case 128: return cg_launch_hpw<128, true, 1, EDT>(a, c.splitk, st);
-    default: return cg_launch_hpw<64, true, 1, EDT>(a, c.splitk, st);
+    case 256: return cg_launch_hpw<256, true, 1, EDT>(a, c.splitk, c.group_m, st);
+    case 128: return cg_launch_hpw<128, true, 1, EDT>(a, c.splitk, c.group_m, st);
+    default: return cg_launch_hpw<64, true, 1, EDT>(a, c.splitk, c.group_m, st);
   }
 }
 
@@ -828,6 +822,11 @@
   }
   *c = cg_choose(a);
   return 1;
+}
+void pp_conv_gn_operand_bytes(const PPGemmArgs& a, int bm, long long* panel, long long* strip) {
+  const long long px = bm + 2 * a.wout;
+  *panel = (a.up ? (px + 3) / 4 : px) * (a.c1 + a.c2) * 2ll + (long long)bm * (a.c3 + a.c4) * 2ll;
+  *strip = (long long)(a.N < CG_BN ? a.N : CG_BN) * a.K * 2ll * (a.subpix ? 4 : 1);
 }
 int pp_conv_gn_run(const PPGemmArgs& a, const CGChoice& c, hipStream_t st) {
   if (c.splitk > 1 && !a.workspace) return PP_ERR_WORKSPACE;
diff --git a/powerpaint_amd/csrc/gemm.hip b/powerpaint_amd/csrc/gemm.hip
--- a/powerpaint_amd/csrc/gemm.hip
+++ b/powerpaint_amd/csrc/gemm.hip
@@ -1,3 +1,7 @@
+#include <array>
+#include <map>
+#include <mutex>
+
 #include "pp_common.h"
 #include "gemm_gn.h"
 #include "gemm_combine.h"
@@ -6,7 +10,7 @@
 
 struct GemmDerived {
   int tiles_m, tiles_n, kt_total, kt_per_split, ctiles;
-  int n_major;
+  int group_m;
 };
 
 PP_DEVINL void ln_row_moments(const PPGemmArgs& a, int m, float& mean, float& rstd) {
@@ -108,13 +112,7 @@
     lid = (xcd < r ? xcd * (q + 1) : r * (q + 1) + (xcd - r) * q) + idx;
   }
   int tile_m, tile_n;
-  if (d.n_major) {
-    tile_n = lid / d.tiles_m;
-    tile_m = lid - tile_n * d.tiles_m;
-  } else {
-    tile_m = lid / d.tiles_n;
-    tile_n = lid - tile_m * d.tiles_n;
-  }
+  pp_tile_decode(lid, d.tiles_m, d.tiles_n, d.group_m, &tile_m, &tile_n);
   const int m_blk = tile_m * BM, n_blk = tile_n * BN;
   const int split = blockIdx.y;
   const int kt_begin = split * d.kt_per_split;
@@ -336,13 +334,7 @@
     lid = (xcd < r ? xcd * (q + 1) : r * (q + 1) + (xcd - r) * q) + idx;
   }
   int tile_m, tile_n;
-  if (d.n_major) {
-    tile_n = lid / d.tiles_m;
-    tile_m = lid - tile_n * d.tiles_m;
-  } else {
-    tile_m = lid / d.tiles_n;
-    tile_n = lid - tile_m * d.tiles_n;
-  }
+  pp_tile_decode(lid, d.tiles_m, d.tiles_n, d.group_m, &tile_m, &tile_n);
   const int m_blk = tile_m * BM, n_blk = tile_n * BN;
   const int split = blockIdx.y;
   const int kt_begin = split * d.kt_per_split;
@@ -1355,8 +1347,9 @@
 struct TileForm {
   int id, bm;
   bool pp, v2;
+  int waves, stages;
 };
-#define PP_ROW(ID, BM_, WM_, NS_, PP_, V2_) {ID, BM_, PP_, V2_},
+#define PP_ROW(ID, BM_, WM_, NS_, PP_, V2_) {ID, BM_, PP_, V2_, WM_ * 2, NS_},
 constexpr TileForm TILE_FORMS[] = {PP_TILE_FORMS(PP_ROW)};
 #undef PP_ROW
 const TileForm* tile_form(int id) {
@@ -1369,7 +1362,7 @@
   int tile, splitk;
 };
 bool gemm_pingpong();
-bool gemm_n_major();
+bool gemm_tile_order();
 
 bool v2_ok(const PPGemmArgs& a) {
   if (a.N % 8) return false;
@@ -1482,24 +1475,24 @@
   return PP_OK;
 }
 
-GemmDerived derive(const PPGemmArgs& a, int bm, int bn, int splitk) {
+GemmDerived derive(const PPGemmArgs& a, int bm, int bn, int splitk, int group_m) {
   GemmDerived d;
   d.tiles_m = (a.M + bm - 1) / bm;
   d.tiles_n = (a.N + bn - 1) / bn;
   d.kt_total = a.K / 64;
   d.kt_per_split = (d.kt_total + splitk - 1) / splitk;
   d.ctiles = (a.c1 + a.c2) / 64;
-  d.n_major = (gemm_n_major() && d.tiles_m < d.tiles_n && d.tiles_m <= 8) ? 1 : 0;
+  d.group_m = group_m < 1 ? 1 : group_m > d.tiles_m ? d.tiles_m : group_m;
   return d;
 }
 
 template <int BM, int BN, int WM, int WN, int XMODE, int EDT>
-int launch(const PPGemmArgs& a, int splitk, hipStream_t st) {
+int launch(const PPGemmArgs& a, int splitk, int group_m, hipStream_t st) {
   constexpr int T = WM * WN * 64;
   constexpr int LDS = 2 * (BM + BN) * 128;
   auto kern = pp_gemm_kernel<BM, BN, WM, WN, XMODE, EDT>;
   if (pp_func_lds(reinterpret_cast<const void*>(kern), LDS, "hipFuncSetAttribute(gemm)") != PP_OK) return PP_ERR_LAUNCH;
-  const GemmDerived d = derive(a, BM, BN, splitk);
+  const GemmDerived d = derive(a, BM, BN, splitk, group_m);
   dim3 grid(d.tiles_m * d.tiles_n, splitk, 1);
   hipLaunchKernelGGL(kern, grid, dim3(T), LDS, st, a, d);
   PP_CHECK_LAUNCH("pp_gemm_kernel");
@@ -1507,7 +1500,7 @@
   return PP_OK;
 }
 
-bool gemm_n_major() {
+bool gemm_tile_order() {
   static const int v = pp_lab_env("PP_GEMM_NMAJOR", 1);
   return v != 0;
 }
@@ -1523,24 +1516,24 @@
 }
 
 template <int BM, int BN, int WM, int WN, int XMODE, int NS, int EPI, bool PP, int EDT>
-int launch2(const PPGemmArgs& a, int splitk, hipStream_t st) {
+int launch2(const PPGemmArgs& a, int splitk, int group_m, hipStream_t st) {
   if constexpr (EPI == 0) {
-    if ((a.gn_acc[0] || a.gn_acc[1]) && splitk == 1) return launch2<BM, BN, WM, WN, XMODE, NS, 4, PP, EDT>(a, splitk, st);
+    if ((a.gn_acc[0] || a.gn_acc[1]) && splitk == 1) return launch2<BM, BN, WM, WN, XMODE, NS, 4, PP, EDT>(a, splitk, group_m, st);
   }
   if constexpr (XMODE == PP_X_PLAIN && EPI == 0) {
     if (a.act == PP_ACT_SOFTMAX80) {
-      if constexpr (BM == 64 && NS == 3 && !PP) return launch2<BM, BN, WM, WN, XMODE, NS, 5, PP, EDT>(a, splitk, st);
+      if constexpr (BM == 64 && NS == 3 && !PP) return launch2<BM, BN, WM, WN, XMODE, NS, 5, PP, EDT>(a, splitk, group_m, st);
       else return PP_ERR_UNSUPPORTED;
     }
-    if (a.act == PP_ACT_GEGLU && splitk == 1) return launch2<BM, BN, WM, WN, XMODE, NS, 2, PP, EDT>(a, splitk, st);
-    if (a.ln_stats || a.row_stats_out) return launch2<BM, BN, WM, WN, XMODE, NS, 1, PP, EDT>(a, splitk, st);
+    if (a.act == PP_ACT_GEGLU && splitk == 1) return launch2<BM, BN, WM, WN, XMODE, NS, 2, PP, EDT>(a, splitk, group_m, st);
+    if (a.ln_stats || a.row_stats_out) return launch2<BM, BN, WM, WN, XMODE, NS, 1, PP, EDT>(a, splitk, group_m, st);
   }
   constexpr bool LNF = EPI == 1 || EPI == 2 || EPI == 5;
   constexpr int T = WM * WN * 64;
   constexpr int LDS = NS * (BM + BN) * 128 + (LNF ? 2048 + BM * 32 : 0);
   static_assert(LDS <= 160 * 1024 || (LNF && NS > 2), "LDS budget");
   if constexpr (LDS > 160 * 1024) {
-    return launch2<BM, BN, WM, WN, XMODE, 2, EPI, false, EDT>(a, splitk, st);
+    return launch2<BM, BN, WM, WN, XMODE, 2, EPI, false, EDT>(a, splitk, group_m, st);
   } else {
 #ifdef PP_LAB
   auto kern = pp_gemm_kernel_v2<BM, BN, WM, WN, XMODE, NS, EPI, false, PP, EDT>;
@@ -1551,7 +1544,7 @@
   auto kern = pp_gemm_kernel_v2<BM, BN, WM, WN, XMODE, NS, EPI, (NS >= 3 && !PP), PP, EDT>;
 #endif
   if (pp_func_lds(reinterpret_cast<const void*>(kern), LDS, "hipFuncSetAttribute(gemm v2)") != PP_OK) return PP_ERR_LAUNCH;
-  const GemmDerived d = derive(a, BM, BN, splitk);
+  const GemmDerived d = derive(a, BM, BN, splitk, group_m);
   dim3 grid(d.tiles_m * d.tiles_n, splitk, 1);
   hipLaunchKernelGGL(kern, grid, dim3(T), LDS, st, a, d);
   PP_CHECK_LAUNCH("pp_gemm_kernel_v2");
@@ -1570,7 +1563,7 @@
 }
 
 int validate(const PPGemmArgs& a) {
-  if (a.M <= 0 || a.N <= 0 || a.K <= 0 || !pp_dt_ok(a.dtype)) return PP_ERR_BAD_ARG;
+  if (a.M <= 0 || a.N <= 0 || a.K <= 0 || !pp_dt_ok(a.dtype) || a.tile_group_m < 0) return PP_ERR_BAD_ARG;
   if (a.K % 64 != 0 || a.N % 4 != 0) return PP_ERR_BAD_ARG;
   if (!a.x1 || !a.w || !a.out) return PP_ERR_BAD_ARG;
   if (a.x_mode == PP_X_PLAIN) {
@@ -1648,8 +1641,52 @@
   int bm, tiles;
   int splitk;
   bool pp_tile;
+  int group_m = 1;
   bool staged_epilogue() const { return family != Family::V1; }
 };
+
+int form_group_m(const PPGemmArgs& a, const LaunchForm& f, int lds, int waves, int wgs_per_tile) {
+  const int tiles_n = (a.N + 159) / 160, tiles_m = (a.M + f.bm - 1) / f.bm;
+  if (a.tile_group_m > 0) return a.tile_group_m < tiles_m ? a.tile_group_m : tiles_m;
+  const int legacy = pp_tile_order_legacy(tiles_m, tiles_n);
+  if (a.w_batch_stride > 0) return legacy;
+  if (!gemm_tile_order()) return 1;
+  static const int classes = pp_lab_env("PP_TILE_ORDER_CLASSES", 1);
+  static const int min_pct = pp_lab_env("PP_TILE_ORDER_MIN_PCT", (int)(PP_TILE_ORDER_MIN_SAVING * 100.0 + 0.5));
+  const int cls = f.family == Family::HALO ? 1 : a.x_mode == PP_X_CONV3X3 ? 2 : f.splitk > 1 ? 4 : 8;
+  if (!(classes & cls)) return legacy;
+  PPTileOrderIn in;
+  in.tiles_m = tiles_m;
+  in.tiles_n = tiles_n;
+  in.splits = f.splitk;
+  in.row_bytes = 2ll * a.K;
+  if (f.family == Family::HALO) {
+    pp_conv_gn_operand_bytes(a, f.bm, &in.panel_bytes, &in.strip_bytes);
+  } else if (a.x_mode == PP_X_CONV3X3) {
+    const long long src = a.up ? (f.bm + 3) / 4 : (long long)f.bm * a.stride * a.stride;
+    in.panel_bytes = (src + 2 * a.win) * (a.c1 + a.c2) * 2ll + (long long)f.bm * (a.c3 + a.c4) * 2ll;
+    in.strip_bytes = (long long)(a.N < 160 ? a.N : 160) * a.K * 2ll;
+  } else {
+    in.panel_bytes = (long long)(a.M < f.bm ? a.M : f.bm) * a.K * 2ll;
+    in.strip_bytes = (long long)(a.N < 160 ? a.N : 160) * a.K * 2ll;
+  }
+  int per_cu = (160 * 1024) / (lds > 0 ? lds : 1);
+  if (per_cu > 32 / waves) per_cu = 32 / waves;
+  per_cu = per_cu < 1 ? 1 : per_cu > 2 ? 2 : per_cu;
+  in.resident_per_xcd = per_cu * ((pp_cu_count() + PP_XCDS - 1) / PP_XCDS) / wgs_per_tile;
+  in.l2_bytes = pp_l2_bytes();
+  typedef std::array<long long, 9> Key;
+  static std::mutex mu;
+  static std::map<Key, int> memo;
+  const Key key = {in.tiles_m, in.tiles_n, in.splits, in.panel_bytes, in.strip_bytes, in.row_bytes, in.resident_per_xcd, in.l2_bytes,
+                   min_pct};
+  std::lock_guard<std::mutex> lock(mu);
+  auto it = memo.find(key);
+  if (it != memo.end()) return it->second;
+  const int g = pp_tile_order_choose(in, min_pct * 0.01);
+  if (memo.size() < 4096) memo[key] = g;
+  return g;
+}
 
 int resolve_form(const PPGemmArgs& a, LaunchForm* f) {
   const int tn = (a.N + 159) / 160;
@@ -1658,12 +1695,17 @@
   if (halo < 0) return halo;
   if (halo) {
     *f = LaunchForm{Family::HALO, 0, cg.bm, (a.M / cg.bm) * tn * (a.subpix ? 4 : 1), cg.splitk, true};
+    f->group_m = form_group_m(a, *f, 160 * 1024, 8, a.subpix ? 4 : 1);
     return PP_OK;
   }
   const Choice c = choose(a);
   const TileForm* t = tile_form(c.tile);
   if (!t) return PP_ERR_BAD_ARG;
   *f = LaunchForm{t->v2 ? Family::V2 : Family::V1, t->id, t->bm, ((a.M + t->bm - 1) / t->bm) * tn, c.splitk, t->pp};
+  const bool lnf = t->v2 && a.x_mode == PP_X_PLAIN && (a.ln_stats || a.row_stats_out || a.act == PP_ACT_GEGLU || a.act == PP_ACT_SOFTMAX80);
+  int lds = (t->v2 ? t->stages : 2) * (t->bm + 160) * 128 + (lnf ? 2048 + t->bm * 32 : 0);
+  if (lds > 160 * 1024) lds = 2 * (t->bm + 160) * 128 + 2048 + t->bm * 32;
+  f->group_m = form_group_m(a, *f, lds, t->waves, 1);
   return PP_OK;
 }
 
@@ -1676,9 +1718,9 @@
 }
 
 template <bool V2, int BM, int WM, int NS, bool PP, int XMODE, int EDT>
-int launch_tile(const PPGemmArgs& a, int splitk, hipStream_t st) {
-  if constexpr (V2) return launch2<BM, 160, WM, 2, XMODE, NS, 0, PP, EDT>(a, splitk, st);
-  else return launch<BM, 160, WM, 2, XMODE, EDT>(a, splitk, st);
+int launch_tile(const PPGemmArgs& a, int splitk, int group_m, hipStream_t st) {
+  if constexpr (V2) return launch2<BM, 160, WM, 2, XMODE, NS, 0, PP, EDT>(a, splitk, group_m, st);
+  else return launch<BM, 160, WM, 2, XMODE, EDT>(a, splitk, group_m, st);
 }
 
 template <int EDT>
@@ -1687,8 +1729,8 @@
   switch (f.tile) {
 #define PP_CASE(ID, BM_, WM_, NS_, PP_, V2_)                                                         \
     case ID:                                                                                         \
-      return conv ? launch_tile<V2_, BM_, WM_, NS_, PP_, PP_X_CONV3X3, EDT>(a, f.splitk, st)         \
-                  : launch_tile<V2_, BM_, WM_, NS_, PP_, PP_X_PLAIN, EDT>(a, f.splitk, st);
+      return conv ? launch_tile<V2_, BM_, WM_, NS_, PP_, PP_X_CONV3X3, EDT>(a, f.splitk, f.group_m, st) \
+                  : launch_tile<V2_, BM_, WM_, NS_, PP_, PP_X_PLAIN, EDT>(a, f.splitk, f.group_m, st);
     PP_TILE_FORMS(PP_CASE)
 #undef PP_CASE
     default:
@@ -1724,6 +1766,11 @@
 }
 
 static bool combine_fused(const PPGemmArgs& a, const LaunchForm& f) { return a.tile_ctr && combine_fusable(a, f, true, false); }
+
+extern "C" int pp_gemm_tile_group_m(const PPGemmArgs* args) {
+  LaunchForm f;
+  return query_form(args, &f) ? f.group_m : 0;
+}
 
 extern "C" int pp_gemm_combine_fused(const PPGemmArgs* args) {
   LaunchForm f;
@@ -1752,7 +1799,7 @@
   if (a.gn_next_out && !gn_next_ok(a, f, a.gn_next_sub)) return PP_ERR_UNSUPPORTED;
   if (f.family == Family::HALO) {
     if ((a.gn_acc[0] || a.gn_acc[1]) && !gn_stats_supported(a)) return PP_ERR_UNSUPPORTED;
-    const int rc = pp_conv_gn_run(a, CGChoice{f.bm, f.splitk}, st);
+    const int rc = pp_conv_gn_run(a, CGChoice{f.bm, f.splitk, f.group_m}, st);
     if (rc != PP_OK || f.splitk == 1 || fused) return rc;
     return a.dtype == PP_DT_F16 ? launch_combine<PP_DT_F16>(a, f.splitk, st) : launch_combine<PP_DT_BF16>(a, f.splitk, st);
   }
diff --git a/powerpaint_amd/csrc/pp_api.cpp b/powerpaint_amd/csrc/pp_api.cpp
--- a/powerpaint_amd/csrc/pp_api.cpp
+++ b/powerpaint_amd/csrc/pp_api.cpp
@@ -40,6 +40,21 @@
   int n = 0;
   if (hipDeviceGetAttribute(&n, hipDeviceAttributeMultiprocessorCount, dev) != hipSuccess || n <= 0) n = 256;
   cus[dev] = n;
+  return n;
+}
+
+long long pp_l2_bytes() {
+  static std::mutex mu;
+  static std::map<int, long long> l2;
+  int dev = 0;
+  if (hipGetDevice(&dev) != hipSuccess) return 4ll << 20;
+  std::lock_guard<std::mutex> g(mu);
+  auto it = l2.find(dev);
+  if (it != l2.end()) return it->second;
+  int n = 0;
+  if (hipDeviceGetAttribute(&n, hipDeviceAttributeL2CacheSize, dev) != hipSuccess || n <= 0) n = 4 << 20;
+  if (n > (4 << 20)) n = 4 << 20;
+  l2[dev] = n;
   return n;
 }
 
diff --git a/powerpaint_amd/csrc/pp_common.h b/powerpaint_amd/csrc/pp_common.h
--- a/powerpaint_amd/csrc/pp_common.h
+++ b/powerpaint_amd/csrc/pp_common.h
@@ -4,6 +4,7 @@
 #include <stdlib.h>
 
 #include "pp_hip.h"
+#include "tile_order.h"
 
 typedef __attribute__((ext_vector_type(8))) __bf16 bf16x8_t;
 typedef __attribute__((ext_vector_type(4))) float f32x4_t;
@@ -114,9 +115,12 @@
 void pp_set_last_error(const char* what, hipError_t e);
 int pp_func_lds(const void* kern, int bytes, const char* what);
 int pp_cu_count();
+long long pp_l2_bytes();
 struct CGChoice {
   int bm, splitk;
+  int group_m = 1;
 };
+void pp_conv_gn_operand_bytes(const PPGemmArgs& a, int bm, long long* panel, long long* strip);
 int pp_conv_gn_form(const PPGemmArgs& a, CGChoice* c);
 int pp_conv_gn_run(const PPGemmArgs& a, const CGChoice& c, hipStream_t st);
 #define PP_CHECK_LAUNCH(what)                         \
diff --git a/powerpaint_amd/csrc/tile_order.h b/powerpaint_amd/csrc/tile_order.h
--- /dev/null
+++ b/powerpaint_amd/csrc/tile_order.h
@@ -0,0 +1,93 @@
+#pragma once
+
+#if defined(__HIPCC__)
+#define PP_TO_FN __host__ __device__ __forceinline__
+#else
+#define PP_TO_FN inline
+#endif
+
+constexpr int PP_XCDS = 8;
+
+PP_TO_FN void pp_tile_decode(int id, int tiles_m, int tiles_n, int group_m, int* tile_m, int* tile_n) {
+  const int per_group = group_m * tiles_n;
+  const int g = id / per_group;
+  const int first = g * group_m;
+  int h = tiles_m - first;
+  if (h > group_m) h = group_m;
+  const int r = id - g * per_group;
+  const int tn = r / h;
+  *tile_m = first + (r - tn * h);
+  *tile_n = tn;
+}
+
+inline void pp_xcd_range(int nwg, int xcd, int* first, int* count) {
+  const int q = nwg / PP_XCDS, r = nwg % PP_XCDS;
+  *first = xcd < r ? xcd * (q + 1) : r * (q + 1) + (xcd - r) * q;
+  *count = q + (xcd < r ? 1 : 0);
+}
+
+struct PPTileOrderIn {
+  int tiles_m, tiles_n;
+  int splits;
+  long long panel_bytes;
+  long long strip_bytes;
+  long long row_bytes;
+  int resident_per_xcd;
+  long long l2_bytes;
+};
+
+inline double pp_tile_order_bytes(const PPTileOrderIn& in, int group_m) {
+  const int tiles = in.tiles_m * in.tiles_n;
+  if (tiles <= 0 || group_m < 1) return 0.0;
+  if (group_m > in.tiles_m) group_m = in.tiles_m;
+  constexpr int MAXT = 64;
+  const int window = in.resident_per_xcd < 1 ? 1 : in.resident_per_xcd > MAXT ? MAXT : in.resident_per_xcd;
+  double total = 0.0;
+  for (int x = 0; x < PP_XCDS; ++x) {
+    int first, count;
+    pp_xcd_range(tiles, x, &first, &count);
+    for (int w0 = 0; w0 < count; w0 += window) {
+      const int w1 = w0 + window < count ? w0 + window : count;
+      int pm[MAXT], pn[MAXT], npm = 0, npn = 0;
+      for (int i = w0; i < w1; ++i) {
+        int tm, tn;
+        pp_tile_decode(first + i, in.tiles_m, in.tiles_n, group_m, &tm, &tn);
+        bool seen = false;
+        for (int k = 0; k < npm; ++k) seen |= pm[k] == tm;
+        if (!seen && npm < MAXT) pm[npm++] = tm;
+        seen = false;
+        for (int k = 0; k < npn; ++k) seen |= pn[k] == tn;
+        if (!seen && npn < MAXT) pn[npn++] = tn;
+      }
+      const double shared = (double)npm * (double)in.panel_bytes + (double)npn * (double)in.strip_bytes;
+      const double rows = shared / (double)(in.row_bytes > 0 ? in.row_bytes : 1);
+      const double together = rows * 512.0 * (double)(in.splits > 0 ? in.splits : 1);
+      const bool unshared = together > (double)in.l2_bytes;
+      total += unshared ? (double)(w1 - w0) * (double)(in.panel_bytes + in.strip_bytes) : shared;
+    }
+  }
+  return total;
+}
+
+constexpr double PP_TILE_ORDER_MIN_SAVING = 0.10;
+
+inline int pp_tile_order_legacy(int tiles_m, int tiles_n) { return (tiles_m < tiles_n && tiles_m <= 8) ? tiles_m : 1; }
+
+inline int pp_tile_order_choose(const PPTileOrderIn& in, double min_saving = PP_TILE_ORDER_MIN_SAVING) {
+  const int legacy = pp_tile_order_legacy(in.tiles_m, in.tiles_n);
+  if (in.tiles_m <= 1 || in.tiles_n <= 1) return legacy;
+  const double base = pp_tile_order_bytes(in, legacy);
+  int best = legacy;
+  double best_bytes = base;
+  for (int g = 1;; g *= 2) {
+    if (g > in.tiles_m) g = in.tiles_m;
+    const double b = pp_tile_order_bytes(in, g);
+    if (b < best_bytes) {
+      best_bytes = b;
+      best = g;
+    }
+    if (g == in.tiles_m) break;
+  }
+  if (best_bytes > base * (1.0 - min_saving)) return legacy;
+  return best;
+}
diff --git a/powerpaint_amd/engine.py b/powerpaint_amd/engine.py
--- a/powerpaint_amd/engine.py
+++ b/powerpaint_amd/engine.py
@@ -226,7 +226,8 @@
         a = getattr(args[0], "_obj", None) if args else None
         if isinstance(a, L.PPGemmArgs):
             return (f"{name} M={a.M} N={a.N} K={a.K} {'conv' if a.x_mode else 'lin'}"
-                    f"{' s2' if a.stride == 2 else ''}{' up' if a.up else ''}{' cat' if a.c2 else ''}")
+                    f"{' s2' if a.stride == 2 else ''}{' up' if a.up else ''}{' cat' if a.c2 else ''}"
+                    f" gm={L.lib().pp_gemm_tile_group_m(C.byref(a))}")
         return name
 
 
diff --git a/powerpaint_amd/ops.py b/powerpaint_amd/ops.py
--- a/powerpaint_amd/ops.py
+++ b/powerpaint_amd/ops.py
@@ -150,7 +150,7 @@
 
 def gemm(x: torch.Tensor, w: torch.Tensor, bias=None, x2=None, res1=None, res2=None, scale: float = 1.0, act: int = 0,
          rowvec=None, rows_per_batch: int = 0, out_f32: bool = False, vt_col0: int = 0, tile: int = 0,
-         splitk: int = 0, row_stats: bool = False, ln_stats=None, ln_colsum=None, ln_dim: int = 0,
+         splitk: int = 0, tile_group_m: int = 0, row_stats: bool = False, ln_stats=None, ln_colsum=None, ln_dim: int = 0,
          ln_eps: float = 1e-5, gn=None, res1_wrap: int = 0, fuse_combine: bool = False, out=None, vt=None, stats=None,
          workspace=None):
     lib = L.lib()
@@ -185,7 +185,7 @@
         a.out_vt, a.vt_col0, a.vt_ld = _p(vt), vt_col0, vt.stride(1)
     elif vt is not None:
         raise L.PPError("gemm: `vt` without vt_col0")
-    a.tile, a.splitk = tile, splitk
+    a.tile, a.splitk, a.tile_group_m = tile, splitk, tile_group_m
     _set_gn(a, gn, rows_per_batch)
     if row_stats:
         tn = (N + 159) // 160
@@ -235,7 +235,7 @@
 def conv3x3(x: torch.Tensor, w: torch.Tensor, bias=None, stride: int = 1, up: bool = False, x2=None, rowvec=None,
             res1=None, res2=None, scale: float = 1.0, tile: int = 0, splitk: int = 0, gn=None, x3=None, x4=None,
             gn_in=None, gn_next=None, dup: bool = False, gn_dup_mask: int = 0, res1_wrap: int = 0,
-            fuse_combine: bool = False, out=None, workspace=None, ynext=None, up_size=None):
+            fuse_combine: bool = False, out=None, workspace=None, ynext=None, up_size=None, tile_group_m: int = 0):
     lib = L.lib()
     B, C1, C2, cout = x.shape[0], x.shape[3], (x2.shape[3] if x2 is not None else 0), w.shape[0]
     a = _conv_request(x, cout, stride, up, x2, x3, x4, up_size)
@@ -257,7 +257,7 @@
         a.out_dup_rows = a.M
         if gn_dup_mask:
             a.gn_dup_batch, a.gn_dup_mask = B, gn_dup_mask
-    a.tile, a.splitk = tile, splitk
+    a.tile, a.splitk, a.tile_group_m = tile, splitk, tile_group_m
     _set_gn(a, gn, ho * wo)
     if gn_next is None and ynext is not None:
         raise L.PPError("conv3x3: `ynext` without gn_next")
@@ -293,7 +293,7 @@
 
 
 def conv3x3_up_subpix(x: torch.Tensor, wfold: torch.Tensor, bias=None, rowvec=None, res1=None, res2=None, scale: float = 1.0,
-                      tile: int = 0, splitk: int = 0, gn=None, out=None, workspace=None):
+                      tile: int = 0, splitk: int = 0, gn=None, out=None, workspace=None, tile_group_m: int = 0):
     B, H, W, C1 = x.shape
     cout = wfold.shape[1]
     assert tuple(wfold.shape) == (4, cout, 4 * C1) and wfold.is_contiguous()
@@ -309,7 +309,7 @@
     a.ldres2 = _res_ld(res2, (B, 2 * H, 2 * W, cout), x, "conv3x3_up_subpix: `res2`")
     if rowvec is not None and rowvec.dim() == 2 and rowvec.shape[0] > 1:
         a.ld_rowvec = rowvec.stride(0)
-    a.tile, a.splitk = tile, splitk
+    a.tile, a.splitk, a.tile_group_m = tile, splitk, tile_group_m
     _set_gn(a, gn, H * W)
     a.workspace = _p(_workspace(L.lib(), a, x.device, workspace))
     L.check(L.lib().pp_gemm_bf16(C.byref(a), _s()), "pp_gemm_bf16(sub-pixel upsampling conv)")
```

Measured after the change: 9.286 images/s (median of 6 runs). 1.01x the previous value.
